# george-tyler-315-incline/ggml-neon-opt

Hardware: AMD Instinct MI355X
Metric: tg128 tok/s + Q4_K GEMV achieved-HBM-GB/s, TinyLlama-1.1B Q4_K_M @1 GPU (higher is better)
Workload: dtype q4_K/q6_K x q8_K (u4/u6*i8 dot4 -> i32, f32 combine); 1 GPU; tinyllama-1.1b Q4_K_M tg2221: full decode graph, token i at position i of a fresh f16 KV cache; parallelism=replicas x1, hipgraph=True

## Files before the change

ggml-neon-opt_amd/csrc/kq_api.hip:

```cpp
#include <algorithm>
#include <stdio.h>
#include <stdlib.h>
#include <string.h>

#include <atomic>
#include <mutex>
#include <string>
#include <vector>

#include <hip/hip_ext.h>

#include "kq_common.h"
#include "kq_internal.h"

namespace kq {

template <int NCOL, bool FUSEDQ, bool DEBUG, int TMASK>
__global__ void kq_gemv(const GemvArgs a);
__global__ void kq_quantize_q8K(const float *x, int64_t x_stride, uint8_t *y, int nb, int64_t nblocks);
template <int TMASK, bool FUSEDQ, int PRO>
__global__ void kq_rows(KQ_ROWS_PARAMS);
template <int TMASK, bool FUSEDQ, int PRO>
__global__ void kq_rows_dyn(KQ_ROWS_PARAMS);
template <bool AM>
__global__ void kq_quantize_q8L(const float *x, int64_t x_stride, uint8_t *y, int nb, int64_t nblocks);
template <int TYPE, int RT, int CW>
__global__ void kq_mmq(const MmqArgs a);
template <int RT, int CW>
__global__ void kq_mmq_mixed(const MmqArgs a);
__global__ void kq_stream_ceiling(const uint8_t *buf, int64_t per_wave, int waves_total, uint32_t *sink);
__global__ void kq_quantize_f16img(const float *x, int64_t x_stride, uint8_t *img, uint8_t *bs, int nb, int64_t nblocks);
template <int TYPE, int NW>
__global__ void kq_mmf(const MmfArgs a);
__global__ void kq_mmf_reduce(const float *slab, int n_split, int m_cols, int n_rows, int slab_rows, float *y,
                              int64_t y_col_stride, const float *res, int64_t res_col_stride);

namespace {

constexpr int kMaxDevices = 64;
std::mutex g_dev_mu;
std::atomic<int> g_dev_state[kMaxDevices];
int g_dev_cus[kMaxDevices] = {0};

int current_device() {
    int dev = 0;
    if (hipGetDevice(&dev) != hipSuccess || dev < 0 || dev >= kMaxDevices) return -1;
    return dev;
}

void probe_device(int dev) {
    int n = 0;
    if (hipGetDeviceCount(&n) != hipSuccess || n <= 0 || dev >= n) {
        g_dev_state[dev].store(-1);
        return;
    }
    hipDeviceProp_t prop;
    if (hipGetDeviceProperties(&prop, dev) != hipSuccess) {
        g_dev_state[dev].store(-1);
        return;
    }
    if (strncmp(prop.gcnArchName, "gfx950", 6) != 0) {
        fprintf(stderr, "ggml_mi355x: device %d is %s, this library is built for gfx950 only\n", dev,
                prop.gcnArchName);
        g_dev_state[dev].store(-1);
        return;
    }
    g_dev_cus[dev] = prop.multiProcessorCount > 0 ? prop.multiProcessorCount : 256;
    g_dev_state[dev].store(1, std::memory_order_release);
}

template <int NCOL, bool FUSEDQ, bool DEBUG>
gemv_fn pick_tm(int tmask) {
    switch (tmask) {
        case 1: return kq_gemv<NCOL, FUSEDQ, DEBUG, 1>;
        case 4: return kq_gemv<NCOL, FUSEDQ, DEBUG, 4>;
        default: return kq_gemv<NCOL, FUSEDQ, DEBUG, 7>;
    }
}

gemv_fn pick_gemv(int ncol, bool fusedq, bool debug, int tmask) {
    if (debug) return pick_tm<1, false, true>(tmask);
    if (fusedq) return pick_tm<1, true, false>(tmask);
    switch (ncol) {
        case 1: return pick_tm<1, false, false>(tmask);
        case 2: return pick_tm<2, false, false>(tmask);
        case 4: return pick_tm<4, false, false>(tmask);
        default: return pick_tm<8, false, false>(tmask);
    }
}

int type_bit(int type) { return type == Q4_K ? 1 : type == Q5_K ? 2 : type == Q6_K ? 4 : 0; }

constexpr size_t kMaxLds = 160 * 1024;
constexpr size_t kTargetLds = 80 * 1024;
constexpr int64_t kFusedQMaxNb = 32;
constexpr int64_t kRowsFusedMaxNb = ROWS_QPASS * 4 * ROWS_WAVES;
constexpr double kRowsSmallBytes = 5e6;
std::atomic<int> g_rows_waves{0};

struct KnobDef {
    const char *name;
    double def;
};
const KnobDef kKnobs[KNOB_COUNT] = {
    {"GEMV_DIAG", 0},  {"GEMV_RING", 0},     {"GEMV_PRE0", 1},       {"GEMV_PF", 0},
// ... 147 lines not shown
    a.R = BLOCKS_PER_STEP;
    a.m_total = (int)M;
    int64_t tasks = 0;
    for (int i = 0; i < n_desc; ++i) {
        a.type[i] = d[i].type;
        a.n_rows[i] = (int)d[i].n_rows;
        a.w[i] = (const uint8_t *)d[i].w;
        a.row_stride[i] = (int64_t)d[i].row_stride;
        a.y[i] = d[i].y;
        a.task_prefix[i] = (int)tasks;
        tasks += (d[i].n_rows + a.R - 1) / a.R;
    }
    if (tasks > 0x7fffffff) return MI355X_E_INVAL;
    for (int i = n_desc; i <= MI355X_MAX_FUSED; ++i) a.task_prefix[i] = (int)tasks;
    a.tasks_total = (int)tasks;
    pl.ncol = ncol;
    pl.fusedq = fusedq;
    pl.debug = debug;
    pl.tmask = tmask;
    pl.fn = pick_gemv(ncol, fusedq, debug, tmask);
    a.diag = (int)knob(KNOB_GEMV_DIAG);
    a.ring_override = (int)knob(KNOB_GEMV_RING);
    a.stamps = g_stamps;
    a.stamps_cap = g_stamps_cap;
    const int slot = tmask == 1 ? 8 * 16 * 9 : 8 * 16 * 14;
    const int dcands[3] = {tmask == 1 ? 8 : 6, tmask == 1 ? 6 : 5, 4};
    int D = 4;
    for (int i = 0; i < 3; ++i) {
        D = dcands[i];
        if ((size_t)lds_layout(ncol, (int)nb, 8 * ncol, fusedq, slot, D).total <= kTargetLds) break;
    }
    if (a.ring_override > 0) D = a.ring_override < 13 ? a.ring_override : 13;
    a.ring = D;
    const int64_t base_lds = lds_layout(ncol, (int)nb, 0, fusedq, slot, D).total;
    if ((size_t)base_lds > kMaxLds) return MI355X_E_UNSUPPORTED;
    int64_t wgs = (int64_t)num_cus() * resident_wgs((const void *)pl.fn, (size_t)base_lds + 1024);
    if (wgs > tasks) wgs = tasks > 0 ? tasks : 1;
    int64_t tpw = (tasks + wgs - 1) / wgs;
    while (tpw * 8 * ncol * 4 > 4096 && tpw > 1) {
        wgs *= 2;
        tpw = (tasks + wgs - 1) / wgs;
    }
    a.out_per_wg = (int)(tpw * 8 * ncol);
    const LdsLayout L = lds_layout(ncol, (int)nb, a.out_per_wg, fusedq, slot, D);
    if ((size_t)L.total > kMaxLds) return MI355X_E_UNSUPPORTED;
    pl.lds = (size_t)L.total;
    pl.grid = dim3((unsigned)wgs, (unsigned)((M + ncol - 1) / ncol), 1);
    return MI355X_OK;
}

void allow_lds(const void *fn, size_t lds) {
    if (lds <= 64 * 1024) return;
    static std::mutex mu;
    static std::vector<std::pair<int, const void *>> done;
    const int dev = current_device();
    std::lock_guard<std::mutex> lk(mu);
    for (auto &e : done)
        if (e.first == dev && e.second == fn) return;
    hipFuncSetAttribute(fn, hipFuncAttributeMaxDynamicSharedMemorySize, (int)kMaxLds);
    done.push_back({dev, fn});
}

int launch_gemv(const GemvPlan &pl, hipStream_t stream) {
    const GemvArgs &a = pl.a;
    if (a.tasks_total == 0 || a.m_total == 0) return MI355X_OK;
    allow_lds((const void *)pl.fn, pl.lds);
    hipEvent_t e0, e1;
    if (timing_slot(stream, e0, e1)) {
        hipExtLaunchKernelGGL(pl.fn, pl.grid, dim3(WG_THREADS), (uint32_t)pl.lds, stream, e0, e1, 0, a);
        timing_log(gemv_name(pl), gemv_bytes(a, pl.fusedq), e0, e1);
    } else {
        hipLaunchKernelGGL(pl.fn, pl.grid, dim3(WG_THREADS), pl.lds, stream, a);
    }
    const hipError_t e = hipGetLastError();
    return e == hipSuccess ? MI355X_OK : (int)e;
}

std::atomic<int> g_impl{MI355X_GEMV_AUTO};
bool rows_enabled() {
    return g_impl.load() != MI355X_GEMV_TASKS;
}


template <int TM, bool FQ, int PR>
rows_fn rows_inst(bool dyn) {
    if constexpr (TM == 7) {
        return kq_rows<TM, FQ, PR>;
    } else {
        return dyn ? kq_rows_dyn<TM, FQ, PR> : kq_rows<TM, FQ, PR>;
    }
}

template <int TM>
rows_fn rows_pick_pro(bool fusedq, int pro, bool dyn) {
    if (!fusedq) return rows_inst<TM, false, 0>(dyn);
    return pro == ROWS_PRO_NORM ? rows_inst<TM, true, 1>(dyn) : pro == ROWS_PRO_SWIGLU ? rows_inst<TM, true, 2>(dyn)
                                                                                       : rows_inst<TM, true, 0>(dyn);
}

rows_fn pick_rows(int tmask, bool fusedq, int pro, bool dyn = false) {
    switch (tmask) {
        case 1: return rows_pick_pro<1>(fusedq, pro, dyn);
        case 2: return rows_pick_pro<2>(fusedq, pro, dyn);
        case 4: return rows_pick_pro<4>(fusedq, pro, dyn);
        default: return rows_pick_pro<7>(fusedq, pro, false);
    }
}

int plan_rows(const mi355x_gemv_desc *d, int n_desc, int64_t K, bool fusedq, RowsPlan &pl, int waves_per_cu) {
    RowsArgs &a = pl.a;
    if (n_desc < 1 || n_desc > MI355X_MAX_FUSED) return MI355X_E_INVAL;
    if (K <= 0 || K % QK != 0) return MI355X_E_INVAL;
    const int64_t nb = K / QK;
    if (nb > 4096) return MI355X_E_UNSUPPORTED;
    if (fusedq && nb > kRowsFusedMaxNb) return MI355X_E_UNSUPPORTED;
    memset(&a, 0, sizeof(a));
    int tmask = 0;
    double bytes_total = 0;
    for (int i = 0; i < n_desc; ++i) {
        const int bb = block_bytes(d[i].type);
        if (!bb) return MI355X_E_UNSUPPORTED;
        if (d[i].n_rows < 0 || d[i].n_rows > 0x7fffffff) return MI355X_E_INVAL;
        if (d[i].n_rows > 0) {
            if (!d[i].w || !d[i].y) return MI355X_E_INVAL;
            if (((uintptr_t)d[i].w & 3u) != 0) return MI355X_E_INVAL;
            if (d[i].row_stride != (size_t)(nb * bb)) return MI355X_E_UNSUPPORTED;
            if (d[i].type != Q6_K && ((uintptr_t)d[i].w & 15u)) return MI355X_E_UNSUPPORTED;
        }
        bytes_total += (double)d[i].n_rows * bb;
        tmask |= type_bit(d[i].type);
    }
    if (tmask != 1 && tmask != 2 && tmask != 4) tmask = 7;
    pl.tmask = tmask;
    pl.fusedq = fusedq;
    pl.fn = pick_rows(tmask, fusedq, ROWS_PRO_NONE);
    a.n_desc = n_desc;
    a.nb = (int)nb;
    for (int i = 0; i < n_desc; ++i) {
        a.type[i] = d[i].type;
        a.w[i] = (const uint8_t *)d[i].w;
        a.y[i] = d[i].y;
        a.n_rows[i] = (int)d[i].n_rows;
    }
    {
        a.pf = (int)knob(KNOB_GEMV_PF);
        a.xmode = (int)knob(KNOB_GEMV_XMODE) & 7;
        a.diag = (int)knob(KNOB_GEMV_DIAG);
        const int pre = (int)knob(KNOB_GEMV_PRE0);
        a.pre0 = pre < 0 ? 0 : pre > 3 ? 3 : pre;
    }
    a.stamps = g_stamps;
    a.stamps_cap = g_stamps_cap;
    const double small_bytes = knob(KNOB_GEMV_SMALL_MB) * 1e6;
    if (waves_per_cu <= 0) {
        const int fixed = g_rows_waves.load();
        const int want = fixed > 0 ? fixed : bytes_total * nb < small_bytes ? ROWS_WAVES_SMALL : ROWS_WAVES;
        waves_per_cu = !fusedq || nb <= ROWS_QPASS * 4 * want ? want : ROWS_WAVES;
    }
    if (waves_per_cu > ROWS_WAVES) return MI355X_E_INVAL;
    pl.nwv = waves_per_cu;
    const int wpc_env = (int)knob(KNOB_GEMV_WPC);
    if (wpc_env > 0 && wpc_env < waves_per_cu) waves_per_cu = wpc_env;
    const int small_wg_env = (int)knob(KNOB_GEMV_SMALL_WG);
    int64_t n_wg = num_cus();
    if (small_wg_env > 0 && bytes_total * nb < small_bytes && small_wg_env < n_wg) n_wg = small_wg_env;
    const int64_t cap = n_wg * waves_per_cu;
    int64_t wv[MI355X_MAX_FUSED] = {0, 0, 0, 0};
    int64_t waves = 0;
    for (int i = 0; i < n_desc; ++i) {
        if (d[i].n_rows == 0) continue;
        const double share = (double)d[i].n_rows * block_bytes(d[i].type) / bytes_total;
        int64_t w = (int64_t)(share * (double)cap);
        const int64_t min_rows = (ROWS_SB + nb - 1) / nb;
        const int64_t wmax = (d[i].n_rows + min_rows - 1) / min_rows;
        if (w > wmax) w = wmax;
        if (w < 1) w = 1;
        wv[i] = w;
        waves += w;
    }
    while (waves > cap) {
        int big = 0;
        for (int i = 1; i < n_desc; ++i)
            if (wv[i] > wv[big]) big = i;
        --wv[big];
        --waves;
    }
    int64_t rpw = 0;
    waves = 0;
    for (int i = 0; i < n_desc; ++i) {
        a.wave_prefix[i] = (int)waves;
        if (wv[i] > 0) {
            a.rbase[i] = (int)(d[i].n_rows / wv[i]);
            a.rrem[i] = (int)(d[i].n_rows % wv[i]);
            const int64_t r = a.rbase[i] + (a.rrem[i] ? 1 : 0);
            rpw = r > rpw ? r : rpw;
        }
        waves += wv[i];
    }
    for (int i = n_desc; i <= MI355X_MAX_FUSED; ++i) a.wave_prefix[i] = (int)waves;
    a.waves_total = (int)waves;
    a.prio_bytes = 0;
    for (int i = 0; i < n_desc; ++i)
        if (wv[i] > 0) {
            const int64_t b = (int64_t)(a.rbase[i] + (a.rrem[i] ? 1 : 0)) * nb * block_bytes(d[i].type);
            a.prio_bytes = b > a.prio_bytes ? b : a.prio_bytes;
        }
    if (rpw > 0x7fffffff / 64) return MI355X_E_UNSUPPORTED;
    a.rpw = (int)(rpw > 0 ? rpw : 1);
    int g16 = ROWS_SB;
    while (nb % g16) g16 >>= 1;
    const int u = ROWS_SB / g16;
    int bR_full = (int)(ROWS_RECS / nb) / u * u;
    if (bR_full < u) bR_full = u;
    a.bR = a.rpw <= bR_full ? a.rpw : bR_full;
    const RowsLayout L = rows_layout((int)nb, tmask, a.bR, a.rpw, pl.nwv);
    if ((size_t)L.total > kMaxLds) return MI355X_E_UNSUPPORTED;
    pl.lds = (size_t)L.total;
    const int64_t grid = waves < n_wg ? waves : n_wg;
    pl.grid = dim3((unsigned)(grid > 0 ? grid : 1), 1, 1);
    pl.dyn = false;
    const double dyn_min = knob(KNOB_GEMV_DYN);
    const bool force = g_impl.load() == MI355X_GEMV_DYN;
    bool same_rows = true;
    for (int i = 1; i < n_desc; ++i) same_rows = same_rows && d[i].n_rows == d[0].n_rows;
    if (tmask != 7 && same_rows && (force || dyn_min > 0)) {
        int ush = 0;
        while ((int64_t)(1 << ush) * nb < ROWS_SB) ++ush;
        const double steps_per_wave = (double)n_desc * d[0].n_rows * nb / ROWS_SB / n_wg / pl.nwv;
        if ((int64_t)(1 << ush) * nb == ROWS_SB && steps_per_wave >= 16) ++ush;
        const int U = 1 << ush;
        const int Tu = (int)((U * nb + ROWS_SB - 1) / ROWS_SB);
        const int D = rows_depth(tmask == 1 ? Q4_K : tmask == 2 ? Q5_K : Q6_K);
        const int64_t flat = (int64_t)n_desc * ((d[0].n_rows + n_wg - 1) / n_wg);
        const int64_t rows = (int64_t)n_desc * d[0].n_rows;
        int bRd = (int)(ROWS_RECS / nb) / U * U;
        if (bRd < U) bRd = U;
        const double per_wave = (double)rows / (double)n_wg / U / pl.nwv;
        const bool auto_ok = per_wave >= dyn_min && steps_per_wave >= knob(KNOB_GEMV_DYN_STEPS);
        const RowsDynLayout DL = rows_dyn_layout((int)nb, tmask, bRd, (int)flat, pl.nwv);
        if ((force || auto_ok) && rows > 0 && (size_t)DL.total <= kMaxLds && flat < 0x7fffffff / 64) {
            pl.dyn = true;
            a.dyn_u = U;
            a.dyn_ush = ush;
            a.rbase[0] = (int)(d[0].n_rows / n_wg);
            a.rrem[0] = (int)(d[0].n_rows % n_wg);
            a.dyn_p = (D + Tu - 1) / Tu;
            const int p_knob = (int)knob(KNOB_GEMV_DYN_P);
            if (p_knob > 0) a.dyn_p = p_knob;
            a.bR = bRd;
            a.rpw = (int)flat;
            pl.lds = (size_t)DL.total;
            pl.grid = dim3((unsigned)n_wg, 1, 1);
            pl.fn = pick_rows(tmask, fusedq, ROWS_PRO_NONE, true);
        }
    }
    return MI355X_OK;
}

std::string rows_name(const RowsPlan &pl) {
    return std::string(pl.dyn ? "kq::kq_rows_dyn<" : "kq::kq_rows<") + std::to_string(pl.tmask) + ", " + (pl.fusedq ? "true" : "false") + ", " +
           std::to_string(pl.a.pro) + ">";
}

double rows_bytes(const RowsArgs &a, bool fusedq) {
    double w = 0, y = 0;
    for (int i = 0; i < a.n_desc; ++i) {
        const double rows = (double)a.n_rows[i];
        w += rows * a.nb * block_bytes(a.type[i]);
        y += rows * 4.0;
    }
    return w + y + (fusedq ? (double)a.nb * QK * 4.0 : (double)a.nb * Q8L_STRIDE);
}

int launch_rows(const RowsPlan &pl, hipStream_t stream) {
    const RowsArgs &a = pl.a;
    if (a.waves_total == 0) return MI355X_OK;
    allow_lds((const void *)pl.fn, pl.lds);
    const void *x = pl.fusedq ? (const void *)a.x : (const void *)a.xq;
    const int pass = 4 * pl.nwv;
    const int qiters = pl.fusedq ? (a.nb + pass - 1) / pass : 0;
    if (pl.nwv < 1 || pl.nwv > ROWS_WAVES || qiters > ROWS_QPASS || a.n_desc < 1 || a.n_desc > MI355X_MAX_FUSED)
        return MI355X_E_INVAL;
    const int cfg = rows_cfg(pl.nwv, qiters, a.n_desc, a.diag & 0x1ff);
    const int grid = (int)pl.grid.x;
    hipEvent_t e0, e1;
    if (timing_slot(stream, e0, e1)) {
        hipExtLaunchKernelGGL(pl.fn, pl.grid, dim3(pl.nwv * 64), (uint32_t)pl.lds, stream, e0, e1, 0, x, a.x2, a.w[0],
                              a.res[0], a.nb, a.waves_total, grid, cfg, a.rbase[0], a.rrem[0], a);
        timing_log(rows_name(pl), rows_bytes(a, pl.fusedq), e0, e1);
    } else {
        hipLaunchKernelGGL(pl.fn, pl.grid, dim3(pl.nwv * 64), pl.lds, stream, x, a.x2, a.w[0], a.res[0], a.nb,
                           a.waves_total, grid, cfg, a.rbase[0], a.rrem[0], a);
    }
    const hipError_t e = hipGetLastError();
    return e == hipSuccess ? MI355X_OK : (int)e;
}

int launch_quantize_q8L(const float *x, int64_t x_stride_floats, void *y, int64_t k, int64_t nrows,
                        hipStream_t stream, bool mmq) {
    const auto kern = mmq ? kq_quantize_q8L<true> : kq_quantize_q8L<false>;
    const int64_t nb = k / QK;
    const int64_t nblocks = nb * nrows;
    if (nblocks == 0) return MI355X_OK;
    const int64_t wgs = (nblocks + 15) / 16;
    hipEvent_t e0, e1;
    if (timing_slot(stream, e0, e1)) {
        hipExtLaunchKernelGGL(kern, dim3((unsigned)wgs), dim3(WG_THREADS), 0, stream, e0, e1, 0, x,
                              x_stride_floats, (uint8_t *)y, (int)nb, nblocks);
        timing_log("kq::kq_quantize_q8L", (double)nblocks * (QK * 4.0 + Q8L_STRIDE), e0, e1);
    } else {
        hipLaunchKernelGGL(kern, dim3((unsigned)wgs), dim3(WG_THREADS), 0, stream, x, x_stride_floats,
                           (uint8_t *)y, (int)nb, nblocks);
    }
    const hipError_t e = hipGetLastError();
    return e == hipSuccess ? MI355X_OK : (int)e;
}

constexpr int64_t kMmqMinCols = 16;

std::atomic<int> g_mmq_impl{MI355X_MMQ_AUTO};
int mmq_impl() { return g_mmq_impl.load(); }

struct MmqShape {
    int rt, cw;
};
MmqShape mmq_shape(int type, int64_t rows, int64_t M) {
    const int impl = mmq_impl();
    if (impl == MI355X_MMQ_TILE128) return {128, 1};
    if (impl == MI355X_MMQ_TILE128W) return {128, 2};
    if (impl == MI355X_MMQ_TILE64W) return {64, 2};
    if (impl == MI355X_MMQ_TILE64) return {64, 1};
    if (impl == MI355X_MMQ_TILE128X) return {128, type == Q6_K ? 2 : 4};
    if (impl == MI355X_MMQ_TILE192) return type == Q6_K ? MmqShape{128, 1} : MmqShape{192, 1};
    const int64_t rt128 = (rows + 127) / 128;
    const int64_t g128x128 = rt128 * ((M + 127) / 128), g128x64 = rt128 * ((M + 63) / 64);
    if (type != Q6_K && g128x128 >= 160 && g128x128 < 384 && g128x64 >= 512) return {128, 1};
    if (g128x128 >= 160) return {128, 2};
    if (type == Q6_K && ((rows + 63) / 64) * ((M + 127) / 128) >= 192) return {64, 2};
    if (type != Q6_K && rt128 * ((M + 63) / 64) >= 256) return {128, 1};
    return {64, 1};
}
const void *mmq_fn(int type, bool mixed, MmqShape sh) {
#define KQ_MMQ_PICK(RT, CW)                                                      \
    return mixed          ? (const void *)kq_mmq_mixed<RT, CW>                 \
         : type == Q5_K ? (const void *)kq_mmq<Q5_K, RT, CW>                   \
         : type == Q6_K ? (const void *)kq_mmq<Q6_K, RT, CW>                   \
                        : (const void *)kq_mmq<Q4_K, RT, CW>;
    if (sh.rt == 192 && !mixed && type != Q6_K)
        return type == Q5_K ? (const void *)kq_mmq<Q5_K, 192, 1> : (const void *)kq_mmq<Q4_K, 192, 1>;
    if (sh.rt == 128 && sh.cw == 4 && !mixed && type != Q6_K)
        return type == Q5_K ? (const void *)kq_mmq<Q5_K, 128, 4> : (const void *)kq_mmq<Q4_K, 128, 4>;
    if (sh.rt == 128 && sh.cw == 2) KQ_MMQ_PICK(128, 2)
    if (sh.rt == 64 && sh.cw == 2) KQ_MMQ_PICK(64, 2)
    if (sh.rt == 128) KQ_MMQ_PICK(128, 1)
    KQ_MMQ_PICK(64, 1)
#undef KQ_MMQ_PICK
}
size_t mmq_lds(int type, MmqShape sh) {
    return (size_t)mmq_nbuf(type, sh.rt, sh.cw) * (size_t)mmq_buf_bytes(type, sh.rt, sh.cw) + 16 + MMQ_PF_LDS;
}

int launch_mmq(int type, const void *w, int64_t K, int64_t N, size_t row_stride, const uint8_t *xq, int64_t M,
               float *y, int64_t y_col_stride, hipStream_t stream, const float *res, int64_t res_col_stride) {
// ... 254 lines not shown
        a.kv_k_cache = kv->k_cache;
        a.kv_v_cache = kv->v_cache;
        a.kv_n_ctx = kv->n_ctx;
        a.kv_hd = kv->hd;
    }
    a.w = a.mw[0];
    a.row_stride = a.mrow_stride[0];
    a.n_rows = a.mn_rows[0];
    a.y = a.my[0];
    a.y_col_stride = a.my_col_stride[0];
    const void *fn = mmq_fn(type, mixed, sh);
    size_t lds = mmq_lds(mixed ? Q6_K : type, sh);
    if (mixed) lds = std::max(lds, std::max(mmq_lds(Q4_K, sh), mmq_lds(Q5_K, sh)));
    const dim3 grid((unsigned)((M + mmq_cols(sh.cw) - 1) / mmq_cols(sh.cw)), (unsigned)tiles, 1);
    allow_lds(fn, lds);
    hipEvent_t e0, e1;
    void *args[] = {&a};
    hipError_t e;
    if (timing_slot(stream, e0, e1)) {
        e = hipExtLaunchKernel(fn, grid, dim3((unsigned)(64 * mmq_waves(rt, sh.cw))), args, lds, stream, e0, e1, 0);
        timing_log(mixed ? std::string("kq::kq_mmq_mixed") : std::string("kq::kq_mmq<") + std::to_string(type) + ">", wbytes + (double)M * a.nb * Q8L_STRIDE + ybytes,
                   e0, e1);
    } else {
        e = hipLaunchKernel(fn, grid, dim3((unsigned)(64 * mmq_waves(rt, sh.cw))), args, lds, stream);
    }
    if (e != hipSuccess) return (int)e;
    e = hipGetLastError();
    return e == hipSuccess ? MI355X_OK : (int)e;
}

bool mmq_applies(int type, const void *w, int64_t N, size_t row_stride, int64_t M) {
    if (!rows_enabled() || M < kMmqMinCols || N <= 0) return false;
    if (type != Q4_K && type != Q5_K && type != Q6_K) return false;
    if (N >= (1ll << 31) || M >= (1ll << 31)) return false;
    if (type == Q6_K) return true;
    return ((uintptr_t)w & 15u) == 0 && (row_stride & 15u) == 0;
}

int launch_quantize(const float *x, int64_t x_stride_floats, void *y, int64_t k, int64_t nrows,
                    hipStream_t stream) {
    const int64_t nb = k / QK;
    const int64_t nblocks = nb * nrows;
    if (nblocks == 0) return MI355X_OK;
    const int64_t wgs = (nblocks + WAVES_PER_WG - 1) / WAVES_PER_WG;
    hipEvent_t e0, e1;
    if (timing_slot(stream, e0, e1)) {
        hipExtLaunchKernelGGL(kq_quantize_q8K, dim3((unsigned)wgs), dim3(WG_THREADS), 0, stream, e0, e1, 0, x,
                              x_stride_floats, (uint8_t *)y, (int)nb, nblocks);
        timing_log("kq::kq_quantize_q8K", (double)nblocks * (QK * 4.0 + 292.0), e0, e1);
    } else {
        hipLaunchKernelGGL(kq_quantize_q8K, dim3((unsigned)wgs), dim3(WG_THREADS), 0, stream, x, x_stride_floats,
                           (uint8_t *)y, (int)nb, nblocks);
    }
    const hipError_t e = hipGetLastError();
    return e == hipSuccess ? MI355X_OK : (int)e;
}

size_t ext_x_bytes(int64_t k) { return ((size_t)k * 4 + 255) & ~(size_t)255; }

int gemv_m1(const mi355x_gemv_desc *d, int n, const float *x, int64_t k, void *ws, size_t ws_size,
            hipStream_t stream, const mi355x_gemv_ext *ext) {
    const bool has_ext = ext && (ext->prologue != MI355X_PRO_NONE || ext->epilogue != MI355X_EPI_NONE || [&] {
        for (int i = 0; i < n && i < MI355X_MAX_FUSED; ++i)
            if (ext->residual[i]) return true;
        return false;
    }());
    if (has_ext) {
        if (ext->prologue != MI355X_PRO_NONE && !ext->x2) return MI355X_E_INVAL;
        const bool epi = ext->epilogue == MI355X_EPI_SWIGLU;
        if (ext->epilogue != MI355X_EPI_NONE && !epi) return MI355X_E_INVAL;
        if (epi && (n != 2 || !ext->epi_y || d[0].n_rows != d[1].n_rows || ext->residual[0] || ext->residual[1]))
            return MI355X_E_INVAL;
        const bool x2_ok = ext->prologue == MI355X_PRO_NONE || ((uintptr_t)ext->x2 & 15u) == 0;
        if (rows_enabled() && k / QK <= kRowsFusedMaxNb && ((uintptr_t)x & 15u) == 0 && x2_ok) {
            RowsPlan rp;
            const int rc = plan_rows(d, n, k, true, rp);
            if (rc == MI355X_OK) {
                rp.a.x = x;
                rp.a.pro = ext->prologue == MI355X_PRO_RMS_NORM ? ROWS_PRO_NORM
                           : ext->prologue == MI355X_PRO_SWIGLU ? ROWS_PRO_SWIGLU
                                                                : ROWS_PRO_NONE;
                rp.a.x2 = ext->x2;
                rp.a.eps = ext->eps;
                rp.fn = pick_rows(rp.tmask, true, rp.a.pro, rp.dyn);
                for (int i = 0; i < n; ++i) {
                    rp.a.res[i] = ext->residual[i];
                    rp.a.n_rows[i] = (int)d[i].n_rows;
                }
                const int g = (int)rp.grid.x;
                const bool paired = epi && (rp.dyn || (rp.a.wave_prefix[2] == 2 * rp.a.wave_prefix[1] &&
                                                       rp.a.wave_prefix[1] % g == 0 && rp.a.rbase[0] == rp.a.rbase[1] &&
                                                       rp.a.rrem[0] == rp.a.rrem[1]));
                if (!epi || paired) {
                    if (paired) {
                        rp.a.epi = 1;
                        rp.a.epi_n = (int)d[0].n_rows;
                        rp.a.epi_wave_off = rp.a.wave_prefix[1] / g;
                        rp.a.epi_y = ext->epi_y;
                    }
                    if (!device_ok()) return MI355X_E_NODEVICE;
                    return launch_rows(rp, stream);
                }
            } else if (rc != MI355X_E_UNSUPPORTED) {
                return rc;
            }
        }
        const float *xs = x;
        uint8_t *w8 = (uint8_t *)ws;
        size_t wsz = ws_size;
        if (ext->prologue != MI355X_PRO_NONE) {
            if (!ws || ws_size < ext_x_bytes(k) || ((uintptr_t)ws & 15u)) return MI355X_E_WORKSPACE;
            if (!device_ok()) return MI355X_E_NODEVICE;
            float *xt = (float *)ws;
            const int rc = ext->prologue == MI355X_PRO_RMS_NORM ? launch_rms_norm(x, ext->x2, xt, k, 1, ext->eps, stream)
                                                                : launch_swiglu(x, ext->x2, xt, k, stream);
            if (rc) return rc;
            xs = xt;
            w8 += ext_x_bytes(k);
            wsz -= ext_x_bytes(k);
        }
        int rc = gemv_m1(d, n, xs, k, w8, wsz, stream, nullptr);
        if (rc) return rc;
        for (int i = 0; i < n; ++i)
            if (ext->residual[i] && d[i].n_rows > 0) {
                rc = launch_binary(0, d[i].y, ext->residual[i], d[i].y, d[i].n_rows, stream);
                if (rc) return rc;
            }
        if (epi && d[0].n_rows > 0) return launch_swiglu(d[0].y, d[1].y, ext->epi_y, d[0].n_rows, stream);
        return MI355X_OK;
    }
    const bool fusedq = k / QK <= kFusedQMaxNb && ((uintptr_t)x & 15u) == 0;
    const size_t need = (size_t)(k / QK) * 292;
    if (rows_enabled()) {
        RowsPlan rp;
        const int64_t fq_max = (int64_t)knob(KNOB_GEMV_FQMAX);
        const bool rows_fq = k / QK <= fq_max && k / QK <= kRowsFusedMaxNb && ((uintptr_t)x & 15u) == 0;
        int rc = plan_rows(d, n, k, rows_fq, rp);
        if (rc == MI355X_OK) {
            if (rows_fq) {
                rp.a.x = x;
                if (!device_ok()) return MI355X_E_NODEVICE;
                return launch_rows(rp, stream);
            }
            const size_t need_l = (size_t)(k / QK) * Q8L_STRIDE;
            if (!ws || ws_size < need_l || ((uintptr_t)ws & 15u)) return MI355X_E_WORKSPACE;
            if (!device_ok()) return MI355X_E_NODEVICE;
            rc = launch_quantize_q8L(x, k, ws, k, 1, stream);
            if (rc) return rc;
            rp.a.xq = (const uint8_t *)ws;
            return launch_rows(rp, stream);
        }
        if (rc != MI355X_E_UNSUPPORTED) return rc;
    }
    GemvPlan pl;
    int rc = plan_gemv(d, n, k, 1, 1, fusedq, false, pl);
    if (rc) return rc;
    if (fusedq) {
        pl.a.x = x;
        pl.a.x_col_stride = k;
        if (!device_ok()) return MI355X_E_NODEVICE;
        return launch_gemv(pl, stream);
    }
    if (!ws || ws_size < need || ((uintptr_t)ws & 3u)) return MI355X_E_WORKSPACE;
    if (!device_ok()) return MI355X_E_NODEVICE;
    rc = launch_quantize(x, k, ws, k, 1, stream);
    if (rc) return rc;
    pl.a.xq = (const uint8_t *)ws;
// ... 153 lines not shown
    if (ne11 == 0 || ne01 == 0) return MI355X_OK;
    if (!src1 || ((uintptr_t)src1 & 3u) || (nb11 & 3u) || !dst || ((uintptr_t)dst & 3u) || (nb1 & 3u))
        return MI355X_E_INVAL;
    if (ne11 > 1 && (nb11 < (size_t)ne00 * 4 || nb1 < (size_t)ne01 * 4)) return MI355X_E_INVAL;
    if (ne11 == 1) {
        mi355x_gemv_desc d = {src0_type, src0, ne01, nb01, dst};
        return gemv_m1(&d, 1, src1, ne00, workspace, workspace_size, (hipStream_t)stream);
    }
    size_t need = mi355x_mul_mat_workspace_size(src0_type, ne00, ne01, ne11);
    if (!workspace || workspace_size < need) return MI355X_E_WORKSPACE;
    if (mmf_applies(src0_type, src0, ne01, nb01, ne11, ne00) && ((uintptr_t)workspace & 15u) == 0) {
        if (!device_ok()) return MI355X_E_NODEVICE;
        int rc = launch_f16img(src1, (int64_t)(nb11 / 4), (uint8_t *)workspace, ne00, ne11, (hipStream_t)stream);
        if (rc) return rc;
        return launch_mmf_gemm(src0_type, src0, ne00, ne01, nb01, (uint8_t *)workspace, ne11, dst, (int64_t)(nb1 / 4),
                               (hipStream_t)stream);
    }
    if (mmq_applies(src0_type, src0, ne01, nb01, ne11) && ((uintptr_t)workspace & 15u) == 0) {
        if (!device_ok()) return MI355X_E_NODEVICE;
        int rc = launch_quantize_q8L(src1, (int64_t)(nb11 / 4), workspace, ne00, ne11, (hipStream_t)stream, true);
        if (rc) return rc;
        return launch_mmq(src0_type, src0, ne00, ne01, nb01, (const uint8_t *)workspace, ne11, dst,
                          (int64_t)(nb1 / 4), (hipStream_t)stream);
    }
    if (!device_ok()) return MI355X_E_NODEVICE;
    int rc = launch_quantize(src1, (int64_t)(nb11 / 4), workspace, ne00, ne11, (hipStream_t)stream);
    if (rc) return rc;
    const size_t q8_row = (size_t)(ne00 / QK) * 292;
    return mi355x_mul_mat_q8(src0_type, src0, ne00, ne01, nb01, workspace, ne11, q8_row, dst, nb1, stream);
}

int mi355x_gemv_fused(const mi355x_gemv_desc *descs, int n_desc, const float *x, int64_t k, void *workspace,
                      size_t workspace_size, void *stream) {
    if (!descs || !x || ((uintptr_t)x & 3u)) return MI355X_E_INVAL;
    if (k <= 0 || k % QK) return MI355X_E_INVAL;
    for (int i = 0; i < n_desc && i < MI355X_MAX_FUSED; ++i)
        if (descs[i].y && ((uintptr_t)descs[i].y & 3u)) return MI355X_E_INVAL;
    return gemv_m1(descs, n_desc, x, k, workspace, workspace_size, (hipStream_t)stream);
}

size_t mi355x_gemv_ext_workspace_size(int64_t k) {
    if (k <= 0 || k % QK) return 0;
    return ext_x_bytes(k) + mi355x_gemv_fused_workspace_size(k);
}

int mi355x_gemv_fused_ext(const mi355x_gemv_desc *descs, int n_desc, const float *x, int64_t k,
                          const mi355x_gemv_ext *ext, void *workspace, size_t workspace_size, void *stream) {
    if (!descs || !x || ((uintptr_t)x & 3u)) return MI355X_E_INVAL;
    if (k <= 0 || k % QK || n_desc < 1 || n_desc > MI355X_MAX_FUSED) return MI355X_E_INVAL;
    if (ext && (ext->prologue < MI355X_PRO_NONE || ext->prologue > MI355X_PRO_SWIGLU)) return MI355X_E_INVAL;
    if (ext && ext->prologue == MI355X_PRO_RMS_NORM && !(ext->eps >= 0.0f)) return MI355X_E_INVAL;
    if (ext && ext->epilogue == MI355X_EPI_SWIGLU && ((uintptr_t)ext->epi_y & 3u)) return MI355X_E_INVAL;
    for (int i = 0; i < n_desc; ++i) {
        if (descs[i].y && ((uintptr_t)descs[i].y & 3u)) return MI355X_E_INVAL;
        if (ext && ext->residual[i] && ((uintptr_t)ext->residual[i] & 3u)) return MI355X_E_INVAL;
    }
    return gemv_m1(descs, n_desc, x, k, workspace, workspace_size, (hipStream_t)stream, ext);
}

int mi355x_debug_stream(const void *buf, size_t bytes, void *sink, void *stream) {
    if (!buf || !sink || ((uintptr_t)buf & 15u)) return MI355X_E_INVAL;
    int dev = current_device();
    if (dev < 0 || !device_ok()) return MI355X_E_NODEVICE;
    const int cus = g_dev_cus[dev] > 0 ? g_dev_cus[dev] : 256;
    const int waves = cus * 12;
    const int64_t per_wave = (int64_t)(bytes / waves) / 2048 * 2048;
    if (per_wave <= 0) return MI355X_E_INVAL;
    const size_t lds = 4 * 4 * 2048;
    allow_lds((const void *)kq_stream_ceiling, lds);
    hipStream_t st = (hipStream_t)stream;
    hipEvent_t e0, e1;
    if (timing_slot(st, e0, e1)) {
        hipExtLaunchKernelGGL(kq_stream_ceiling, dim3((unsigned)(cus * 3)), dim3(256), (uint32_t)lds, st, e0, e1, 0,
                              (const uint8_t *)buf, per_wave, waves, (uint32_t *)sink);
        timing_log("kq::kq_stream_ceiling", (double)per_wave * waves, e0, e1);
    } else {
        hipLaunchKernelGGL(kq_stream_ceiling, dim3((unsigned)(cus * 3)), dim3(256), lds, st, (const uint8_t *)buf,
                           per_wave, waves, (uint32_t *)sink);
    }
    const hipError_t e = hipGetLastError();
    return e == hipSuccess ? MI355X_OK : (int)e;
}

int mi355x_debug_block_partials(int src0_type, const void *src0, int64_t ne00, int64_t ne01, size_t nb01,
                                const void *src1_q8, int32_t *out, void *stream) {
    if (!out || !src1_q8 || ((uintptr_t)src1_q8 & 3u)) return MI355X_E_INVAL;
    if (ne01 == 0) return MI355X_OK;
    const int64_t nb = ne00 / QK;
    float *dst = (float *)out;
    mi355x_gemv_desc d = {src0_type, src0, ne01, nb01, dst};
    GemvPlan pl;
    int rc = plan_gemv(&d, 1, ne00, 1, 1, false, true, pl);
    if (rc) return rc;
    pl.a.xq = (const uint8_t *)src1_q8;
    pl.a.xq_col_stride = (int64_t)(nb * 292);
    pl.a.dbg = out;
    if (!device_ok()) return MI355X_E_NODEVICE;
    return launch_gemv(pl, (hipStream_t)stream);
}

int mi355x_gemv_impl(int impl) {
    if (impl < MI355X_GEMV_AUTO || impl > MI355X_GEMV_DYN) return MI355X_E_INVAL;
    return g_impl.exchange(impl);
}

int mi355x_debug_knob(const char *name, double value, double *previous) {
    if (!name) return MI355X_E_INVAL;
    for (int k = 0; k < KNOB_COUNT; ++k) {
        if (strcmp(name, kKnobs[k].name) != 0) continue;
        if (previous) *previous = knob((Knob)k);
        if (value != value) {
            g_knob_set[k].store(false);
        } else {
            g_knob[k].store(value);
            g_knob_set[k].store(true);
        }
        g_knob_gen.fetch_add(1);
        return MI355X_OK;
    }
    return MI355X_E_INVAL;
}

int mi355x_mmq_impl(int impl) {
    if (impl < MI355X_MMQ_AUTO || impl > MI355X_MMQ_TILE192) return MI355X_E_INVAL;
    const int prev = mmq_impl();
    g_mmq_impl.store(impl);
    return prev;
}

int mi355x_prefill_precision(int precision) {
    if (precision < 0) return prefill_precision();
    if (precision > MI355X_PREFILL_F16_ALL) return MI355X_E_INVAL;
    const int prev = prefill_precision();
    g_prefill.store(precision);
    return prev;
}

int mi355x_gemv_waves(int waves) {
    if (waves < 0 || waves > ROWS_WAVES) return MI355X_E_INVAL;
    return g_rows_waves.exchange(waves);
}

}
namespace kq {
uint64_t *diag_stamps(int64_t *cap) {
    if (cap) *cap = g_stamps_cap;
    return g_stamps;
}
}
extern "C" {
int mi355x_diag_stamps(void *buf, size_t bytes) {
    g_stamps = (uint64_t *)buf;
    g_stamps_cap = buf ? (int64_t)(bytes / 8) : 0;
    return MI355X_OK;
}

int mi355x_timing_enable(int enable) {
    std::lock_guard<std::mutex> lk(g_tmu);
    g_timing = enable != 0;
    g_tlog.clear();
    g_tpool_used = 0;
    return MI355X_OK;
}

int mi355x_timing_read(mi355x_launch_timing *out, int max) {
    if (hipDeviceSynchronize() != hipSuccess) return MI355X_E_NODEVICE;
// ... 59 lines not shown
```

ggml-neon-opt_amd/csrc/kq_common.h:

```cpp
#pragma once

#include <hip/hip_runtime.h>
#include <stdint.h>

#include "ggml_mi355x.h"

namespace kq {

constexpr int QK = 256;
constexpr int WAVE = 64;
constexpr int WG_THREADS = 256;
constexpr int WAVES_PER_WG = WG_THREADS / WAVE;
constexpr int LANES_PER_BLOCK = 8;
constexpr int BLOCKS_PER_STEP = WAVE / LANES_PER_BLOCK;
constexpr int ACT_QS_STRIDE = 272;
constexpr int MAX_NCOL = 8;

constexpr int Q4_K = MI355X_TYPE_Q4_K;
constexpr int Q5_K = MI355X_TYPE_Q5_K;
constexpr int Q6_K = MI355X_TYPE_Q6_K;

__host__ __device__ constexpr int block_bytes(int type) {
    return type == Q4_K ? 144 : type == Q5_K ? 176 : type == Q6_K ? 210 : 0;
}

struct GemvArgs {
    int n_desc;
    int nb;
    int R;
    int m_total;
    int tasks_total;
    int out_per_wg;
    int diag;
    int ring;
    int ring_override;
    int task_prefix[MI355X_MAX_FUSED + 1];
    int type[MI355X_MAX_FUSED];
    int n_rows[MI355X_MAX_FUSED];
    const uint8_t *w[MI355X_MAX_FUSED];
    int64_t row_stride[MI355X_MAX_FUSED];
    float *y[MI355X_MAX_FUSED];
    int64_t y_col_stride[MI355X_MAX_FUSED];
    const float *x;
    int64_t x_col_stride;
    const uint8_t *xq;
    int64_t xq_col_stride;
    int32_t *dbg;
    uint64_t *stamps;
    int64_t stamps_cap;
};

struct LdsLayout {
    int ring, act, act_per_wave, act_col, recs, outs, spw, total;
};

__host__ __device__ inline LdsLayout lds_layout(int ncol, int nb, int out_per_wg, bool fusedq, int slot, int D) {
    LdsLayout L;
    L.spw = (nb + WAVES_PER_WG - 1) / WAVES_PER_WG;
    L.ring = 0;
    L.act = WAVES_PER_WG * D * slot;
    L.act_col = (L.spw * 292 + 16 + 15) & ~15;
    L.act_per_wave = fusedq ? L.spw * 1024 : ncol * L.act_col;
    L.recs = L.act + WAVES_PER_WG * L.act_per_wave;
    L.outs = L.recs + 2 * (WAVES_PER_WG - 1) * ncol * 8 * L.spw * 16;
    L.total = L.outs + out_per_wg * 4;
    return L;
}

#ifndef KQ_ROWS_WAVES
#define KQ_ROWS_WAVES 12
#endif
constexpr int ROWS_WAVES = KQ_ROWS_WAVES;
#ifndef KQ_ROWS_WAVES_SMALL
#define KQ_ROWS_WAVES_SMALL 6
#endif
constexpr int ROWS_WAVES_SMALL = KQ_ROWS_WAVES_SMALL;
constexpr int ROWS_QPASS = 3;
#ifndef KQ_ROWS_PF
#define KQ_ROWS_PF 2
#endif
constexpr int ROWS_PF = KQ_ROWS_PF;

#define KQ_ROWS_PARAMS                                                                                        \
    const void *x, const float *x2, const uint8_t *w0, const float *res0, int nb, int waves_total, int grid, \
        int cfg, int rbase0, int rrem0, const RowsArgs a
__host__ __device__ constexpr int rows_cfg(int nwv, int qiters, int n_desc, int diag) {
    return nwv | (qiters << 8) | (n_desc << 12) | (diag << 16);
}

struct RowsArgs {
    int bR;
    int rpw;
    int wave_prefix[MI355X_MAX_FUSED + 1];
    int epi;
    int rbase[MI355X_MAX_FUSED];
    int rrem[MI355X_MAX_FUSED];
    int type[MI355X_MAX_FUSED];
    const uint8_t *w[MI355X_MAX_FUSED];
    const float *res[MI355X_MAX_FUSED];
    float *y[MI355X_MAX_FUSED];
    float *epi_y;
    float eps;
    int epi_n, epi_wave_off;
    int dyn_u, dyn_p, dyn_ush;
    int n_rows[MI355X_MAX_FUSED];
    uint64_t *stamps;
    int64_t stamps_cap;
    int n_desc;
    int nb;
    int waves_total;
    const float *x;
    const uint8_t *xq;
    const float *x2;
    int pro;
    int diag;
    int pre0;
    int pf;
    int xmode;
    int64_t prio_bytes;
};
constexpr int ROWS_PRO_NONE = 0, ROWS_PRO_NORM = 1, ROWS_PRO_SWIGLU = 2;
constexpr int ROWS_X_ROT = 1, ROWS_X_BAR = 2, ROWS_X_PIPE = 4;

constexpr int ROWS_SB = 16;
#ifndef KQ_MMQ_PF
#define KQ_MMQ_PF 0
#endif
constexpr int MMQ_PF_LDS = KQ_MMQ_PF ? 1024 : 0;
constexpr int Q8L_STRIDE = 304;
#ifndef KQ_MMQ_NBUF
#define KQ_MMQ_NBUF 2
#endif
__host__ __device__ constexpr int mmq_cgroups(int cw) { return cw == 4 ? 1 : 2; }
__host__ __device__ constexpr int mmq_cols(int cw) { return 32 * cw * mmq_cgroups(cw); }
__host__ __device__ constexpr int mmq_waves(int rt, int cw) { return rt / 32 * mmq_cgroups(cw); }
#ifndef KQ_MMQ_Q6_STRIDE
#define KQ_MMQ_Q6_STRIDE 240
#endif
static_assert(KQ_MMQ_Q6_STRIDE % 16 == 0 && KQ_MMQ_Q6_STRIDE >= 224, "whole granules");
__host__ __device__ constexpr int mmq_buf_bytes(int type, int rt, int cw) {
    return mmq_cols(cw) * Q8L_STRIDE + rt * (type == Q6_K ? KQ_MMQ_Q6_STRIDE : block_bytes(type));
}
__host__ __device__ constexpr int mmq_nbuf(int type, int rt, int cw) {
    return KQ_MMQ_NBUF == 1 ? 1 : KQ_MMQ_NBUF >= 3 && ((rt == 128 && cw == 1) || (rt == 64 && cw == 2)) &&
                   3 * mmq_buf_bytes(type, rt, cw) + 16 + MMQ_PF_LDS <= 160 * 1024
               ? 3
               : 2;
}
constexpr int ROWS_RECS = 64;
__host__ __device__ constexpr int rows_gran(int type) { return block_bytes(type) + 1; }
__host__ __device__ constexpr int rows_slot(int type) { return 16 * rows_gran(type); }
__host__ __device__ constexpr int rows_ni(int type) { return (rows_gran(type) + 63) / 64; }
#ifndef KQ_ROWS_DQ4
#define KQ_ROWS_DQ4 3
#endif
#ifndef KQ_ROWS_DQ6
#define KQ_ROWS_DQ6 2
#endif
__host__ __device__ constexpr int rows_depth(int type) {
    return type == Q4_K ? KQ_ROWS_DQ4 : type == Q5_K ? 3 : KQ_ROWS_DQ6;
}
__host__ __device__ constexpr int rows_ring_bytes(int type) { return rows_depth(type) * rows_slot(type); }
__host__ __device__ constexpr int cmax(int a, int b) { return a > b ? a : b; }
__host__ __device__ constexpr int rows_ring(int tmask) {
    return 16 + cmax((tmask & 1) ? rows_ring_bytes(Q4_K) : 0,
                     cmax((tmask & 2) ? rows_ring_bytes(Q5_K) : 0, (tmask & 4) ? rows_ring_bytes(Q6_K) : 0));
}

struct RowsLayout {
    int act, ring, ring_stride, recs, recs_stride, outs, outs_stride, sums, total;
// ... 160 lines not shown
```

ggml-neon-opt_amd/csrc/kq_internal.h:

```cpp
#pragma once

#include <string>

#include "kq_common.h"

namespace kq {

int device_ok();
bool timing_slot(hipStream_t s, hipEvent_t &a, hipEvent_t &b);
void timing_log(const std::string &kernel, double bytes, hipEvent_t a, hipEvent_t b);
int num_cus();
int choose_ncol(int64_t M, int nb);
typedef void (*gemv_fn)(const GemvArgs);
struct GemvPlan {
    GemvArgs a;
    dim3 grid;
    size_t lds;
    gemv_fn fn;
    int ncol, tmask;
    bool fusedq, debug;
};
int plan_gemv(const mi355x_gemv_desc *d, int n_desc, int64_t K, int64_t M, int ncol, bool fusedq, bool debug,
              GemvPlan &pl);
int launch_gemv(const GemvPlan &pl, hipStream_t stream);
typedef void (*rows_fn)(KQ_ROWS_PARAMS);
struct RowsPlan {
    RowsArgs a;
    dim3 grid;
    size_t lds;
    rows_fn fn;
    int tmask;
    bool fusedq;
    int nwv;
    bool dyn = false;
};
int plan_rows(const mi355x_gemv_desc *d, int n_desc, int64_t K, bool fusedq, RowsPlan &pl,
              int waves_per_cu = 0);
int launch_rows(const RowsPlan &pl, hipStream_t stream);
bool rows_enabled();
int launch_quantize(const float *x, int64_t x_stride_floats, void *y, int64_t k, int64_t nrows,
                    hipStream_t stream);
int gemv_m1(const mi355x_gemv_desc *d, int n, const float *x, int64_t k, void *ws, size_t ws_size,
            hipStream_t stream, const mi355x_gemv_ext *ext = nullptr);
int launch_rms_norm(const float *x, const float *w, float *y, int64_t n, int64_t nrows, float eps, hipStream_t s);
int launch_binary(int op, const float *a, const float *b, float *y, int64_t n, hipStream_t s,
                  int64_t nb = 0);
int launch_attn_prompt(const AttnArgs &a, int n_tok, hipStream_t s);
int attn_cells_reserve(const AttnArgs &a, hipStream_t stream);
bool attn_prompt_q8_ok(const AttnArgs &a);
bool mmq_applies(int type, const void *w, int64_t N, size_t row_stride, int64_t M);
int launch_quantize_q8L(const float *x, int64_t x_stride_floats, void *y, int64_t k, int64_t nrows,
                        hipStream_t stream, bool mmq = false);
int launch_mmq(int type, const void *w, int64_t K, int64_t N, size_t row_stride, const uint8_t *xq, int64_t M,
               float *y, int64_t y_col_stride, hipStream_t stream, const float *res = nullptr,
               int64_t res_col_stride = 0);
bool mmq_tile64(int type, int64_t N, int64_t M);
bool mmf_on();
bool mmf_applies(int type, const void *w, int64_t N, size_t row_stride, int64_t M, int64_t K);
bool mmf_prefers(int type, int64_t N, int64_t K);
int launch_f16img(const float *x, int64_t x_stride_floats, uint8_t *ws, int64_t K, int64_t M, hipStream_t stream);
int launch_mmf_gemm(int type, const void *w, int64_t K, int64_t N, size_t row_stride, uint8_t *ws, int64_t M,
                    float *y, int64_t y_col_stride, hipStream_t stream, const float *res = nullptr,
                    int64_t res_col_stride = 0);
int launch_mmf_multi(int type, int n_mat, const void *const *w, const int64_t *N, const size_t *row_stride,
                     float *const *y, const int64_t *y_col_stride, int64_t K, uint8_t *ws, size_t ws_size, int64_t M,
                     hipStream_t stream, const float *res = nullptr, int64_t res_col_stride = 0);
struct MmqKv {
    int kind[4];
    const int32_t *pos;
    const float *rope;
    uint16_t *k_cache, *v_cache;
    int n_ctx, hd;
};
int launch_mmq_multi(const int *types, int n_mat, const void *const *w, const int64_t *N, const size_t *row_stride,
                     float *const *y, const int64_t *y_col_stride, int64_t K, const uint8_t *xq, int64_t M,
                     hipStream_t stream, const MmqKv *kv = nullptr);
int launch_rms_norm_q8L(const float *x, const float *w, void *yq, int64_t n, int64_t nrows, float eps, hipStream_t s);
int launch_swiglu_q8L(const float *g, const float *u, void *yq, int64_t n, int64_t nrows, hipStream_t s);
int launch_swiglu(const float *g, const float *u, float *y, int64_t n, hipStream_t s);
int attn_args_from(const mi355x_attn_desc *d, AttnArgs &a);
int launch_attn(const AttnArgs &a, hipStream_t s);
bool attn_group_ok(const AttnArgs &a, int nwaves);
size_t attn_group_bytes(const AttnArgs &a, int nwaves);
constexpr size_t kAttnOprojCounterBytes = 1024;
constexpr int kAttnOprojMaxCtx = 256;
size_t attn_oproj_buffer(int hd, int n_head, int n_head_kv, int n_ctx, int type, int64_t K, int64_t n_rows, int *nsb);
int launch_attn_oproj(const AttnArgs &a, int type, const void *w, int64_t n_rows, size_t row_stride, const float *res,
                      float *y, uint8_t *buf, size_t buf_size, hipStream_t stream);
int attn_batch_args_from(const mi355x_attn_batch_desc *d, int n_pos, AttnBatchArgs &b);
int attn_batch_form(const AttnBatchArgs &b);
int launch_attn_batch(const AttnBatchArgs &b, hipStream_t s);
int attn_impl();
size_t attn_lds16(int hd, int n_ctx);
int layer_plan(LayerArgs &a, int hd, int n_head);
int launch_layer(const LayerArgs &a, hipStream_t stream);
int64_t layer_table_stride(const LayerArgs &a);
void layer_table_fill(const LayerArgs &a, uint8_t *buf, int64_t stride);
uint64_t *diag_stamps(int64_t *cap);
void allow_lds(const void *fn, size_t lds);
enum Knob {
    KNOB_GEMV_DIAG,
    KNOB_GEMV_RING,
    KNOB_GEMV_PRE0,
    KNOB_GEMV_PF,
    KNOB_GEMV_XMODE,
    KNOB_GEMV_SMALL_MB,
    KNOB_GEMV_WPC,
    KNOB_GEMV_SMALL_WG,
    KNOB_GEMV_FQMAX,
    KNOB_MMF_WAVES,
    KNOB_MMF_ORDER,
    KNOB_ATTN_DIAG,
    KNOB_LOOPBACK_NOCOPY,
    KNOB_ATTN_OPROJ,
    KNOB_AO_NRB,
    KNOB_GEMV_DYN,
    KNOB_GEMV_DYN_P,
    KNOB_GEMV_DYN_STEPS,
    KNOB_COUNT
};
double knob(Knob k);
// ... 6 lines not shown
```

ggml-neon-opt_amd/csrc/kq_rows.hip:

```cpp
#include <hip/hip_ext.h>

#include "kq_internal.h"
#include "kq_ops_device.h"
#include "kq_rows_device.h"

#ifndef KQ_ROWS_DIAG
#define KQ_ROWS_DIAG 0
#endif
#if KQ_ROWS_DIAG
#define RDIAG(ld) ((ld).diag)
#define RSTAMPS(h) ((h).stamps)
#define RSTAMP() __builtin_amdgcn_s_memrealtime()
#else
#define RDIAG(ld) 0
#define RSTAMPS(h) ((uint64_t *)nullptr)
#define RSTAMP() ((uint64_t)0)
#endif

#ifndef KQ_ROWS_XMODE
#define KQ_ROWS_XMODE 0
#endif
#ifndef KQ_ROWS_PRE0
#define KQ_ROWS_PRE0 1
#endif
// ... 192 lines not shown
    __device__ __forceinline__ T *ptr() const {
        return (T *)(uintptr_t)((uint64_t)dw<I>() | ((uint64_t)dw<I + 1>() << 32));
    }
};
__device__ __forceinline__ RowsRun rows_fetch() {
    const auto *ka = __builtin_amdgcn_kernarg_segment_ptr();
    RowsRun r;
    asm volatile("s_load_dwordx16 %0, %4, %5\n\t"
                 "s_load_dwordx16 %1, %4, %6\n\t"
                 "s_load_dwordx16 %2, %4, %7\n\t" KQ_ROWS_RUN_TAIL " %3, %4, %8\n\t"
                 "s_waitcnt lgkmcnt(0)"
                 : "=&s"(r.a), "=&s"(r.b), "=&s"(r.c), "=&s"(r.d)
                 : "s"(ka), "i"(kRowsArgsOff), "i"(kRowsArgsOff + 64), "i"(kRowsArgsOff + 128), "i"(kRowsArgsOff + 192));
    return r;
}

template <class T>
__device__ __forceinline__ T sreg(T v) {
    asm volatile("" : "+s"(v));
    return v;
}

struct RowsHot {
    int m, r0, nrows;
    int type, bR, rpw;
    const uint8_t *w;
    const float *res;
    float *y;
    float eps;
    int epi, epi_n, epi_wave_off;
    float *epi_y;
    uint64_t *stamps;
    int64_t stamps_cap;
};

template <int TMASK>
__device__ __forceinline__ RowsHot rows_resolve(const RowsLead &ld, int gw) {
    const RowsRun r = rows_fetch();
    RowsHot h;
    h.bR = r.i32<RA_DW(bR)>(), h.rpw = r.i32<RA_DW(rpw)>();
    h.epi = r.i32<RA_DW(epi)>(), h.epi_n = r.i32<RA_DW(epi_n)>(), h.epi_wave_off = r.i32<RA_DW(epi_wave_off)>();
    h.eps = __uint_as_float(r.dw<RA_DW(eps)>());
    h.epi_y = r.ptr<float, RA_DW(epi_y)>();
#if KQ_ROWS_DIAG
    h.stamps = r.ptr<uint64_t, RA_DW(stamps)>();
    h.stamps_cap = (int64_t)(uintptr_t)r.ptr<uint8_t, RA_DW(stamps_cap)>();
#else
    h.stamps = nullptr, h.stamps_cap = 0;
#endif
    h.m = 0, h.w = ld.w0, h.res = ld.res0;
    h.type = TMASK == 7 ? sreg(r.i32<RA_DW(type)>()) : 0;
    h.y = sreg(r.ptr<float, RA_DW(y)>());
    int j = gw, base = ld.rbase0, rem = ld.rrem0;
    if (ld.n_desc > 1) {
        const int p1 = sreg(r.i32<RA_DW(wave_prefix) + 1>()), p2 = sreg(r.i32<RA_DW(wave_prefix) + 2>()),
                  p3 = sreg(r.i32<RA_DW(wave_prefix) + 3>());
        const int b1 = sreg(r.i32<RA_DW(rbase) + 1>()), b2 = sreg(r.i32<RA_DW(rbase) + 2>()), b3 = sreg(r.i32<RA_DW(rbase) + 3>());
        const int e1 = sreg(r.i32<RA_DW(rrem) + 1>()), e2 = sreg(r.i32<RA_DW(rrem) + 2>()), e3 = sreg(r.i32<RA_DW(rrem) + 3>());
        const uint8_t *w1 = sreg(r.ptr<const uint8_t, RA_DW(w) + 2>()), *w2 = sreg(r.ptr<const uint8_t, RA_DW(w) + 4>()),
                      *w3 = sreg(r.ptr<const uint8_t, RA_DW(w) + 6>());
        const float *s1 = sreg(r.ptr<const float, RA_DW(res) + 2>()), *s2 = sreg(r.ptr<const float, RA_DW(res) + 4>()),
                    *s3 = sreg(r.ptr<const float, RA_DW(res) + 6>());
        float *y1 = sreg(r.ptr<float, RA_DW(y) + 2>()), *y2 = sreg(r.ptr<float, RA_DW(y) + 4>()), *y3 = sreg(r.ptr<float, RA_DW(y) + 6>());
        int m = gw >= p1 ? 1 : 0;
        if (ld.n_desc > 2 && gw >= p2) m = 2;
        if (ld.n_desc > 3 && gw >= p3) m = 3;
        h.m = m;
        j = gw - (m == 0 ? 0 : m == 1 ? p1 : m == 2 ? p2 : p3);
        base = m == 0 ? base : m == 1 ? b1 : m == 2 ? b2 : b3;
        rem = m == 0 ? rem : m == 1 ? e1 : m == 2 ? e2 : e3;
        if (TMASK == 7) {
            const int t1 = sreg(r.i32<RA_DW(type) + 1>()), t2 = sreg(r.i32<RA_DW(type) + 2>()), t3 = sreg(r.i32<RA_DW(type) + 3>());
            h.type = m == 0 ? h.type : m == 1 ? t1 : m == 2 ? t2 : t3;
        }
        h.w = m == 0 ? h.w : m == 1 ? w1 : m == 2 ? w2 : w3;
        h.res = m == 0 ? h.res : m == 1 ? s1 : m == 2 ? s2 : s3;
        h.y = m == 0 ? h.y : m == 1 ? y1 : m == 2 ? y2 : y3;
    }
    h.r0 = j * base + (j < rem ? j : rem);
    h.nrows = gw < ld.waves_total ? base + (j < rem ? 1 : 0) : 0;
    return h;
}

template <int TYPE, bool FUSEDQ, int PRO, int TMASK, class Resolve>
__device__ __forceinline__ void rows_body(const RowsArgs &a, const RowsLead &ld, uint8_t *smem, int wave, int lane,
                                          uint64_t st0, Resolve resolve) {
    constexpr int BSZ = block_bytes(TYPE);
    constexpr int GRAN = rows_gran(TYPE);
    constexpr int NI = rows_ni(TYPE);
    constexpr int SLOT = rows_slot(TYPE);
    constexpr int D = rows_depth(TYPE);
    static_assert(D >= 2 && D <= 4, "vm_wait_k covers 3 steps in flight");
    const int nb = ld.nb;
    const int nwv = ld.nwv;
    const int q = lane >> 2, s = lane & 3;

    const int PASS = 4 * nwv;
    const int xm = !FUSEDQ ? 0 : KQ_ROWS_XMODE >= 0 ? KQ_ROWS_XMODE : a.xmode;
    u32x4 xv[ROWS_QPASS][4] = {};
    u32x4 x2v[ROWS_QPASS][4] = {};
    int qw = 0;
    const int rot = (xm & ROWS_X_ROT) ? (int)(blockIdx.x % (unsigned)nb) : 0;
    auto sbk = [&](int j) {
        int b = (j < nb ? j : nb - 1) + rot;
        return b >= nb ? b - nb : b;
    };
    if (FUSEDQ) {
        const float *const x = (const float *)ld.x;
#pragma unroll
        for (int i = 0; i < ROWS_QPASS; ++i) qw += (i < ld.qiters && PASS * i + 4 * wave < nb) ? 1 : 0;
#pragma unroll
        for (int i = 0; i < ROWS_QPASS; ++i) {
            if (i < qw) {
                const int b = sbk(PASS * i + 4 * wave + (lane >> 4));
                const float *xp = x + (int64_t)b * QK + 16 * (lane & 15);
#pragma unroll
                for (int k = 0; k < 4; ++k) xv[i][k] = gload16_asm(xp + 4 * k);
                if (PRO != ROWS_PRO_NONE) {
                    const float *x2p = ((RDIAG(ld) & 16) ? x : ld.x2) + (int64_t)b * QK + 16 * (lane & 15);
#pragma unroll
                    for (int k = 0; k < 4; ++k) x2v[i][k] = gload16_asm(x2p + 4 * k);
                }
            }
        }
    }
    const RowsHot h = resolve();
    const uint64_t sa = RSTAMP();
    const int bR = h.bR;
    const RowsLayout L = rows_layout(nb, TMASK, bR, h.rpw, nwv);
    uint8_t *const ring = smem + L.ring + wave * L.ring_stride;
    uint8_t *const ring_end = ring + D * SLOT;
    Rec *const recs = (Rec *)(smem + L.recs + wave * L.recs_stride);
    float *const outs = (float *)(smem + L.outs + wave * L.outs_stride);
    const uint8_t *const actq = smem + L.act;

    const int G = h.nrows * nb;
    const int T = (G + ROWS_SB - 1) / ROWS_SB;
    const uint8_t *src = h.w + (int64_t)h.r0 * nb * BSZ;
    const uint32_t mis = (uint32_t)((uintptr_t)src & 15u);
    const uint8_t *s16 = src - mis;
    const uint8_t *last16 =
        G > 0 ? (const uint8_t *)((uintptr_t)(src + (int64_t)G * BSZ - 1) & ~(uintptr_t)15) : s16;

    const bool pf_on = FUSEDQ && (KQ_ROWS_L2PF < 0 ? a.pf != 0 : KQ_ROWS_L2PF != 0) && T > D + 1;
    uint32_t pf_sink = 0;
    uint8_t *islot = ring;
    int it_ = 0;
    auto issue = [&]() {
        const uint8_t *base = s16 + (int64_t)it_ * (ROWS_SB * BSZ) + 16 * lane;
        if (it_ + 1 < T) {
#pragma unroll
            for (int i = 0; i < NI; ++i)
                if (i + 1 < NI || lane < GRAN - 64 * (NI - 1)) dma16_nt(base + 1024 * i, (LDS void *)(islot + 1024 * i));
        } else {
#pragma unroll
            for (int i = 0; i < NI; ++i) {
                const uint8_t *p = base + 1024 * i;
                if (i + 1 < NI || lane < GRAN - 64 * (NI - 1))
                    dma16_nt(p < last16 ? p : last16, (LDS void *)(islot + 1024 * i));
            }
        }
        islot = islot + SLOT == ring_end ? ring : islot + SLOT;
        ++it_;
    };

    const float *const res_p = h.res;
    uint32_t rv = 0;

    const int pre_req = KQ_ROWS_PRE0 < 0 ? a.pre0 : KQ_ROWS_PRE0;
    const int pre_cap = pre_req < D ? pre_req : D;
    const int pre0 = T >= pre_cap ? pre_cap : (T > 0 ? T : 0);
    uint64_t sx = 0, sq = 0, sf = 0;
    if (FUSEDQ) {
        const float *const x = (const float *)ld.x;
        constexpr int pro = PRO;
        constexpr int PL = PRO != ROWS_PRO_NONE ? 8 : 4;
        rv = gload4_asm(res_p && h.nrows > 0 ? res_p + h.r0 + (lane < h.nrows ? lane : 0) : x);
        if (xm & ROWS_X_BAR) asm volatile("s_barrier" ::: "memory");
        constexpr bool kConstPre = KQ_ROWS_PRE0 == 1 && KQ_ROWS_L2PF == 0;
        if (kConstPre && T == 0) {
            const uint8_t *xb = (const uint8_t *)x + 16 * lane;
#pragma unroll
            for (int i = 0; i < NI; ++i)
                if (KQ_ROWS_MASKED && i + 1 == NI) dma16_nt_lanes(xb, (LDS void *)(islot + 1024 * i), lane, GRAN - 64 * (NI - 1));
                else if (i + 1 < NI || lane < GRAN - 64 * (NI - 1)) dma16_nt(xb, (LDS void *)(islot + 1024 * i));
        }
        if (KQ_ROWS_MASKED && kConstPre && T > 0) {
            const uint8_t *base = s16 + 16 * lane;
            const uint8_t *lim = T > 1 ? base + 1024 * (NI - 1) : base + 1024 * (NI - 1) < last16 ? base + 1024 * (NI - 1) : last16;
#pragma unroll
            for (int i = 0; i + 1 < NI; ++i) {
                const uint8_t *p = base + 1024 * i;
                dma16_nt(T > 1 || p < last16 ? p : last16, (LDS void *)(islot + 1024 * i));
            }
            dma16_nt_lanes(lim, (LDS void *)(islot + 1024 * (NI - 1)), lane, GRAN - 64 * (NI - 1));
            islot = islot + SLOT == ring_end ? ring : islot + SLOT;
            ++it_;
        } else {
            for (int j = 0; j < pre0; ++j) issue();
        }
        if (pf_on) {
            const uint8_t *p = s16 + (int64_t)D * (ROWS_SB * BSZ) + 64 * lane;
#pragma unroll
            for (int i = 0; i < ROWS_PF; ++i) l2_touch(p + 4096 * i < last16 ? p + 4096 * i : last16, pf_sink);
        }
        const int tail = 1 + NI * pre0 + (pf_on ? ROWS_PF : 0);
        auto pin = [&]() {
            asm volatile("" : "+v"(xv[0][0]), "+v"(xv[0][1]), "+v"(xv[0][2]), "+v"(xv[0][3]), "+v"(xv[1][0]),
                         "+v"(xv[1][1]), "+v"(xv[1][2]), "+v"(xv[1][3]), "+v"(xv[2][0]), "+v"(xv[2][1]),
                         "+v"(xv[2][2]), "+v"(xv[2][3]));
            if (pro != ROWS_PRO_NONE) {
#pragma unroll
                for (int i = 0; i < ROWS_QPASS; ++i)
#pragma unroll
                    for (int k = 0; k < 4; ++k) asm volatile("" : "+v"(x2v[i][k]));
            }
        };
        if (pro != ROWS_PRO_NORM && (xm & ROWS_X_PIPE)) {
#pragma unroll
            for (int i = 0; i < ROWS_QPASS; ++i) {
                if (i < qw) {
                    vm_wait_dyn((qw - 1 - i) * PL + tail);
                    pin();
                    if (pro == ROWS_PRO_SWIGLU && !(RDIAG(ld) & 32)) {
#pragma unroll
                        for (int k = 0; k < 4; ++k) xv[i][k] = swiglu4(xv[i][k], x2v[i][k]);
                    }
                    const int j = PASS * i + 4 * wave + (lane >> 4);
                    if (j < nb && !(RDIAG(ld) & 64)) quant16_store(xv[i], lane & 15, smem + L.act + Q8L_STRIDE * sbk(j));
                }
            }
            if (RSTAMPS(h)) sx = sq = __builtin_amdgcn_s_memrealtime();
        } else {
            if (KQ_ROWS_LINT_BREAK) {
            } else if (kConstPre && KQ_ROWS_MASKED == 2) {
                vm_wait<NI + 1>();
            } else if (kConstPre) {
                vm_wait<NI>();
            } else {
                vm_wait_dyn(tail);
            }
            pin();
            if (RDIAG(ld) & 32) {
            } else if (pro == ROWS_PRO_SWIGLU) {
#pragma unroll
                for (int i = 0; i < ROWS_QPASS; ++i)
                    if (i < qw)
#pragma unroll
                        for (int k = 0; k < 4; ++k) xv[i][k] = swiglu4(xv[i][k], x2v[i][k]);
            } else if (pro == ROWS_PRO_NORM) {
                double *sums = (double *)(smem + L.sums);
#pragma unroll
                for (int i = 0; i < ROWS_QPASS; ++i) {
                    if (i < qw) {
                        const int j = PASS * i + 4 * wave + (lane >> 4);
                        double sq = 0.0;
                        if (j < nb) {
                            float v[16];
#pragma unroll
                            for (int k = 0; k < 4; ++k) {
                                v[4 * k] = __uint_as_float(xv[i][k].x), v[4 * k + 1] = __uint_as_float(xv[i][k].y);
                                v[4 * k + 2] = __uint_as_float(xv[i][k].z), v[4 * k + 3] = __uint_as_float(xv[i][k].w);
                            }
                            sq = sumsq16(v);
                        }
                        sq = row16_sum(sq);
                        if (j < nb && (lane & 15) == 0) sums[sbk(j)] = sq;
                    }
                }
                asm volatile("s_waitcnt lgkmcnt(0)\n\ts_barrier" ::: "memory");
                double tot = seq_sum_lanes(sums, nb, lane);
                if (rms_mean_ambiguous(div_by_count(tot, (int64_t)nb * QK), (int64_t)nb * QK))
                    tot = seq_sumsq_wave(x, (int64_t)nb * QK, lane);
                const float mean = (float)div_by_count(tot, (int64_t)nb * QK);
                const float scale = 1.0f / sqrtf(mean + h.eps);
#pragma unroll
                for (int i = 0; i < ROWS_QPASS; ++i)
                    if (i < qw)
#pragma unroll
                        for (int k = 0; k < 4; ++k) xv[i][k] = normmul4(xv[i][k], x2v[i][k], scale);
            }
            if (RSTAMPS(h)) sx = __builtin_amdgcn_s_memrealtime();
#pragma unroll 1
            for (int i = 0; i < qw; ++i) {
                u32x4 cur[4];
#pragma unroll
                for (int k = 0; k < 4; ++k) cur[k] = i == 0 ? xv[0][k] : i == 1 ? xv[1][k] : xv[2][k];
                const int j = PASS * i + 4 * wave + (lane >> 4);
                if (j < nb && !(RDIAG(ld) & 64)) quant16_store(cur, lane & 15, smem + L.act + Q8L_STRIDE * sbk(j));
            }
            if (RSTAMPS(h)) {
                asm volatile("s_waitcnt lgkmcnt(0)" ::: "memory");
                sq = __builtin_amdgcn_s_memrealtime();
            }
        }
    } else {
        const int ng = nb * (Q8L_STRIDE / 16);
        for (int j = wave; 64 * j < ng; j += nwv) {
            const int k = 64 * j + lane;
            if (k < ng) dma16((const uint8_t *)ld.x + 16 * k, (LDS void *)(smem + L.act + 1024 * j));
        }
        for (int j = 0; j < pre0; ++j) issue();
        vm_wait_k<NI>(pre0);
    }
    while (it_ < D && it_ < T) issue();
    asm volatile("s_waitcnt lgkmcnt(0)\n\ts_barrier" ::: "memory");
    const uint64_t st1 = RSTAMPS(h) ? __builtin_amdgcn_s_memrealtime() : 0;

    int io = q, rr = 0;
    while (io >= nb) {
        io -= nb;
        ++rr;
    }
    int bend = bR * nb < G ? bR * nb : G;
    int brow = 0;
    const uint8_t *cslot = ring;
    int prio = -1;
#pragma unroll 1
    for (int t = 0; t < T; ++t) {
        if (KQ_ROWS_PRIO && (t & 3) == 0) {
            const int64_t rem = (int64_t)(T - t) * (ROWS_SB * BSZ);
            int p = (int)(rem * 4 / (a.prio_bytes + 1));
            p = __builtin_amdgcn_readfirstlane(p > 3 ? 3 : p);
            if (p != prio) {
                prio = p;
                if (p == 3) __builtin_amdgcn_s_setprio(3);
                else if (p == 2) __builtin_amdgcn_s_setprio(2);
                else if (p == 1) __builtin_amdgcn_s_setprio(1);
                else __builtin_amdgcn_s_setprio(0);
            }
        }
        if (pf_on && t < pre0) {
            if (T - t >= D) vm_wait<NI * (D - 1) + ROWS_PF>();
            else vm_wait_kp<NI, ROWS_PF>(T - t - 1);
        } else if (T - t >= D) {
            vm_wait<NI * (D - 1)>();
        } else {
            vm_wait_k<NI>(T - t - 1);
        }
        if (!(RDIAG(ld) & 8) && ROWS_SB * t + q < G) {
            const uint8_t *blk = cslot + mis + q * BSZ;
            const uint8_t *ab = actq + io * Q8L_STRIDE;
            QuadOut r = TYPE == Q4_K ? quad_q4K(blk, ab, s) : TYPE == Q5_K ? quad_q5K(blk, ab, s) : quad_q6K(blk, ab, s);
            const int isum = quad_sum(r.isum);
            const int imin = quad_sum(r.imin);
            if (s == 0) {
                const float yd = *(const float *)ab;
                Rec rec;
                if (TYPE == Q6_K) {
                    rec.a = isum - 32 * imin;
                    rec.b = 0;
                    rec.c = h2f(r.dh) * yd;
                    rec.e = 0.f;
                } else {
                    rec.a = isum;
                    rec.b = imin;
                    rec.c = yd * h2f(r.dh & 0xffffu);
                    rec.e = yd * h2f(r.dh >> 16);
                }
                recs[io * bR + rr] = rec;
            }
        }
        cslot = cslot + SLOT == ring_end ? ring : cslot + SLOT;
        io += ROWS_SB;
        if (nb >= ROWS_SB) {
            if (io >= nb) {
                io -= nb;
                ++rr;
            }
        } else {
            while (io >= nb) {
                io -= nb;
                ++rr;
            }
        }
        if (it_ < T) issue();
        if (RSTAMPS(h) && t == 0) sf = __builtin_amdgcn_s_memrealtime();
        if (ROWS_SB * (t + 1) >= bend) {
            wave_lds_fence();
            const int nr = bR < h.nrows - brow ? bR : h.nrows - brow;
            if (lane < nr) {
                float v = 0.f;
                const Rec *rc = recs + lane;
#pragma unroll 4
                for (int i = 0; i < nb; ++i) v = chain_step(TYPE, rc[i * bR], v);
                outs[brow + lane] = v;
            }
            brow += bR;
            rr -= bR;
            bend = bend + bR * nb < G ? bend + bR * nb : G;
            wave_lds_fence();
        }
    }
    if (KQ_ROWS_PRIO) __builtin_amdgcn_s_setprio(0);
    const uint64_t st2 = RSTAMPS(h) ? __builtin_amdgcn_s_memrealtime() : 0;
    if (pf_on) {
        asm volatile("" ::"v"(pf_sink));
    }

    if (h.nrows > 0) {
        wave_lds_fence();
        float *y = h.y + h.r0;
        if (res_p) {
            asm volatile("s_waitcnt vmcnt(0)" ::: "memory");
            asm volatile("" : "+v"(rv));
            for (int k = 0; k < h.nrows; k += 64)
                if (k + lane < h.nrows)
                    store_y(y + k + lane, outs[k + lane] + (k == 0 ? __uint_as_float(rv) : res_p[h.r0 + k + lane]));
        } else {
            for (int k = 0; k < h.nrows; k += 64)
                if (k + lane < h.nrows) store_y(y + k + lane, outs[k + lane]);
        }
    }
    if (h.epi && !(RDIAG(ld) & 128)) {
        asm volatile("s_waitcnt lgkmcnt(0)\n\ts_barrier" ::: "memory");
        if (h.m == 1 && h.nrows > 0) {
            const float *gouts = (const float *)(smem + L.outs + (wave - h.epi_wave_off) * L.outs_stride);
            const int n4 = h.epi_n & ~3;
            for (int k = 0; k < h.nrows; k += 64)
                if (k + lane < h.nrows) {
                    const int r = h.r0 + k + lane;
                    const float gv = gouts[k + lane], uv = outs[k + lane];
                    store_y(h.epi_y + r, r < n4 ? v_silu(gv) * uv : (gv / (1.0f + expf(-gv))) * uv);
                }
        }
    }
    if (RSTAMPS(h)) {
        const int64_t o = ((int64_t)blockIdx.x * ROWS_WAVES + wave) * 8;
        if (lane == 0 && o + 7 < h.stamps_cap) {
            RSTAMPS(h)[o] = st0;
            RSTAMPS(h)[o + 1] = st1;
            RSTAMPS(h)[o + 2] = st2;
            RSTAMPS(h)[o + 3] = __builtin_amdgcn_s_memrealtime();
            RSTAMPS(h)[o + 4] = sx;
            RSTAMPS(h)[o + 5] = sq;
            RSTAMPS(h)[o + 6] = sf;
            RSTAMPS(h)[o + 7] = sa;
        }
    }
}

template <int TMASK, bool FUSEDQ, int PRO>
__global__ void __launch_bounds__(ROWS_WAVES * 64) kq_rows(KQ_ROWS_PARAMS) {
    extern __shared__ __attribute__((aligned(16))) uint8_t smem[];
    const RowsLead ld = rows_lead(x, x2, w0, res0, nb, waves_total, grid, cfg, rbase0, rrem0);
    if (RDIAG(ld) & 256) return;
    const uint64_t st0 = RSTAMP();
    const int lane = threadIdx.x & 63;
    const int wave = __builtin_amdgcn_readfirstlane(threadIdx.x >> 6);
    const int gw = wave * ld.grid + blockIdx.x;
    auto resolve = [&]() { return rows_resolve<TMASK>(ld, gw); };

    if (TMASK == 1) {
        rows_body<Q4_K, FUSEDQ, PRO, TMASK>(a, ld, smem, wave, lane, st0, resolve);
    } else if (TMASK == 2) {
        rows_body<Q5_K, FUSEDQ, PRO, TMASK>(a, ld, smem, wave, lane, st0, resolve);
    } else if (TMASK == 4) {
        rows_body<Q6_K, FUSEDQ, PRO, TMASK>(a, ld, smem, wave, lane, st0, resolve);
    } else {
        const RowsHot h = resolve();
        auto resolved = [&]() { return h; };
        if (h.type == Q6_K) rows_body<Q6_K, FUSEDQ, PRO, TMASK>(a, ld, smem, wave, lane, st0, resolved);
        else if (h.type == Q5_K) rows_body<Q5_K, FUSEDQ, PRO, TMASK>(a, ld, smem, wave, lane, st0, resolved);
        else rows_body<Q4_K, FUSEDQ, PRO, TMASK>(a, ld, smem, wave, lane, st0, resolved);
    }
}

#define KQ_ROWS_INST(TM, FQ, PR) template __global__ void kq_rows<TM, FQ, PR>(KQ_ROWS_PARAMS);
#define KQ_ROWS_INST_T(TM)        \
    KQ_ROWS_INST(TM, true, 0)     \
    KQ_ROWS_INST(TM, true, 1)     \
    KQ_ROWS_INST(TM, true, 2)     \
    KQ_ROWS_INST(TM, false, 0)
KQ_ROWS_INST_T(1)
KQ_ROWS_INST_T(2)
KQ_ROWS_INST_T(4)
KQ_ROWS_INST_T(7)

#ifndef KQ_ROWS_DYN_RR
#define KQ_ROWS_DYN_RR 0
#endif
namespace {
static_assert(MI355X_MAX_FUSED == 4, "four matrices at most");
struct DynUnit {
    const uint8_t *src;
    int rows, flat, G, T;
};
}

struct RowsDynHot {
    int bR, rpw, U, P, ush, N, epi, epi_n;
    const uint8_t *w1, *w2, *w3;
    const float *s1, *s2, *s3;
    float *y0, *y1, *y2, *y3, *epi_y;
    float eps;
    uint64_t *stamps;
    int64_t stamps_cap;
};
__device__ __forceinline__ RowsDynHot rows_dyn_resolve() {
    const RowsRun r = rows_fetch();
    RowsDynHot h;
    h.bR = r.i32<RA_DW(bR)>(), h.rpw = r.i32<RA_DW(rpw)>();
    h.U = r.i32<RA_DW(dyn_u)>(), h.P = r.i32<RA_DW(dyn_p)>(), h.ush = r.i32<RA_DW(dyn_ush)>(), h.N = r.i32<RA_DW(n_rows)>();
    h.epi = r.i32<RA_DW(epi)>(), h.epi_n = r.i32<RA_DW(epi_n)>();
    h.epi_y = r.ptr<float, RA_DW(epi_y)>();
    h.eps = __uint_as_float(r.dw<RA_DW(eps)>());
    h.w1 = sreg(r.ptr<const uint8_t, RA_DW(w) + 2>()), h.w2 = sreg(r.ptr<const uint8_t, RA_DW(w) + 4>());
    h.w3 = sreg(r.ptr<const uint8_t, RA_DW(w) + 6>());
    h.s1 = sreg(r.ptr<const float, RA_DW(res) + 2>()), h.s2 = sreg(r.ptr<const float, RA_DW(res) + 4>());
    h.s3 = sreg(r.ptr<const float, RA_DW(res) + 6>());
    h.y0 = sreg(r.ptr<float, RA_DW(y)>()), h.y1 = sreg(r.ptr<float, RA_DW(y) + 2>());
    h.y2 = sreg(r.ptr<float, RA_DW(y) + 4>()), h.y3 = sreg(r.ptr<float, RA_DW(y) + 6>());
#if KQ_ROWS_DIAG
    h.stamps = r.ptr<uint64_t, RA_DW(stamps)>();
    h.stamps_cap = (int64_t)(uintptr_t)r.ptr<uint8_t, RA_DW(stamps_cap)>();
#else
    h.stamps = nullptr, h.stamps_cap = 0;
#endif
    return h;
}

template <int TYPE, bool FUSEDQ, int PRO, int TMASK>
__device__ __forceinline__ void rows_dyn_body(const RowsArgs &a, const RowsLead &ld, uint8_t *smem, int wave, int lane,
                                              uint64_t st0) {
    uint64_t sx = 0, sq = 0, sf = 0;
    constexpr int BSZ = block_bytes(TYPE);
    constexpr int GRAN = rows_gran(TYPE);
    constexpr int NI = rows_ni(TYPE);
    constexpr int SLOT = rows_slot(TYPE);
    constexpr int D = rows_depth(TYPE);
    static_assert(D >= 2 && D <= 4, "vm_wait_k covers 3 steps in flight");
    const int nb = ld.nb;
    const int nwv = ld.nwv;
    const int b = (int)blockIdx.x;
    const int q = lane >> 2, s = lane & 3;

    const float *const x = (const float *)ld.x;
    const int PASS = 4 * nwv;
    u32x4 xv[ROWS_QPASS][4] = {};
    u32x4 x2v[ROWS_QPASS][4] = {};
    int qw = 0;
    if (FUSEDQ) {
#pragma unroll
        for (int i = 0; i < ROWS_QPASS; ++i) qw += (i < ld.qiters && PASS * i + 4 * wave < nb) ? 1 : 0;
#pragma unroll
        for (int i = 0; i < ROWS_QPASS; ++i) {
            if (i < qw) {
                const int j = PASS * i + 4 * wave + (lane >> 4);
                const int bb = j < nb ? j : nb - 1;
                const float *xp = x + (int64_t)bb * QK + 16 * (lane & 15);
#pragma unroll
                for (int k = 0; k < 4; ++k) xv[i][k] = gload16_asm(xp + 4 * k);
                if (PRO != ROWS_PRO_NONE) {
                    const float *x2p = ld.x2 + (int64_t)bb * QK + 16 * (lane & 15);
#pragma unroll
                    for (int k = 0; k < 4; ++k) x2v[i][k] = gload16_asm(x2p + 4 * k);
                }
            }
        }
    }
    const RowsDynHot h = rows_dyn_resolve();
    const uint8_t *const w0 = ld.w0, *const w1 = h.w1, *const w2 = h.w2, *const w3 = h.w3;
    const float *const s0 = ld.res0, *const s1 = h.s1, *const s2 = h.s2, *const s3 = h.s3;
    float *const y0 = h.y0, *const y1 = h.y1, *const y2 = h.y2, *const y3 = h.y3;
    const int U = h.U, P = h.P, bR = h.bR;
    const RowsDynLayout L = rows_dyn_layout(nb, TMASK, bR, h.rpw, nwv);
    uint8_t *const ring = smem + L.ring + wave * L.ring_stride;
    uint8_t *const ring_end = ring + D * SLOT;
    Rec *const recs = (Rec *)(smem + L.recs + wave * L.recs_stride);
    float *const outs = (float *)(smem + L.outs);
    uint32_t *const cnt = (uint32_t *)(smem + L.cnt);
    const uint8_t *const actq = smem + L.act;

    const int N = h.N;
    const int ush = h.ush;
    const int rbase = ld.rbase0, rrem = ld.rrem0;
    const int r0 = b * rbase + (b < rrem ? b : rrem);
    const int nr = rbase + (b < rrem ? 1 : 0);
    const int nu = (nr + U - 1) >> ush;
    const int units = ld.n_desc * nu, nflat = ld.n_desc * nr;
    const int64_t rowb = (int64_t)nb * BSZ;
    auto row_of = [&](int f) { return r0 + f; };
    auto unit_of = [&](int u) {
        DynUnit d;
        const int m = (u >= nu ? 1 : 0) + (u >= 2 * nu ? 1 : 0) + (u >= 3 * nu ? 1 : 0);
        const int lr = (u - m * nu) << ush;
        d.rows = nr - lr < U ? nr - lr : U;
        d.flat = m * nr + lr;
        const uint8_t *w = m == 0 ? w0 : m == 1 ? w1 : m == 2 ? w2 : w3;
        d.src = w + (int64_t)(r0 + lr) * rowb;
        d.G = d.rows * nb;
        d.T = (d.G + ROWS_SB - 1) / ROWS_SB;
        return d;
    };
    const int nstat = nwv * P < units ? nwv * P : units;

    uint32_t ul = 0, uh = 0, ug = 0, uf = 0;
    int ki = -1, is = 0, iT = 0, issued = 0;
    bool idone = false, iwait = false;
    const uint8_t *is16 = nullptr, *il16 = nullptr;
    uint8_t *islot = ring;
    auto take = [&](int u) {
        ++ki;
        const DynUnit d = unit_of(u);
        const bool mine = lane == (ki & 7);
        ul = mine ? (uint32_t)(uintptr_t)d.src : ul;
        uh = mine ? (uint32_t)((uintptr_t)d.src >> 32) : uh;
        ug = mine ? (uint32_t)(d.G | (d.rows << 16)) : ug;
        uf = mine ? (uint32_t)d.flat : uf;
        is16 = (const uint8_t *)((uintptr_t)d.src & ~(uintptr_t)15);
        il16 = (const uint8_t *)((uintptr_t)(d.src + (int64_t)d.G * BSZ - 1) & ~(uintptr_t)15);
        iT = d.T;
        is = 0;
    };
    auto next_unit = [&](bool claim_ok) {
        const int k = ki + 1;
        if (k < P) {
            const int u = wave * P + k;
            if (u < nstat) take(u);
            else idone = true;
            return;
        }
        if (!claim_ok) {
            iwait = true;
            return;
        }
        iwait = false;
#if KQ_ROWS_DYN_RR
        const int uu = nwv * P + (k - P) * nwv + wave;
#else
        uint32_t u = 0;
        if (lane == 0) u = __hip_atomic_fetch_add(cnt, 1u, __ATOMIC_RELAXED, __HIP_MEMORY_SCOPE_WORKGROUP);
        const int uu = __builtin_amdgcn_readfirstlane((int)u);
#endif
        if (uu < units) take(uu);
        else idone = true;
    };
    auto issue = [&](bool claim_ok) {
        const uint8_t *base = is16 + (int64_t)is * (ROWS_SB * BSZ) + 16 * lane;
        if (is + 1 < iT) {
#pragma unroll
            for (int i = 0; i < NI; ++i)
                if (i + 1 < NI || lane < GRAN - 64 * (NI - 1)) dma16_nt(base + 1024 * i, (LDS void *)(islot + 1024 * i));
        } else {
#pragma unroll
            for (int i = 0; i < NI; ++i) {
                const uint8_t *p = base + 1024 * i;
                if (i + 1 < NI || lane < GRAN - 64 * (NI - 1))
                    dma16_nt(p < il16 ? p : il16, (LDS void *)(islot + 1024 * i));
            }
        }
        islot = islot + SLOT == ring_end ? ring : islot + SLOT;
        ++is;
        ++issued;
        if (is == iT) next_unit(claim_ok);
    };
    next_unit(false);

    const int f0 = 64 * wave + lane;
    const int fm = (f0 >= nr ? 1 : 0) + (f0 >= 2 * nr ? 1 : 0) + (f0 >= 3 * nr ? 1 : 0);
    const float *fres = fm == 0 ? s0 : fm == 1 ? s1 : fm == 2 ? s2 : s3;
    const int frow = row_of(f0 - fm * nr);
    uint32_t rv = 0;

    if (FUSEDQ) {
        rv = gload4_asm(fres && f0 < nflat && frow < N ? fres + frow : x);
        if (ki < 0) {
            const uint8_t *xb = (const uint8_t *)x + 16 * lane;
#pragma unroll
            for (int i = 0; i < NI; ++i)
                if (i + 1 == NI) dma16_nt_lanes(xb, (LDS void *)(islot + 1024 * i), lane, GRAN - 64 * (NI - 1));
                else dma16_nt(xb, (LDS void *)(islot + 1024 * i));
        } else {
            const uint8_t *base = is16 + 16 * lane;
            const uint8_t *lim = iT > 1 ? base + 1024 * (NI - 1) : base + 1024 * (NI - 1) < il16 ? base + 1024 * (NI - 1) : il16;
#pragma unroll
            for (int i = 0; i + 1 < NI; ++i) {
                const uint8_t *p = base + 1024 * i;
                dma16_nt(iT > 1 || p < il16 ? p : il16, (LDS void *)(islot + 1024 * i));
            }
            dma16_nt_lanes(lim, (LDS void *)(islot + 1024 * (NI - 1)), lane, GRAN - 64 * (NI - 1));
            islot = islot + SLOT == ring_end ? ring : islot + SLOT;
            ++is;
            ++issued;
            if (is == iT) next_unit(false);
        }
        vm_wait<NI + 1>();
        if (RSTAMPS(h)) sx = __builtin_amdgcn_s_memrealtime();
        asm volatile("" : "+v"(xv[0][0]), "+v"(xv[0][1]), "+v"(xv[0][2]), "+v"(xv[0][3]), "+v"(xv[1][0]),
                     "+v"(xv[1][1]), "+v"(xv[1][2]), "+v"(xv[1][3]), "+v"(xv[2][0]), "+v"(xv[2][1]),
                     "+v"(xv[2][2]), "+v"(xv[2][3]));
        if (PRO != ROWS_PRO_NONE) {
#pragma unroll
            for (int i = 0; i < ROWS_QPASS; ++i)
#pragma unroll
                for (int k = 0; k < 4; ++k) asm volatile("" : "+v"(x2v[i][k]));
        }
        if (PRO == ROWS_PRO_SWIGLU) {
#pragma unroll
            for (int i = 0; i < ROWS_QPASS; ++i)
                if (i < qw)
#pragma unroll
                    for (int k = 0; k < 4; ++k) xv[i][k] = swiglu4(xv[i][k], x2v[i][k]);
        } else if (PRO == ROWS_PRO_NORM) {
            double *sums = (double *)(smem + L.sums);
#pragma unroll
            for (int i = 0; i < ROWS_QPASS; ++i) {
                if (i < qw) {
                    const int j = PASS * i + 4 * wave + (lane >> 4);
                    double sq = 0.0;
                    if (j < nb) {
                        float v[16];
#pragma unroll
                        for (int k = 0; k < 4; ++k) {
                            v[4 * k] = __uint_as_float(xv[i][k].x), v[4 * k + 1] = __uint_as_float(xv[i][k].y);
                            v[4 * k + 2] = __uint_as_float(xv[i][k].z), v[4 * k + 3] = __uint_as_float(xv[i][k].w);
                        }
                        sq = sumsq16(v);
                    }
                    sq = row16_sum(sq);
                    if (j < nb && (lane & 15) == 0) sums[j] = sq;
                }
            }
            asm volatile("s_waitcnt lgkmcnt(0)\n\ts_barrier" ::: "memory");
            double tot = seq_sum_lanes(sums, nb, lane);
            if (rms_mean_ambiguous(div_by_count(tot, (int64_t)nb * QK), (int64_t)nb * QK))
                tot = seq_sumsq_wave(x, (int64_t)nb * QK, lane);
            const float mean = (float)div_by_count(tot, (int64_t)nb * QK);
            const float scale = 1.0f / sqrtf(mean + h.eps);
#pragma unroll
            for (int i = 0; i < ROWS_QPASS; ++i)
                if (i < qw)
#pragma unroll
                    for (int k = 0; k < 4; ++k) xv[i][k] = normmul4(xv[i][k], x2v[i][k], scale);
        }
#pragma unroll 1
        for (int i = 0; i < qw; ++i) {
            u32x4 cur[4];
#pragma unroll
            for (int k = 0; k < 4; ++k) cur[k] = i == 0 ? xv[0][k] : i == 1 ? xv[1][k] : xv[2][k];
            const int j = PASS * i + 4 * wave + (lane >> 4);
            if (j < nb) quant16_store(cur, lane & 15, smem + L.act + Q8L_STRIDE * j);
        }
        if (RSTAMPS(h)) {
            asm volatile("s_waitcnt lgkmcnt(0)" ::: "memory");
            sq = __builtin_amdgcn_s_memrealtime();
        }
    } else {
        const int ng = nb * (Q8L_STRIDE / 16);
        for (int j = wave; 64 * j < ng; j += nwv) {
            const int k = 64 * j + lane;
            if (k < ng) dma16((const uint8_t *)ld.x + 16 * k, (LDS void *)(smem + L.act + 1024 * j));
        }
        rv = gload4_asm(fres && f0 < nflat && frow < N ? fres + frow : (const float *)ld.x);
        if (!idone && !iwait && ki >= 0) issue(false);
        vm_wait_k<NI>(issued);
    }
    while (!idone && !iwait && ki >= 0 && issued < D) issue(false);
    if (wave == 0 && lane == 0) *cnt = (uint32_t)(nwv * P);
    asm volatile("s_waitcnt lgkmcnt(0)\n\ts_barrier" ::: "memory");
    if (iwait) next_unit(true);
    while (!idone && ki >= 0 && issued < D) issue(true);
    const uint64_t st1 = RSTAMPS(h) ? __builtin_amdgcn_s_memrealtime() : 0;

    int kc = 0, cs = 0, cT = 0, cG = 0, cmis = 0, crows = 0, io = 0, rr = 0;
    int bro = 0;
    uint32_t bfl = 0;
    auto consume_unit = [&](int k) {
        const uint32_t gr = (uint32_t)__builtin_amdgcn_readlane((int)ug, k & 7);
        const int flat = __builtin_amdgcn_readlane((int)uf, k & 7);
        cG = (int)(gr & 0xffffu);
        crows = (int)(gr >> 16);
        cT = (cG + ROWS_SB - 1) / ROWS_SB;
        cmis = (int)((uint32_t)__builtin_amdgcn_readlane((int)ul, k & 7) & 15u);
        bfl = lane >= bro && lane < bro + crows ? (uint32_t)(flat + lane - bro) : bfl;
        cs = 0;
        io = q;
        rr = bro;
        while (io >= nb) {
            io -= nb;
            ++rr;
        }
    };
    auto replay = [&]() {
        wave_lds_fence();
        if (lane < bro) {
            float v = 0.f;
            const Rec *rc = recs + lane;
#pragma unroll 4
            for (int i = 0; i < nb; ++i) v = chain_step(TYPE, rc[i * bR], v);
            outs[bfl] = v;
        }
        wave_lds_fence();
        bro = 0;
    };
    int consumed = 0;
    if (issued > 0) consume_unit(0);
    const uint8_t *cslot = ring;
#pragma unroll 1
    while (consumed < issued) {
        vm_wait_k<NI>(issued - consumed - 1);
        if (ROWS_SB * cs + q < cG) {
            const uint8_t *blk = cslot + cmis + q * BSZ;
            const uint8_t *ab = actq + io * Q8L_STRIDE;
            QuadOut r = TYPE == Q4_K ? quad_q4K(blk, ab, s) : TYPE == Q5_K ? quad_q5K(blk, ab, s) : quad_q6K(blk, ab, s);
            const int isum = quad_sum(r.isum);
            const int imin = quad_sum(r.imin);
            if (s == 0) {
                const float yd = *(const float *)ab;
                Rec rec;
                if (TYPE == Q6_K) {
                    rec.a = isum - 32 * imin;
                    rec.b = 0;
                    rec.c = h2f(r.dh) * yd;
                    rec.e = 0.f;
                } else {
                    rec.a = isum;
                    rec.b = imin;
                    rec.c = yd * h2f(r.dh & 0xffffu);
                    rec.e = yd * h2f(r.dh >> 16);
                }
                recs[io * bR + rr] = rec;
            }
        }
        cslot = cslot + SLOT == ring_end ? ring : cslot + SLOT;
        ++consumed;
        ++cs;
        if (!idone) issue(true);
        if (RSTAMPS(h) && consumed == 1) sf = __builtin_amdgcn_s_memrealtime();
        if (cs == cT) {
            bro += crows;
            if (bro + U > bR || consumed == issued) replay();
            ++kc;
            if (consumed < issued) consume_unit(kc);
        } else {
            io += ROWS_SB;
            while (io >= nb) {
                io -= nb;
                ++rr;
            }
        }
    }

    const uint64_t st2 = RSTAMPS(h) ? __builtin_amdgcn_s_memrealtime() : 0;
    asm volatile("s_waitcnt vmcnt(0)" ::: "memory");
    asm volatile("" : "+v"(rv));
    asm volatile("s_waitcnt lgkmcnt(0)\n\ts_barrier" ::: "memory");
    for (int f = f0; f < nflat; f += 64 * nwv) {
        const int m = (f >= nr ? 1 : 0) + (f >= 2 * nr ? 1 : 0) + (f >= 3 * nr ? 1 : 0);
        const int row = f == f0 ? frow : row_of(f - m * nr);
        if (row >= N) continue;
        const float *res = m == 0 ? s0 : m == 1 ? s1 : m == 2 ? s2 : s3;
        float *y = m == 0 ? y0 : m == 1 ? y1 : m == 2 ? y2 : y3;
        float v = outs[f];
        if (res) v = v + (f == f0 ? __uint_as_float(rv) : res[row]);
        store_y(y + row, v);
    }
    if (h.epi) {
        const int n4 = h.epi_n & ~3;
        for (int f = f0; f < nr; f += 64 * nwv) {
            const int r = row_of(f);
            if (r >= N) continue;
            const float gv = outs[f], uv = outs[nr + f];
            store_y(h.epi_y + r, r < n4 ? v_silu(gv) * uv : (gv / (1.0f + expf(-gv))) * uv);
        }
    }
    if (RSTAMPS(h)) {
        const int64_t o = ((int64_t)blockIdx.x * ROWS_WAVES + wave) * 8;
        if (lane == 0 && o + 7 < h.stamps_cap) {
            RSTAMPS(h)[o] = st0;
            RSTAMPS(h)[o + 1] = st1;
            RSTAMPS(h)[o + 2] = st2;
            RSTAMPS(h)[o + 3] = __builtin_amdgcn_s_memrealtime();
            RSTAMPS(h)[o + 4] = sx;
            RSTAMPS(h)[o + 5] = sq;
            RSTAMPS(h)[o + 6] = sf;
            RSTAMPS(h)[o + 7] = (uint64_t)(ki + 1);
        }
    }
}
template <int TMASK, bool FUSEDQ, int PRO>
__global__ void __launch_bounds__(ROWS_WAVES * 64) kq_rows_dyn(KQ_ROWS_PARAMS) {
    extern __shared__ __attribute__((aligned(16))) uint8_t smem[];
    const RowsLead ld = rows_lead(x, x2, w0, res0, nb, waves_total, grid, cfg, rbase0, rrem0);
    const uint64_t st0 = RSTAMP();
    const int lane = threadIdx.x & 63;
    const int wave = __builtin_amdgcn_readfirstlane(threadIdx.x >> 6);
    constexpr int TYPE = TMASK == 1 ? Q4_K : TMASK == 2 ? Q5_K : Q6_K;
    rows_dyn_body<TYPE, FUSEDQ, PRO, TMASK>(a, ld, smem, wave, lane, st0);
}

#define KQ_ROWS_DYN_INST(TM, FQ, PR) template __global__ void kq_rows_dyn<TM, FQ, PR>(KQ_ROWS_PARAMS);
#define KQ_ROWS_DYN_INST_T(TM)        \
    KQ_ROWS_DYN_INST(TM, true, 0)     \
    KQ_ROWS_DYN_INST(TM, true, 1)     \
    KQ_ROWS_DYN_INST(TM, true, 2)     \
    KQ_ROWS_DYN_INST(TM, false, 0)
KQ_ROWS_DYN_INST_T(1)
KQ_ROWS_DYN_INST_T(2)
KQ_ROWS_DYN_INST_T(4)

}
```

ggml-neon-opt_amd/csrc/kq_rows_device.h:

```cpp
#pragma once

#include "kq_device.h"
#include "kq_ops_device.h"

namespace kq {

template <typename Op>
__device__ __forceinline__ int row16_reduce(int v, Op op) {
    v = op(v, __builtin_amdgcn_update_dpp(v, v, 0xB1, 0xF, 0xF, false));
    v = op(v, __builtin_amdgcn_update_dpp(v, v, 0x4E, 0xF, 0xF, false));
    v = op(v, __builtin_amdgcn_update_dpp(v, v, 0x141, 0xF, 0xF, false));
    v = op(v, __builtin_amdgcn_update_dpp(v, v, 0x140, 0xF, 0xF, false));
    return v;
}

__device__ __forceinline__ uint32_t qbyte(float iscale, float x) {
    int q = nearest_int_fused(iscale, x);
    q = q < 127 ? q : 127;
    return (uint32_t)q & 0xffu;
}

template <bool AM = false>
__device__ __forceinline__ void quant16_store(const u32x4 v[4], int l, uint8_t *qb) {
    float x[16];
#pragma unroll
    for (int k = 0; k < 4; ++k) {
        x[4 * k + 0] = __uint_as_float(v[k].x);
        x[4 * k + 1] = __uint_as_float(v[k].y);
        x[4 * k + 2] = __uint_as_float(v[k].z);
        x[4 * k + 3] = __uint_as_float(v[k].w);
    }
    float mp = 0.f, mn = 0.f;
#pragma unroll
    for (int k = 0; k < 16; ++k) {
        mp = fmaxf(mp, x[k]);
        mn = fmaxf(mn, -x[k]);
    }
    const int mpb = row16_reduce(__float_as_int(mp), [](int a, int c) { return a > c ? a : c; });
    const int mnb = row16_reduce(__float_as_int(mn), [](int a, int c) { return a > c ? a : c; });
    const float m = __int_as_float(mpb > mnb ? mpb : mnb);
    bool neg = mnb > mpb;
    if (mpb == mnb && mpb != 0) {
        uint32_t key = 0xffffffffu;
#pragma unroll
        for (int k = 15; k >= 0; --k)
            if (fabsf(x[k]) == m) key = 2u * (uint32_t)(16 * l + k) + (x[k] < 0.f ? 1u : 0u);
        key = (uint32_t)row16_reduce((int)key, [](int a, int c) { return (uint32_t)a < (uint32_t)c ? a : c; });
        neg = (key & 1u) != 0;
    }
    const float maxv = neg ? -m : m;
    const float iscale = -127.f / maxv;
    u32x4 q;
    q.x = qbyte(iscale, x[0]) | (qbyte(iscale, x[1]) << 8) | (qbyte(iscale, x[2]) << 16) | (qbyte(iscale, x[3]) << 24);
    q.y = qbyte(iscale, x[4]) | (qbyte(iscale, x[5]) << 8) | (qbyte(iscale, x[6]) << 16) | (qbyte(iscale, x[7]) << 24);
    q.z = qbyte(iscale, x[8]) | (qbyte(iscale, x[9]) << 8) | (qbyte(iscale, x[10]) << 16) |
          (qbyte(iscale, x[11]) << 24);
    q.w = qbyte(iscale, x[12]) | (qbyte(iscale, x[13]) << 8) | (qbyte(iscale, x[14]) << 16) |
          (qbyte(iscale, x[15]) << 24);
    int bsum = sdot4(q.x, 0x01010101u, 0);
    bsum = sdot4(q.y, 0x01010101u, bsum);
    bsum = sdot4(q.z, 0x01010101u, bsum);
    bsum = sdot4(q.w, 0x01010101u, bsum);
    float d = 1.f / iscale;
    if (m == 0.f) {
        q = u32x4{0u, 0u, 0u, 0u};
        bsum = 0;
        d = 0.f;
    }
    *(u32x4 *)(qb + 16 + 16 * l) = q;
    if (AM) {
        const int bs = bsum + __builtin_amdgcn_update_dpp(bsum, bsum, 0xB1, 0xF, 0xF, false);
        if (!(l & 1)) {
            *(_Float16 *)(qb + 272 + l) = (_Float16)(bs & 63);
            *(_Float16 *)(qb + 288 + l) = (_Float16)(bs >> 6);
        }
    } else {
        *(int16_t *)(qb + 272 + 2 * l) = (int16_t)bsum;
    }
    if (l == 0) *(float *)qb = d;
}

__device__ __forceinline__ uint32_t gload4_asm(const float *p) {
    uint32_t r;
    asm volatile("global_load_dword %0, %1, off" : "=v"(r) : "v"(p) : "memory");
    return r;
}

__device__ __forceinline__ u32x4 swiglu4(u32x4 g, u32x4 u) {
    u32x4 r;
    r.x = __float_as_uint(v_silu(__uint_as_float(g.x)) * __uint_as_float(u.x));
    r.y = __float_as_uint(v_silu(__uint_as_float(g.y)) * __uint_as_float(u.y));
    r.z = __float_as_uint(v_silu(__uint_as_float(g.z)) * __uint_as_float(u.z));
    r.w = __float_as_uint(v_silu(__uint_as_float(g.w)) * __uint_as_float(u.w));
    return r;
}

__device__ __forceinline__ u32x4 normmul4(u32x4 x, u32x4 w, float scale) {
    u32x4 r;
    r.x = __float_as_uint((__uint_as_float(x.x) * scale) * __uint_as_float(w.x));
    r.y = __float_as_uint((__uint_as_float(x.y) * scale) * __uint_as_float(w.y));
    r.z = __float_as_uint((__uint_as_float(x.z) * scale) * __uint_as_float(w.z));
    r.w = __float_as_uint((__uint_as_float(x.w) * scale) * __uint_as_float(w.w));
    return r;
}

__device__ __forceinline__ u32x4 gload16_asm(const float *p) {
    u32x4 r;
    asm volatile("global_load_dwordx4 %0, %1, off" : "=v"(r) : "v"(p) : "memory");
    return r;
}

__device__ __forceinline__ int dotacc(u32x4 q, u32x4 a, int acc) {
    acc = sdot4(q.x, a.x, acc);
    acc = sdot4(q.y, a.y, acc);
    acc = sdot4(q.z, a.z, acc);
    return sdot4(q.w, a.w, acc);
}

struct QuadOut {
    int isum, imin;
    uint32_t dh;
};

__device__ __forceinline__ QuadOut quad_q4K(const uint8_t *blk, const uint8_t *ab, int s) {
    const u32x4 hdr = *(const u32x4 *)blk;
    const u32x4 q0 = *(const u32x4 *)(blk + 16 + 32 * s);
    const u32x4 q1 = *(const u32x4 *)(blk + 32 + 32 * s);
    const uint8_t *aq = ab + 16 + 64 * s;
    const u32x4 a0 = *(const u32x4 *)(aq), a1 = *(const u32x4 *)(aq + 16);
    const u32x4 a2 = *(const u32x4 *)(aq + 32), a3 = *(const u32x4 *)(aq + 48);
    const ScMn s0 = scales_k4(hdr, 2 * s), s1 = scales_k4(hdr, 2 * s + 1);
    const int dlo = dotacc(q1 & 0x0f0f0f0fu, a1, dotacc(q0 & 0x0f0f0f0fu, a0, 0));
    const int dhi = dotacc((q1 >> 4) & 0x0f0f0f0fu, a3, dotacc((q0 >> 4) & 0x0f0f0f0fu, a2, 0));
    const uint2 bs = *(const uint2 *)(ab + 272 + 8 * s);
    QuadOut r;
    r.isum = __mul24(dlo, s0.sc_lo) + __mul24(dhi, s0.sc_hi);
    r.imin = ((int)(int16_t)(bs.x & 0xffffu) + (int)(int16_t)(bs.x >> 16)) * s0.mn +
             ((int)(int16_t)(bs.y & 0xffffu) + (int)(int16_t)(bs.y >> 16)) * s1.mn;
    r.dh = hdr.x;
    return r;
}

__device__ __forceinline__ QuadOut quad_q5K(const uint8_t *blk, const uint8_t *ab, int s) {
    const u32x4 hdr = *(const u32x4 *)blk;
    const u32x4 h0 = *(const u32x4 *)(blk + 16), h1 = *(const u32x4 *)(blk + 32);
    const u32x4 q0 = *(const u32x4 *)(blk + 48 + 32 * s);
    const u32x4 q1 = *(const u32x4 *)(blk + 64 + 32 * s);
    const uint8_t *aq = ab + 16 + 64 * s;
    const u32x4 a0 = *(const u32x4 *)(aq), a1 = *(const u32x4 *)(aq + 16);
    const u32x4 a2 = *(const u32x4 *)(aq + 32), a3 = *(const u32x4 *)(aq + 48);
    const ScMn s0 = scales_k4(hdr, 2 * s), s1 = scales_k4(hdr, 2 * s + 1);
    const uint32_t sl = (uint32_t)(2 * s), shh = (uint32_t)(2 * s + 1);
    const u32x4 lo0 = (q0 & 0x0f0f0f0fu) | (((h0 >> sl) & 0x01010101u) << 4);
    const u32x4 hi0 = ((q0 >> 4) & 0x0f0f0f0fu) | (((h0 >> shh) & 0x01010101u) << 4);
    const u32x4 lo1 = (q1 & 0x0f0f0f0fu) | (((h1 >> sl) & 0x01010101u) << 4);
    const u32x4 hi1 = ((q1 >> 4) & 0x0f0f0f0fu) | (((h1 >> shh) & 0x01010101u) << 4);
    const int dlo = dotacc(lo1, a1, dotacc(lo0, a0, 0));
    const int dhi = dotacc(hi1, a3, dotacc(hi0, a2, 0));
    const uint2 bs = *(const uint2 *)(ab + 272 + 8 * s);
    QuadOut r;
    r.isum = __mul24(dlo, s0.sc_lo) + __mul24(dhi, s0.sc_hi);
    r.imin = ((int)(int16_t)(bs.x & 0xffffu) + (int)(int16_t)(bs.x >> 16)) * s0.mn +
             ((int)(int16_t)(bs.y & 0xffffu) + (int)(int16_t)(bs.y >> 16)) * s1.mn;
    r.dh = hdr.x;
    return r;
}

__device__ __forceinline__ QuadOut quad_q6K(const uint8_t *blk, const uint8_t *ab, int s) {
    const uint32_t s4 = (uint32_t)((uintptr_t)blk & 3u);
    const uint8_t *b = blk - s4;
    const int n = s >> 1, part2 = s & 1;
    const u32x4 L0 = realign(*(const u32x4a *)(b + 32 * s), *(const uint32_t *)(b + 32 * s + 16), s4);
    const u32x4 L1 = realign(*(const u32x4a *)(b + 32 * s + 16), *(const uint32_t *)(b + 32 * s + 32), s4);
    const u32x4 H0 = realign(*(const u32x4a *)(b + 128 + 32 * n), *(const uint32_t *)(b + 144 + 32 * n), s4);
    const u32x4 H1 = realign(*(const u32x4a *)(b + 144 + 32 * n), *(const uint32_t *)(b + 160 + 32 * n), s4);
    const uint32_t w208 = *(const uint32_t *)(b + 208);
    const u32x4 SC = realign(*(const u32x4a *)(b + 192), w208, s4);
    const uint32_t shl = (uint32_t)part2 * 2u;
    const u32x4 ql0 = (L0 & 0x0f0f0f0fu) | (((H0 >> shl) & 0x03030303u) << 4);
    const u32x4 qh0 = ((L0 >> 4) & 0x0f0f0f0fu) | (((H0 >> (shl + 4u)) & 0x03030303u) << 4);
    const u32x4 ql1 = (L1 & 0x0f0f0f0fu) | (((H1 >> shl) & 0x03030303u) << 4);
    const u32x4 qh1 = ((L1 >> 4) & 0x0f0f0f0fu) | (((H1 >> (shl + 4u)) & 0x03030303u) << 4);
    const int elo = 128 * n + 32 * part2;
    const uint8_t *aq = ab + 16 + elo;
    const int sb = elo >> 4;
    const int d00 = dotacc(ql0, *(const u32x4 *)(aq), 0);
    const int d01 = dotacc(qh0, *(const u32x4 *)(aq + 64), 0);
    const int d10 = dotacc(ql1, *(const u32x4 *)(aq + 16), 0);
    const int d11 = dotacc(qh1, *(const u32x4 *)(aq + 80), 0);
    QuadOut r;
    r.isum = __mul24(d00, sbyte(SC, sb)) + __mul24(d01, sbyte(SC, sb + 4)) + __mul24(d10, sbyte(SC, sb + 1)) +
             __mul24(d11, sbyte(SC, sb + 5));
// ... 54 lines not shown
```

ggml-neon-opt_amd/ggml_mi355x/__init__.py:

```python
from __future__ import annotations

import ctypes
import os

HERE = os.path.dirname(os.path.abspath(__file__))
PKG_ROOT = os.path.dirname(HERE)
LIB_PATH = os.environ.get("MI355X_LIB") or os.path.join(PKG_ROOT, "lib", "libggml_mi355x.so")

TYPE_F32, TYPE_F16, TYPE_Q4_K, TYPE_Q5_K, TYPE_Q6_K, TYPE_Q8_K, TYPE_I32 = 0, 1, 12, 13, 14, 15, 26
TYPE_I64 = 27
QK_K = 256
BLOCK_BYTES = {TYPE_Q4_K: 144, TYPE_Q5_K: 176, TYPE_Q6_K: 210, TYPE_Q8_K: 292}
TYPE_NAMES = {TYPE_Q4_K: "q4_K", TYPE_Q5_K: "q5_K", TYPE_Q6_K: "q6_K", TYPE_Q8_K: "q8_K", TYPE_F32: "f32"}
MAX_FUSED = 4
OP_NONE, OP_MUL_MAT, OP_GET_ROWS, OP_RMS_NORM, OP_MUL, OP_ADD, OP_SWIGLU, OP_ROPE, OP_ATTN_DECODE, OP_ALL_GATHER, \
    OP_ALL_REDUCE = range(11)
OP_ATTN_BATCH = 11
MAX_SRC = 10
FLAG_OUTPUT = 1
E_OK, E_INVAL, E_UNSUPPORTED, E_WORKSPACE, E_NODEVICE, E_COMM, E_LAYER = 0, -1, -2, -3, -4, -6, -7
PRO_NONE, PRO_RMS_NORM, PRO_SWIGLU = 0, 1, 2
EPI_NONE, EPI_SWIGLU = 0, 1
ATTN_GROUP, ATTN_HEAD, ATTN_SPLIT = 0, 1, 2
ATTN_PATH_HEAD, ATTN_PATH_HEAD_BATCH, ATTN_PATH_SPLIT4, ATTN_PATH_SPLIT8, ATTN_PATH_CELLS, ATTN_PATH_GROUP, ATTN_PATH_KD1 = range(7)
MMQ_AUTO, MMQ_TILE64, MMQ_TILE128, MMQ_TILE128W, MMQ_TILE64W, MMQ_TILE128X, MMQ_TILE192 = 0, 1, 2, 3, 4, 5, 6
PREFILL_EXACT, PREFILL_F16, PREFILL_F16_ALL = 0, 1, 2

EXPORTED_SYMBOLS = (
    "mi355x_row_size", "mi355x_version", "mi355x_device_available",
    "mi355x_quantize_row_q8_K", "mi355x_vec_dot_q4_K_q8_K", "mi355x_vec_dot_q5_K_q8_K",
    "mi355x_vec_dot_q6_K_q8_K", "mi355x_quantize_q8_K", "mi355x_mul_mat_workspace_size",
    "mi355x_mul_mat", "mi355x_mul_mat_q8", "mi355x_gemv_fused", "mi355x_debug_block_partials", "mi355x_debug_stream",
    "mi355x_backend_init", "mi355x_backend_free", "mi355x_backend_name", "mi355x_backend_stream",
    "mi355x_backend_alloc", "mi355x_backend_free_buffer", "mi355x_backend_set_tensor",
    "mi355x_backend_get_tensor", "mi355x_backend_synchronize", "mi355x_backend_supports_op",
    "mi355x_backend_graph_compute", "mi355x_timing_enable", "mi355x_timing_read", "mi355x_diag_stamps",
    "mi355x_gemv_fused_workspace_size", "mi355x_gemv_impl",
    "mi355x_gguf_open", "mi355x_gguf_close", "mi355x_gguf_version", "mi355x_gguf_alignment",
    "mi355x_gguf_data_offset", "mi355x_gguf_n_tensors", "mi355x_gguf_find_tensor", "mi355x_gguf_get_tensor",
    "mi355x_gguf_tensor_data", "mi355x_gguf_upload", "mi355x_gguf_n_kv", "mi355x_gguf_find_key",
    "mi355x_gguf_key", "mi355x_gguf_kv_type", "mi355x_gguf_get_int", "mi355x_gguf_get_float",
    "mi355x_gguf_get_str", "mi355x_gguf_arr_n",
    "mi355x_gemv_ext_workspace_size", "mi355x_gemv_fused_ext", "mi355x_backend_set_fusion",
    "mi355x_get_rows", "mi355x_rms_norm", "mi355x_add", "mi355x_mul", "mi355x_swiglu",
    "mi355x_rope_table_size", "mi355x_rope_table", "mi355x_rope", "mi355x_attn_decode", "mi355x_attn_path",
    "mi355x_comm_id_size", "mi355x_comm_get_unique_id", "mi355x_backend_set_comm", "mi355x_backend_comm_world",
    "mi355x_backend_set_comm_loopback", "mi355x_lower_ggml_graph", "mi355x_attn_impl",
    "mi355x_mmq_impl",
    "mi355x_prefill_precision",
    "mi355x_gemv_waves",
    "mi355x_debug_knob",
    "mi355x_device_count", "mi355x_device_ordinal", "mi355x_device_memory", "mi355x_backend_memset", "mi355x_backend_set_attn_oproj",
    "mi355x_backend_set_layer_engine", "mi355x_backend_layer_error",
    "mi355x_attn_prompt",
    "mi355x_attn_prompt_impl",
    "mi355x_attn_batch", "mi355x_attn_batch_path",
)


class Mi355xError(RuntimeError):
    pass


class GemvDesc(ctypes.Structure):
    _fields_ = [("type", ctypes.c_int), ("w", ctypes.c_void_p), ("n_rows", ctypes.c_int64),
                ("row_stride", ctypes.c_size_t), ("y", ctypes.c_void_p)]


class LaunchTiming(ctypes.Structure):
    _fields_ = [("kernel", ctypes.c_char * 96), ("bytes", ctypes.c_double), ("ms", ctypes.c_float)]


class Tensor(ctypes.Structure):
    pass


Tensor._fields_ = [("type", ctypes.c_int), ("op", ctypes.c_int), ("ne", ctypes.c_int64 * 4),
                   ("nb", ctypes.c_size_t * 4), ("src", ctypes.POINTER(Tensor) * MAX_SRC), ("data", ctypes.c_void_p),
                   ("op_params", ctypes.c_int32 * 8), ("flags", ctypes.c_int32)]


class GTensor(ctypes.Structure):
    pass


GTensor._fields_ = [("type", ctypes.c_int), ("op", ctypes.c_int), ("ne", ctypes.c_int64 * 4),
                    ("nb", ctypes.c_size_t * 4), ("op_params", ctypes.c_int32 * 16), ("flags", ctypes.c_int32),
                    ("src", ctypes.POINTER(GTensor) * 10), ("view_src", ctypes.POINTER(GTensor)),
                    ("view_offs", ctypes.c_size_t), ("data", ctypes.c_void_p), ("name", ctypes.c_char * 64)]


class LowerOpts(ctypes.Structure):
    _fields_ = [("rope_table", ctypes.c_void_p), ("rope_n_pos", ctypes.c_int), ("rope_freq_base", ctypes.c_float),
                ("rope_freq_scale", ctypes.c_float), ("cells_eq_pos", ctypes.c_int),
                ("cells_from_graph", ctypes.c_int)]


(GOP_NONE, GOP_GET_ROWS, GOP_RMS_NORM, GOP_MUL, GOP_ADD, GOP_MUL_MAT, GOP_ROPE, GOP_SET_ROWS, GOP_SOFT_MAX, GOP_GLU,
 GOP_RESHAPE, GOP_VIEW, GOP_PERMUTE, GOP_TRANSPOSE, GOP_CONT, GOP_CPY) = range(16)
GLU_SWIGLU = 2


class AttnDesc(ctypes.Structure):
    _fields_ = [("q", ctypes.c_void_p), ("k", ctypes.c_void_p), ("v", ctypes.c_void_p), ("pos", ctypes.c_void_p),
                ("rope_table", ctypes.c_void_p), ("k_cache", ctypes.c_void_p), ("v_cache", ctypes.c_void_p),
                ("out", ctypes.c_void_p), ("n_ctx", ctypes.c_int), ("n_head", ctypes.c_int),
                ("n_head_kv", ctypes.c_int), ("head_dim", ctypes.c_int), ("scale", ctypes.c_float),
                ("rope_row", ctypes.c_int)]


class AttnBatchDesc(ctypes.Structure):
    _fields_ = [("a", AttnDesc), ("cells", ctypes.c_void_p), ("cells_type", ctypes.c_int), ("mask", ctypes.c_void_p),
                ("mask_type", ctypes.c_int), ("mask_row_bytes", ctypes.c_size_t), ("n_kv", ctypes.c_int),
                ("n_tokens", ctypes.c_int)]


class GemvExt(ctypes.Structure):
    _fields_ = [("prologue", ctypes.c_int), ("x2", ctypes.c_void_p), ("eps", ctypes.c_float),
                ("residual", ctypes.c_void_p * MAX_FUSED), ("epilogue", ctypes.c_int), ("epi_y", ctypes.c_void_p)]

_lib = None


def lib():
    global _lib
    if _lib is not None:
        return _lib
    if not os.path.exists(LIB_PATH):
        raise Mi355xError(f"{LIB_PATH} missing: run __graft_entry__.build() (make -C ggml-neon-opt_amd)")
    L = ctypes.CDLL(LIB_PATH)
    vp, sz, i64, i32 = ctypes.c_void_p, ctypes.c_size_t, ctypes.c_int64, ctypes.c_int
    L.mi355x_row_size.argtypes = [i32, i64]
    L.mi355x_row_size.restype = sz
    L.mi355x_version.restype = ctypes.c_char_p
    L.mi355x_device_available.restype = i32
    L.mi355x_device_count.restype = i32
    L.mi355x_device_ordinal.restype = i32
    L.mi355x_device_ordinal.argtypes = [i32]
    L.mi355x_device_memory.argtypes = [i32, ctypes.POINTER(ctypes.c_size_t), ctypes.POINTER(ctypes.c_size_t)]
    L.mi355x_device_memory.restype = i32
    L.mi355x_backend_memset.argtypes = [ctypes.c_void_p, ctypes.c_void_p, i32, ctypes.c_size_t]
    L.mi355x_backend_memset.restype = i32
    L.mi355x_backend_set_attn_oproj.argtypes = [ctypes.c_void_p, i32]
    L.mi355x_backend_set_attn_oproj.restype = i32
    L.mi355x_backend_set_layer_engine.argtypes = [ctypes.c_void_p, i32]
    L.mi355x_backend_set_layer_engine.restype = i32
    L.mi355x_backend_layer_error.argtypes = [ctypes.c_void_p]
    L.mi355x_backend_layer_error.restype = i32
    L.mi355x_quantize_row_q8_K.argtypes = [vp, vp, i64]
    for n in ("q4_K", "q5_K", "q6_K"):
        getattr(L, f"mi355x_vec_dot_{n}_q8_K").argtypes = [i32, vp, sz, vp, sz, vp, sz, i32]
    L.mi355x_quantize_q8_K.argtypes = [vp, sz, vp, i64, i64, vp]
    L.mi355x_quantize_q8_K.restype = i32
    L.mi355x_mul_mat_workspace_size.argtypes = [i32, i64, i64, i64]
    L.mi355x_mul_mat_workspace_size.restype = sz
    L.mi355x_mul_mat.argtypes = [i32, vp, i64, i64, sz, vp, i64, sz, vp, sz, vp, sz, vp]
    L.mi355x_mul_mat.restype = i32
    L.mi355x_mul_mat_q8.argtypes = [i32, vp, i64, i64, sz, vp, i64, sz, vp, sz, vp]
    L.mi355x_mul_mat_q8.restype = i32
    L.mi355x_gemv_fused.argtypes = [ctypes.POINTER(GemvDesc), i32, vp, i64, vp, sz, vp]
    L.mi355x_gemv_fused_workspace_size.argtypes = [i64]
    L.mi355x_gemv_fused_workspace_size.restype = sz
    L.mi355x_gemv_fused.restype = i32
    L.mi355x_debug_block_partials.argtypes = [i32, vp, i64, i64, sz, vp, vp, vp]
    L.mi355x_debug_block_partials.restype = i32
    L.mi355x_debug_stream.argtypes = [vp, sz, vp, vp]
    L.mi355x_debug_stream.restype = i32
    L.mi355x_backend_init.argtypes = [i32]
    L.mi355x_backend_init.restype = vp
    L.mi355x_backend_free.argtypes = [vp]
    L.mi355x_backend_name.argtypes = [vp]
    L.mi355x_backend_name.restype = ctypes.c_char_p
    L.mi355x_backend_stream.argtypes = [vp]
    L.mi355x_backend_stream.restype = vp
    L.mi355x_backend_alloc.argtypes = [vp, sz]
    L.mi355x_backend_alloc.restype = vp
    L.mi355x_backend_free_buffer.argtypes = [vp, vp]
    L.mi355x_backend_set_tensor.argtypes = [vp, vp, vp, sz]
    L.mi355x_backend_set_tensor.restype = i32
    L.mi355x_backend_get_tensor.argtypes = [vp, vp, vp, sz]
    L.mi355x_backend_get_tensor.restype = i32
    L.mi355x_backend_synchronize.argtypes = [vp]
    L.mi355x_backend_synchronize.restype = i32
    L.mi355x_backend_supports_op.argtypes = [ctypes.POINTER(Tensor)]
    L.mi355x_backend_supports_op.restype = i32
    L.mi355x_backend_graph_compute.argtypes = [vp, ctypes.POINTER(ctypes.POINTER(Tensor)), i32, i32]
    L.mi355x_backend_graph_compute.restype = i32
    L.mi355x_timing_enable.argtypes = [i32]
    L.mi355x_timing_enable.restype = i32
    L.mi355x_timing_read.argtypes = [ctypes.POINTER(LaunchTiming), i32]
    L.mi355x_timing_read.restype = i32
    L.mi355x_gemv_impl.argtypes = [i32]
    L.mi355x_gemv_impl.restype = i32
    L.mi355x_diag_stamps.argtypes = [vp, sz]
    L.mi355x_diag_stamps.restype = i32
    f32 = ctypes.c_float
    L.mi355x_gemv_ext_workspace_size.argtypes = [i64]
    L.mi355x_gemv_ext_workspace_size.restype = sz
    L.mi355x_gemv_fused_ext.argtypes = [ctypes.POINTER(GemvDesc), i32, vp, i64, ctypes.POINTER(GemvExt), vp, sz, vp]
    L.mi355x_gemv_fused_ext.restype = i32
    L.mi355x_backend_set_fusion.argtypes = [vp, i32]
    L.mi355x_backend_set_fusion.restype = i32
    L.mi355x_get_rows.argtypes = [i32, vp, i64, sz, i64, vp, i64, vp, vp]
    L.mi355x_rms_norm.argtypes = [vp, vp, vp, i64, i64, f32, vp]
    L.mi355x_add.argtypes = [vp, vp, vp, i64, vp]
    L.mi355x_mul.argtypes = [vp, vp, vp, i64, vp]
    L.mi355x_swiglu.argtypes = [vp, vp, vp, i64, vp]
    L.mi355x_rope_table_size.argtypes = [i32, i32]
    L.mi355x_rope_table_size.restype = sz
    L.mi355x_rope_table.argtypes = [vp, i32, i32, f32, f32, vp]
    L.mi355x_rope.argtypes = [vp, vp, i32, i32, i32, vp, vp, i32, vp]
    L.mi355x_attn_decode.argtypes = [ctypes.POINTER(AttnDesc), vp]
    L.mi355x_attn_path.argtypes = [ctypes.POINTER(AttnDesc)]
    L.mi355x_attn_path.restype = i32
    L.mi355x_attn_prompt.argtypes = [ctypes.POINTER(AttnDesc), i32, vp]
    L.mi355x_attn_batch.argtypes = [ctypes.POINTER(AttnBatchDesc), vp]
    L.mi355x_attn_batch.restype = i32
    L.mi355x_attn_batch_path.argtypes = [ctypes.POINTER(AttnBatchDesc)]
    L.mi355x_attn_batch_path.restype = i32
    L.mi355x_attn_prompt_impl.argtypes = [i32]
    L.mi355x_attn_prompt_impl.restype = i32
    L.mi355x_attn_impl.argtypes = [i32]
    L.mi355x_attn_impl.restype = i32
    L.mi355x_mmq_impl.argtypes = [i32]
    L.mi355x_mmq_impl.restype = i32
    L.mi355x_prefill_precision.argtypes = [i32]
    L.mi355x_prefill_precision.restype = i32
    L.mi355x_gemv_waves.argtypes = [i32]
    L.mi355x_gemv_waves.restype = i32
    L.mi355x_debug_knob.argtypes = [ctypes.c_char_p, ctypes.c_double, ctypes.POINTER(ctypes.c_double)]
    L.mi355x_debug_knob.restype = i32
    for n in ("mi355x_get_rows", "mi355x_rms_norm", "mi355x_add", "mi355x_mul", "mi355x_swiglu",
              "mi355x_rope_table", "mi355x_rope", "mi355x_attn_decode", "mi355x_attn_prompt"):
        getattr(L, n).restype = i32
    L.mi355x_lower_ggml_graph.argtypes = [ctypes.POINTER(ctypes.POINTER(GTensor)), i32, ctypes.POINTER(LowerOpts),
                                          ctypes.POINTER(Tensor), i32, ctypes.POINTER(ctypes.POINTER(Tensor)), i32,
                                          ctypes.POINTER(i32)]
    L.mi355x_lower_ggml_graph.restype = i32
    L.mi355x_comm_id_size.argtypes = []
    L.mi355x_comm_id_size.restype = sz
    L.mi355x_comm_get_unique_id.argtypes = [vp]
    L.mi355x_comm_get_unique_id.restype = i32
    L.mi355x_backend_set_comm.argtypes = [vp, i32, i32, vp]
    L.mi355x_backend_set_comm.restype = i32
    L.mi355x_backend_comm_world.argtypes = [vp]
    L.mi355x_backend_comm_world.restype = i32
    L.mi355x_backend_set_comm_loopback.argtypes = [vp, i32, i32]
    L.mi355x_backend_set_comm_loopback.restype = i32
    from . import gguf as _gguf
    _gguf.bind(L)
# ... 68 lines not shown
        x = x[None]
    assert x.dtype == torch.float32 and x.is_cuda and x.stride(1) == 1
    M, K = x.shape
    if out is None:
        out = torch.empty((M, K // QK_K * 292), dtype=torch.uint8, device=x.device)
    _check(lib().mi355x_quantize_q8_K(x.data_ptr(), x.stride(0) * 4, out.data_ptr(), K, M, _stream(stream)),
           "mi355x_quantize_q8_K")
    return out


def mul_mat(type_, w, K, x, out=None, workspace=None, stream=None):
    torch = _torch()
    _require_device()
    if x.dim() == 1:
        x = x[None]
    M = x.shape[0]
    N = w.shape[0]
    if out is None:
        out = torch.empty((M, N), dtype=torch.float32, device=x.device)
    ws = int(lib().mi355x_mul_mat_workspace_size(type_, K, N, M))
    if M == 1 and x.data_ptr() % 16:
        ws = max(ws, K // QK_K * 304)
    if ws and (workspace is None or workspace.numel() < ws):
        workspace = _workspace(ws, x.device, stream)
    _check(lib().mi355x_mul_mat(type_, w.data_ptr(), K, N, w.stride(0), x.data_ptr(), M, x.stride(0) * 4,
                                out.data_ptr(), out.stride(0) * 4,
                                workspace.data_ptr() if ws else None, ws, _stream(stream)), "mi355x_mul_mat")
    return out


def mul_mat_q8(type_, w, K, q8, out=None, stream=None):
    torch = _torch()
    _require_device()
    if q8.dim() == 1:
        q8 = q8[None]
    M = q8.shape[0]
    N = w.shape[0]
    if out is None:
        out = torch.empty((M, N), dtype=torch.float32, device=q8.device)
    _check(lib().mi355x_mul_mat_q8(type_, w.data_ptr(), K, N, w.stride(0), q8.data_ptr(), M, q8.stride(0),
                                   out.data_ptr(), out.stride(0) * 4, _stream(stream)), "mi355x_mul_mat_q8")
    return out


_ws_cache = {}


def _workspace(nbytes, device, stream=None):
    torch = _torch()
    key = (str(device), _stream(stream).value or 0)
    buf = _ws_cache.get(key)
    if buf is None or buf.numel() < nbytes:
        buf = torch.empty(max(nbytes, 1), dtype=torch.uint8, device=device)
        _ws_cache[key] = buf
    return buf


def gemv_fused(mats, x, stream=None, workspace=None):
    _require_device()
    n = len(mats)
    descs = (GemvDesc * n)()
    for i, (t, w, y) in enumerate(mats):
        descs[i] = GemvDesc(t, w.data_ptr(), w.shape[0], w.stride(0), y.data_ptr())
    K = x.shape[-1]
    need = int(lib().mi355x_gemv_fused_workspace_size(K))
    if need and (workspace is None or workspace.numel() < need):
        workspace = _workspace(need, x.device, stream)
    _check(lib().mi355x_gemv_fused(descs, n, x.data_ptr(), K, workspace.data_ptr() if need else None, need,
                                   _stream(stream)), "mi355x_gemv_fused")


def mmq_impl(impl):
    return int(lib().mi355x_mmq_impl(impl))


def prefill_precision(p=-1):
    return int(lib().mi355x_prefill_precision(p))


def gemv_waves(waves):
    return int(lib().mi355x_gemv_waves(waves))


DEBUG_KNOBS = ("GEMV_DIAG", "GEMV_RING", "GEMV_PRE0", "GEMV_PF", "GEMV_XMODE", "GEMV_SMALL_MB", "GEMV_WPC",
               "GEMV_SMALL_WG", "GEMV_FQMAX", "MMF_WAVES", "MMF_ORDER", "ATTN_DIAG", "LOOPBACK_NOCOPY",
               "ATTN_OPROJ", "AO_NRB", "GEMV_DYN", "GEMV_DYN_P", "GEMV_DYN_STEPS")


def debug_knob(name, value=float("nan")):
    prev = ctypes.c_double(0.0)
    rc = lib().mi355x_debug_knob(name.encode(), float(value), ctypes.byref(prev))
    if rc != 0:
        raise Mi355xError(f"debug_knob: unknown knob {name!r}")
    return prev.value


def attn_prompt_impl(impl):
    return int(lib().mi355x_attn_prompt_impl(impl))


def attn_impl(impl):
    return int(lib().mi355x_attn_impl(impl))


def gemv_fused_ext(mats, x, prologue=PRO_NONE, x2=None, eps=0.0, residual=None, epi_y=None, stream=None):
    _require_device()
    n = len(mats)
    descs = (GemvDesc * n)()
    for i, (t, w, y) in enumerate(mats):
        descs[i] = GemvDesc(t, w.data_ptr(), w.shape[0], w.stride(0), y.data_ptr())
    ext = GemvExt()
    ext.prologue = prologue
    ext.x2 = x2.data_ptr() if x2 is not None else None
    ext.eps = eps
    for i in range(MAX_FUSED):
        r = residual[i] if residual is not None and i < len(residual) else None
        ext.residual[i] = r.data_ptr() if r is not None else None
    ext.epilogue = EPI_SWIGLU if epi_y is not None else EPI_NONE
    ext.epi_y = epi_y.data_ptr() if epi_y is not None else None
    K = x.shape[-1]
    need = int(lib().mi355x_gemv_ext_workspace_size(K))
    ws = _workspace(need, x.device, stream)
    _check(lib().mi355x_gemv_fused_ext(descs, n, x.data_ptr(), K, ctypes.byref(ext), ws.data_ptr(), need,
                                       _stream(stream)), "mi355x_gemv_fused_ext")


def get_rows(type_, table, K, ids, out=None, stream=None):
    torch = _torch()
    _require_device()
    n = ids.numel()
    if out is None:
        out = torch.empty((n, K), dtype=torch.float32, device=ids.device)
    _check(lib().mi355x_get_rows(type_, table.data_ptr(), K, table.stride(0) * table.element_size(), table.shape[0],
                                 ids.data_ptr(), n, out.data_ptr(), _stream(stream)), "mi355x_get_rows")
    return out


def rms_norm(x, eps, w=None, out=None, stream=None):
    torch = _torch()
    _require_device()
    x2 = x if x.dim() == 2 else x[None]
    if out is None:
        out = torch.empty_like(x)
    _check(lib().mi355x_rms_norm(x.data_ptr(), w.data_ptr() if w is not None else None, out.data_ptr(),
                                 x2.shape[1], x2.shape[0], eps, _stream(stream)), "mi355x_rms_norm")
    return out


def add(a, b, out=None, stream=None):
    out = _torch().empty_like(a) if out is None else out
    _check(lib().mi355x_add(a.data_ptr(), b.data_ptr(), out.data_ptr(), a.numel(), _stream(stream)), "mi355x_add")
    return out


def mul(a, b, out=None, stream=None):
    out = _torch().empty_like(a) if out is None else out
    _check(lib().mi355x_mul(a.data_ptr(), b.data_ptr(), out.data_ptr(), a.numel(), _stream(stream)), "mi355x_mul")
    return out


def swiglu(g, u, out=None, stream=None):
    out = _torch().empty_like(g) if out is None else out
    _check(lib().mi355x_swiglu(g.data_ptr(), u.data_ptr(), out.data_ptr(), g.numel(), _stream(stream)),
           "mi355x_swiglu")
    return out

# ... 234 lines not shown
```

include/ggml_mi355x.h:

```cpp
#ifndef GGML_MI355X_H
#define GGML_MI355X_H

#include <stddef.h>
#include <stdint.h>

#ifdef __cplusplus
extern "C" {
#endif

#define MI355X_QK_K 256
#define MI355X_K_SCALE_SIZE 12

typedef uint16_t mi355x_half;

typedef struct {
    mi355x_half d;
    mi355x_half dmin;
    uint8_t scales[MI355X_K_SCALE_SIZE];
    uint8_t qs[MI355X_QK_K / 2];
} mi355x_block_q4_K;

typedef struct {
    mi355x_half d;
    mi355x_half dmin;
// ... 15 lines not shown
    int16_t bsums[MI355X_QK_K / 16];
} mi355x_block_q8_K;

enum mi355x_type {
    MI355X_TYPE_F32  = 0,
    MI355X_TYPE_F16  = 1,
    MI355X_TYPE_Q4_K = 12,
    MI355X_TYPE_Q5_K = 13,
    MI355X_TYPE_Q6_K = 14,
    MI355X_TYPE_Q8_K = 15,
    MI355X_TYPE_I32  = 26,
    MI355X_TYPE_I64  = 27,
};

enum mi355x_status {
    MI355X_OK           = 0,
    MI355X_E_INVAL      = -1,
    MI355X_E_UNSUPPORTED = -2,
    MI355X_E_WORKSPACE  = -3,
    MI355X_E_NODEVICE   = -4,
    MI355X_E_COMM       = -6,
    MI355X_E_LAYER      = -7,
};

size_t mi355x_row_size(int type, int64_t k);

const char *mi355x_version(void);
int mi355x_device_available(void);

void mi355x_quantize_row_q8_K(const float *x, void *y, int64_t k);

void mi355x_vec_dot_q4_K_q8_K(int n, float *s, size_t bs, const void *vx, size_t bx,
                              const void *vy, size_t by, int nrc);
void mi355x_vec_dot_q5_K_q8_K(int n, float *s, size_t bs, const void *vx, size_t bx,
                              const void *vy, size_t by, int nrc);
void mi355x_vec_dot_q6_K_q8_K(int n, float *s, size_t bs, const void *vx, size_t bx,
                              const void *vy, size_t by, int nrc);

int mi355x_quantize_q8_K(const float *x, size_t x_stride, void *y, int64_t k, int64_t nrows,
                         void *stream);

size_t mi355x_mul_mat_workspace_size(int src0_type, int64_t ne00, int64_t ne01, int64_t ne11);
int mi355x_mul_mat(int src0_type, const void *src0, int64_t ne00, int64_t ne01, size_t nb01,
                   const float *src1, int64_t ne11, size_t nb11,
                   float *dst, size_t nb1,
                   void *workspace, size_t workspace_size, void *stream);

int mi355x_mul_mat_q8(int src0_type, const void *src0, int64_t ne00, int64_t ne01, size_t nb01,
                      const void *src1_q8, int64_t ne11, size_t nb11,
                      float *dst, size_t nb1, void *stream);

#define MI355X_MAX_FUSED 4
typedef struct {
    int type;
    const void *w;
    int64_t n_rows;
    size_t row_stride;
    float *y;
} mi355x_gemv_desc;
size_t mi355x_gemv_fused_workspace_size(int64_t k);
int mi355x_gemv_fused(const mi355x_gemv_desc *descs, int n_desc, const float *x, int64_t k,
                      void *workspace, size_t workspace_size, void *stream);

#define MI355X_PRO_NONE 0
#define MI355X_PRO_RMS_NORM 1
#define MI355X_PRO_SWIGLU 2
#define MI355X_EPI_NONE 0
#define MI355X_EPI_SWIGLU 1
typedef struct {
    int prologue;
    const float *x2;
    float eps;
    const float *residual[MI355X_MAX_FUSED];
    int epilogue;
    float *epi_y;
} mi355x_gemv_ext;
size_t mi355x_gemv_ext_workspace_size(int64_t k);
int mi355x_gemv_fused_ext(const mi355x_gemv_desc *descs, int n_desc, const float *x, int64_t k,
                          const mi355x_gemv_ext *ext, void *workspace, size_t workspace_size, void *stream);

int mi355x_debug_stream(const void *buf, size_t bytes, void *sink, void *stream);
int mi355x_debug_block_partials(int src0_type, const void *src0, int64_t ne00, int64_t ne01,
                                size_t nb01, const void *src1_q8, int32_t *out, void *stream);

typedef struct {
    char kernel[96];
    double bytes;
    float ms;
} mi355x_launch_timing;
int mi355x_timing_enable(int enable);
int mi355x_timing_read(mi355x_launch_timing *out, int max);
int mi355x_diag_stamps(void *buf, size_t bytes);
#define MI355X_GEMV_AUTO 0
#define MI355X_GEMV_TASKS 1
#define MI355X_GEMV_ROWS 2
#define MI355X_GEMV_DYN 3
int mi355x_gemv_impl(int impl);
#define MI355X_MMQ_AUTO 0
#define MI355X_MMQ_TILE64 1
#define MI355X_MMQ_TILE128 2
#define MI355X_MMQ_TILE128W 3
#define MI355X_MMQ_TILE64W 4
#define MI355X_MMQ_TILE128X 5
#define MI355X_MMQ_TILE192 6
int mi355x_mmq_impl(int impl);
#define MI355X_PREFILL_EXACT 0
#define MI355X_PREFILL_F16 1
#define MI355X_PREFILL_F16_ALL 2
int mi355x_prefill_precision(int precision);
int mi355x_gemv_waves(int waves);
int mi355x_debug_knob(const char *name, double value, double *previous);


int mi355x_get_rows(int type, const void *table, int64_t ne0, size_t row_stride, int64_t n_rows,
                    const int32_t *ids, int64_t n_ids, float *dst, void *stream);
int mi355x_rms_norm(const float *x, const float *w, float *y, int64_t n, int64_t nrows, float eps, void *stream);
int mi355x_add(const float *a, const float *b, float *y, int64_t n, void *stream);
int mi355x_mul(const float *a, const float *b, float *y, int64_t n, void *stream);
int mi355x_swiglu(const float *gate, const float *up, float *y, int64_t n, void *stream);
size_t mi355x_rope_table_size(int n_pos, int n_dims);
int mi355x_rope_table(float *table, int n_pos, int n_dims, float freq_base, float freq_scale, void *stream);
int mi355x_rope(const float *x, float *y, int head_dim, int n_dims, int n_heads, const int32_t *pos,
                const float *table, int n_pos, void *stream);
typedef struct {
    const float *q, *k, *v;
    const int32_t *pos;
    const float *rope_table;
    uint16_t *k_cache;
    uint16_t *v_cache;
    float *out;
    int n_ctx, n_head, n_head_kv, head_dim;
    float scale;
    int rope_row;
} mi355x_attn_desc;
int mi355x_attn_decode(const mi355x_attn_desc *a, void *stream);
#define MI355X_ATTN_PATH_HEAD 0
#define MI355X_ATTN_PATH_HEAD_BATCH 1
#define MI355X_ATTN_PATH_SPLIT4 2
#define MI355X_ATTN_PATH_SPLIT8 3
#define MI355X_ATTN_PATH_CELLS 4
#define MI355X_ATTN_PATH_GROUP 5
#define MI355X_ATTN_PATH_KD1 6
int mi355x_attn_path(const mi355x_attn_desc *a);
int mi355x_attn_prompt(const mi355x_attn_desc *a, int n_tokens, void *stream);
#define MI355X_ATTN_GROUP 0
#define MI355X_ATTN_HEAD 1
#define MI355X_ATTN_SPLIT 2
int mi355x_attn_impl(int impl);
int mi355x_attn_prompt_impl(int impl);
typedef struct {
    mi355x_attn_desc a;
    const void *cells; int cells_type;
    const void *mask;  int mask_type; size_t mask_row_bytes;
    int n_kv, n_tokens;
} mi355x_attn_batch_desc;
int mi355x_attn_batch(const mi355x_attn_batch_desc *d, void *stream);
int mi355x_attn_batch_path(const mi355x_attn_batch_desc *d);

enum mi355x_op {
    MI355X_OP_NONE = 0, MI355X_OP_MUL_MAT = 1, MI355X_OP_GET_ROWS = 2, MI355X_OP_RMS_NORM = 3,
    MI355X_OP_MUL = 4, MI355X_OP_ADD = 5, MI355X_OP_SWIGLU = 6, MI355X_OP_ROPE = 7,
    MI355X_OP_ATTN_DECODE = 8, MI355X_OP_ALL_GATHER = 9, MI355X_OP_ALL_REDUCE = 10,
    MI355X_OP_ATTN_BATCH = 11,
};
#define MI355X_MAX_SRC 10
#define MI355X_TENSOR_FLAG_OUTPUT 1
// ... 118 lines not shown
```

Measured before the change: 1379 tok/s.

## Add wide-lane fused activation prologue for rows GEMV when few row steps

Adds a templated prologue form (LSH) in the fused-quantize rows GEMV kernels that spreads each 256-element superblock over 32 or 64 lanes, so the activation load, norm/swiglu and q8 quantization finish in a single pass instead of several 16-lane passes. The wide form is picked only when the per-wave row step count is small and the K dimension fits in the waves, which is the small-matrix decode case. New cross-lane reductions use permlane16/32 swaps. It also adds a debug entry point and a plan query for testing. The cost is three times as many kernel instantiations and extra cross-lane reduction work per superblock.

New measurement: 1438 tok/s, median of 6. 1.04x the previous value.

```diff
diff --git a/ggml-neon-opt_amd/csrc/kq_api.hip b/ggml-neon-opt_amd/csrc/kq_api.hip
--- a/ggml-neon-opt_amd/csrc/kq_api.hip
+++ b/ggml-neon-opt_amd/csrc/kq_api.hip
@@ -18,9 +18,9 @@
 template <int NCOL, bool FUSEDQ, bool DEBUG, int TMASK>
 __global__ void kq_gemv(const GemvArgs a);
 __global__ void kq_quantize_q8K(const float *x, int64_t x_stride, uint8_t *y, int nb, int64_t nblocks);
-template <int TMASK, bool FUSEDQ, int PRO>
+template <int TMASK, bool FUSEDQ, int PRO, int LSH>
 __global__ void kq_rows(KQ_ROWS_PARAMS);
-template <int TMASK, bool FUSEDQ, int PRO>
+template <int TMASK, bool FUSEDQ, int PRO, int LSH>
 __global__ void kq_rows_dyn(KQ_ROWS_PARAMS);
 template <bool AM>
 __global__ void kq_quantize_q8L(const float *x, int64_t x_stride, uint8_t *y, int nb, int64_t nblocks);
@@ -334,28 +334,33 @@
 }
 
 
-template <int TM, bool FQ, int PR>
+template <int TM, bool FQ, int PR, int LS>
 rows_fn rows_inst(bool dyn) {
     if constexpr (TM == 7) {
-        return kq_rows<TM, FQ, PR>;
+        return kq_rows<TM, FQ, PR, LS>;
     } else {
-        return dyn ? kq_rows_dyn<TM, FQ, PR> : kq_rows<TM, FQ, PR>;
-    }
+        return dyn ? kq_rows_dyn<TM, FQ, PR, LS> : kq_rows<TM, FQ, PR, LS>;
+    }
+}
+
+template <int TM, int PR>
+rows_fn rows_pick_form(int lsh, bool dyn) {
+    return lsh == 2 ? rows_inst<TM, true, PR, 2>(dyn) : lsh == 1 ? rows_inst<TM, true, PR, 1>(dyn) : rows_inst<TM, true, PR, 0>(dyn);
 }
 
 template <int TM>
-rows_fn rows_pick_pro(bool fusedq, int pro, bool dyn) {
-    if (!fusedq) return rows_inst<TM, false, 0>(dyn);
-    return pro == ROWS_PRO_NORM ? rows_inst<TM, true, 1>(dyn) : pro == ROWS_PRO_SWIGLU ? rows_inst<TM, true, 2>(dyn)
-                                                                                       : rows_inst<TM, true, 0>(dyn);
-}
-
-rows_fn pick_rows(int tmask, bool fusedq, int pro, bool dyn = false) {
+rows_fn rows_pick_pro(bool fusedq, int pro, bool dyn, int lsh) {
+    if (!fusedq) return rows_inst<TM, false, 0, 0>(dyn);
+    return pro == ROWS_PRO_NORM ? rows_pick_form<TM, 1>(lsh, dyn) : pro == ROWS_PRO_SWIGLU ? rows_pick_form<TM, 2>(lsh, dyn)
+                                                                                         : rows_pick_form<TM, 0>(lsh, dyn);
+}
+
+rows_fn pick_rows(int tmask, bool fusedq, int pro, bool dyn, int lsh) {
     switch (tmask) {
-        case 1: return rows_pick_pro<1>(fusedq, pro, dyn);
-        case 2: return rows_pick_pro<2>(fusedq, pro, dyn);
-        case 4: return rows_pick_pro<4>(fusedq, pro, dyn);
-        default: return rows_pick_pro<7>(fusedq, pro, false);
+        case 1: return rows_pick_pro<1>(fusedq, pro, dyn, lsh);
+        case 2: return rows_pick_pro<2>(fusedq, pro, dyn, lsh);
+        case 4: return rows_pick_pro<4>(fusedq, pro, dyn, lsh);
+        default: return rows_pick_pro<7>(fusedq, pro, false, lsh);
     }
 }
 
@@ -385,7 +390,6 @@
     if (tmask != 1 && tmask != 2 && tmask != 4) tmask = 7;
     pl.tmask = tmask;
     pl.fusedq = fusedq;
-    pl.fn = pick_rows(tmask, fusedq, ROWS_PRO_NONE);
     a.n_desc = n_desc;
     a.nb = (int)nb;
     for (int i = 0; i < n_desc; ++i) {
@@ -459,6 +463,8 @@
         }
     if (rpw > 0x7fffffff / 64) return MI355X_E_UNSUPPORTED;
     a.rpw = (int)(rpw > 0 ? rpw : 1);
+    pl.lsh = fusedq ? rows_pro_form((int)nb, pl.nwv, (rpw * nb + ROWS_SB - 1) / ROWS_SB).lsh : 0;
+    pl.fn = pick_rows(tmask, fusedq, ROWS_PRO_NONE, false, pl.lsh);
     int g16 = ROWS_SB;
     while (nb % g16) g16 >>= 1;
     const int u = ROWS_SB / g16;
@@ -503,7 +509,7 @@
             a.rpw = (int)flat;
             pl.lds = (size_t)DL.total;
             pl.grid = dim3((unsigned)n_wg, 1, 1);
-            pl.fn = pick_rows(tmask, fusedq, ROWS_PRO_NONE, true);
+            pl.fn = pick_rows(tmask, fusedq, ROWS_PRO_NONE, true, pl.lsh);
         }
     }
     return MI355X_OK;
@@ -529,8 +535,8 @@
     if (a.waves_total == 0) return MI355X_OK;
     allow_lds((const void *)pl.fn, pl.lds);
     const void *x = pl.fusedq ? (const void *)a.x : (const void *)a.xq;
-    const int pass = 4 * pl.nwv;
-    const int qiters = pl.fusedq ? (a.nb + pass - 1) / pass : 0;
+    const int qiters = !pl.fusedq ? 0 : pl.lsh ? 1 : (a.nb + 4 * pl.nwv - 1) / (4 * pl.nwv);
+    if (pl.lsh < 0 || pl.lsh > 2 || (pl.lsh && (!pl.fusedq || a.nb * (16 << pl.lsh) > 64 * pl.nwv))) return MI355X_E_INVAL;
     if (pl.nwv < 1 || pl.nwv > ROWS_WAVES || qiters > ROWS_QPASS || a.n_desc < 1 || a.n_desc > MI355X_MAX_FUSED)
         return MI355X_E_INVAL;
     const int cfg = rows_cfg(pl.nwv, qiters, a.n_desc, a.diag & 0x1ff);
@@ -951,7 +957,7 @@
                                                                 : ROWS_PRO_NONE;
                 rp.a.x2 = ext->x2;
                 rp.a.eps = ext->eps;
-                rp.fn = pick_rows(rp.tmask, true, rp.a.pro, rp.dyn);
+                rp.fn = pick_rows(rp.tmask, true, rp.a.pro, rp.dyn, rp.lsh);
                 for (int i = 0; i < n; ++i) {
                     rp.a.res[i] = ext->residual[i];
                     rp.a.n_rows[i] = (int)d[i].n_rows;
@@ -1271,6 +1277,32 @@
     return e == hipSuccess ? MI355X_OK : (int)e;
 }
 
+int mi355x_rows_prologue_plan(int64_t k, int waves, int64_t steps, int *lanes, int *passes) {
+    if (k <= 0 || k % QK || waves < 1 || waves > ROWS_WAVES || steps < 0) return MI355X_E_INVAL;
+    const int64_t nb = k / QK;
+    if (nb > kRowsFusedMaxNb) return MI355X_E_UNSUPPORTED;
+    const RowsProForm f = rows_pro_form((int)nb, waves, steps);
+    if (f.passes > ROWS_QPASS) return MI355X_E_UNSUPPORTED;
+    if (lanes) *lanes = 16 << f.lsh;
+    if (passes) *passes = f.passes;
+    return MI355X_OK;
+}
+
+int mi355x_debug_rows_prologue(int prologue, const float *x, const float *x2, float eps, int64_t k, int waves, void *out,
+                               size_t out_bytes, void *stream) {
+    if (!x || !out || ((uintptr_t)x & 15u) || ((uintptr_t)out & 15u)) return MI355X_E_INVAL;
+    if (prologue < MI355X_PRO_NONE || prologue > MI355X_PRO_SWIGLU) return MI355X_E_INVAL;
+    if (prologue != MI355X_PRO_NONE && (!x2 || ((uintptr_t)x2 & 15u))) return MI355X_E_INVAL;
+    if (prologue == MI355X_PRO_RMS_NORM && !(eps >= 0.0f)) return MI355X_E_INVAL;
+    const int rc = mi355x_rows_prologue_plan(k, waves, 0, nullptr, nullptr);
+    if (rc) return rc;
+    const int64_t nb = k / QK;
+    if (out_bytes < (size_t)nb * Q8L_STRIDE) return MI355X_E_INVAL;
+    if (!device_ok()) return MI355X_E_NODEVICE;
+    const int pro = prologue == MI355X_PRO_RMS_NORM ? ROWS_PRO_NORM : prologue == MI355X_PRO_SWIGLU ? ROWS_PRO_SWIGLU : ROWS_PRO_NONE;
+    return launch_rows_prologue_dbg(pro, x, x2, eps, (int)nb, waves, (uint8_t *)out, (hipStream_t)stream);
+}
+
 int mi355x_debug_block_partials(int src0_type, const void *src0, int64_t ne00, int64_t ne01, size_t nb01,
                                 const void *src1_q8, int32_t *out, void *stream) {
     if (!out || !src1_q8 || ((uintptr_t)src1_q8 & 3u)) return MI355X_E_INVAL;
diff --git a/ggml-neon-opt_amd/csrc/kq_common.h b/ggml-neon-opt_amd/csrc/kq_common.h
--- a/ggml-neon-opt_amd/csrc/kq_common.h
+++ b/ggml-neon-opt_amd/csrc/kq_common.h
@@ -86,6 +86,19 @@
         int cfg, int rbase0, int rrem0, const RowsArgs a
 __host__ __device__ constexpr int rows_cfg(int nwv, int qiters, int n_desc, int diag) {
     return nwv | (qiters << 8) | (n_desc << 12) | (diag << 16);
+}
+constexpr int ROWS_PRO_WIDE_STEPS = 2;
+struct RowsProForm {
+    int lsh, passes;
+};
+#ifndef KQ_ROWS_PRO_WIDE
+#define KQ_ROWS_PRO_WIDE 1
+#endif
+__host__ __device__ constexpr RowsProForm rows_pro_form(int nb, int nwv, int64_t steps = 0) {
+    const bool wide = KQ_ROWS_PRO_WIDE && steps <= ROWS_PRO_WIDE_STEPS;
+    return wide && nb * 64 <= 64 * nwv   ? RowsProForm{2, 1}
+           : wide && nb * 32 <= 64 * nwv ? RowsProForm{1, 1}
+                                         : RowsProForm{0, (nb + 4 * nwv - 1) / (4 * nwv)};
 }
 
 struct RowsArgs {
diff --git a/ggml-neon-opt_amd/csrc/kq_internal.h b/ggml-neon-opt_amd/csrc/kq_internal.h
--- a/ggml-neon-opt_amd/csrc/kq_internal.h
+++ b/ggml-neon-opt_amd/csrc/kq_internal.h
@@ -32,11 +32,14 @@
     int tmask;
     bool fusedq;
     int nwv;
+    int lsh = 0;
     bool dyn = false;
 };
 int plan_rows(const mi355x_gemv_desc *d, int n_desc, int64_t K, bool fusedq, RowsPlan &pl,
               int waves_per_cu = 0);
 int launch_rows(const RowsPlan &pl, hipStream_t stream);
+int launch_rows_prologue_dbg(int pro, const float *x, const float *x2, float eps, int nb, int waves, uint8_t *out,
+                             hipStream_t s);
 bool rows_enabled();
 int launch_quantize(const float *x, int64_t x_stride_floats, void *y, int64_t k, int64_t nrows,
                     hipStream_t stream);
diff --git a/ggml-neon-opt_amd/csrc/kq_rows.hip b/ggml-neon-opt_amd/csrc/kq_rows.hip
--- a/ggml-neon-opt_amd/csrc/kq_rows.hip
+++ b/ggml-neon-opt_amd/csrc/kq_rows.hip
@@ -298,7 +298,201 @@
     return h;
 }
 
-template <int TYPE, bool FUSEDQ, int PRO, int TMASK, class Resolve>
+template <int LSH>
+struct RowsPrologue {
+    static constexpr int NP = LSH ? 1 : ROWS_QPASS;
+    static constexpr int NL = 4 >> LSH;
+    static constexpr int LP = 16 << LSH;
+    static constexpr int SPW = 4 >> LSH;
+    u32x4 xv[NP][NL];
+    u32x4 x2v[NP][NL];
+    int qw = 0;
+    int nb, pass, rot, wave, lane;
+
+    __device__ __forceinline__ int slot(int i) const { return pass * i + SPW * wave + (lane >> (4 + LSH)); }
+    __device__ __forceinline__ int sl() const { return lane & (LP - 1); }
+    __device__ __forceinline__ int sbk(int j) const {
+        const int b = (j < nb ? j : nb - 1) + rot;
+        return b >= nb ? b - nb : b;
+    }
+
+    template <int PRO, bool ASM = true>
+    __device__ __forceinline__ void load(const RowsLead &ld, int wave_, int lane_, int rot_, int diag) {
+        nb = ld.nb, pass = SPW * ld.nwv, rot = rot_, wave = wave_, lane = lane_;
+        const float *const x = (const float *)ld.x;
+        const float *const x2 = (diag & 16) ? x : ld.x2;
+#pragma unroll
+        for (int i = 0; i < NP; ++i) qw += (i < ld.qiters && pass * i + SPW * wave < nb) ? 1 : 0;
+#pragma unroll
+        for (int i = 0; i < NP; ++i)
+#pragma unroll
+            for (int k = 0; k < NL; ++k) {
+                asm volatile("" : "=v"(xv[i][k]));
+                if (PRO != ROWS_PRO_NONE) asm volatile("" : "=v"(x2v[i][k]));
+            }
+#pragma unroll
+        for (int i = 0; i < NP; ++i) {
+            if (i < qw) {
+                const int64_t e = (int64_t)sbk(slot(i)) * QK + (16 >> LSH) * sl();
+#pragma unroll
+                for (int k = 0; k < NL; ++k) {
+                    if (ASM) gload16_into(xv[i][k], x + e + 4 * k);
+                    else xv[i][k] = *(const u32x4 *)(x + e + 4 * k);
+                }
+                if (PRO != ROWS_PRO_NONE) {
+#pragma unroll
+                    for (int k = 0; k < NL; ++k) {
+                        if (ASM) gload16_into(x2v[i][k], x2 + e + 4 * k);
+                        else x2v[i][k] = *(const u32x4 *)(x2 + e + 4 * k);
+                    }
+                }
+            }
+        }
+    }
+
+    template <int PRO>
+    __device__ __forceinline__ void pin() {
+        if constexpr (LSH == 0) {
+            asm volatile("" : "+v"(xv[0][0]), "+v"(xv[0][1]), "+v"(xv[0][2]), "+v"(xv[0][3]), "+v"(xv[1][0]),
+                         "+v"(xv[1][1]), "+v"(xv[1][2]), "+v"(xv[1][3]), "+v"(xv[2][0]), "+v"(xv[2][1]),
+                         "+v"(xv[2][2]), "+v"(xv[2][3]));
+        } else {
+#pragma unroll
+            for (int k = 0; k < NL; ++k) asm volatile("" : "+v"(xv[0][k]));
+        }
+        if (PRO != ROWS_PRO_NONE) {
+#pragma unroll
+            for (int i = 0; i < NP; ++i)
+#pragma unroll
+                for (int k = 0; k < NL; ++k) asm volatile("" : "+v"(x2v[i][k]));
+        }
+    }
+
+    __device__ __forceinline__ void swiglu_pass(int i) {
+#pragma unroll
+        for (int k = 0; k < NL; ++k) xv[i][k] = swiglu4(xv[i][k], x2v[i][k]);
+    }
+
+    __device__ __forceinline__ void values(int i, float v[4 * NL]) const {
+#pragma unroll
+        for (int k = 0; k < NL; ++k) {
+            v[4 * k] = __uint_as_float(xv[i][k].x), v[4 * k + 1] = __uint_as_float(xv[i][k].y);
+            v[4 * k + 2] = __uint_as_float(xv[i][k].z), v[4 * k + 3] = __uint_as_float(xv[i][k].w);
+        }
+    }
+
+    __device__ __forceinline__ void norm(double *sums, const float *x, float eps) {
+#pragma unroll
+        for (int i = 0; i < NP; ++i) {
+            if (i < qw) {
+                const int j = slot(i);
+                double sq = 0.0;
+                if (j < nb) {
+                    float v[4 * NL];
+#pragma unroll
+                    for (int k = 0; k < NL; ++k) {
+                        v[4 * k] = __uint_as_float(xv[i][k].x), v[4 * k + 1] = __uint_as_float(xv[i][k].y);
+                        v[4 * k + 2] = __uint_as_float(xv[i][k].z), v[4 * k + 3] = __uint_as_float(xv[i][k].w);
+                    }
+                    if constexpr (LSH == 0) {
+                        sq = sumsq16(v);
+                    } else {
+#pragma unroll
+                        for (int k = 0; k < 4 * NL; ++k) sq += (double)(v[k] * v[k]);
+                    }
+                }
+                if constexpr (LSH == 0) sq = row16_sum(sq);
+                else sq = sblk_sum<LP>(sq);
+                if (j < nb && sl() == 0) sums[sbk(j)] = sq;
+            }
+        }
+        asm volatile("s_waitcnt lgkmcnt(0)\n\ts_barrier" ::: "memory");
+        double tot = seq_sum_lanes(sums, nb, lane);
+        if (rms_mean_ambiguous(div_by_count(tot, (int64_t)nb * QK), (int64_t)nb * QK))
+            tot = seq_sumsq_wave(x, (int64_t)nb * QK, lane);
+        const float mean = (float)div_by_count(tot, (int64_t)nb * QK);
+        const float scale = 1.0f / sqrtf(mean + eps);
+#pragma unroll
+        for (int i = 0; i < NP; ++i)
+            if (i < qw)
+#pragma unroll
+                for (int k = 0; k < NL; ++k) xv[i][k] = normmul4(xv[i][k], x2v[i][k], scale);
+    }
+
+    __device__ __forceinline__ void quantize_pass(int i, uint8_t *act) {
+        const int j = slot(i);
+        uint8_t *const qb = act + Q8L_STRIDE * sbk(j);
+        if constexpr (LSH == 0) {
+            u32x4 cur[4];
+#pragma unroll
+            for (int k = 0; k < 4; ++k) {
+                const u32x4 p0 = xv[0][k], p1 = xv[1][k], p2 = xv[2][k];
+                cur[k] = i == 0 ? p0 : i == 1 ? p1 : p2;
+            }
+            if (j < nb) quant16_store(cur, lane & 15, qb);
+        } else {
+            float v[4 * NL];
+            values(0, v);
+            quant_wide_store<LP>(v, sl(), qb, j < nb);
+        }
+    }
+
+    template <int PRO>
+    __device__ __forceinline__ void finish(uint8_t *act, double *sums, const float *x, float eps, int diag, bool stamp,
+                                           uint64_t &sx) {
+        pin<PRO>();
+        if (diag & 32) {
+        } else if (PRO == ROWS_PRO_SWIGLU) {
+#pragma unroll
+            for (int i = 0; i < NP; ++i)
+                if (i < qw) swiglu_pass(i);
+        } else if (PRO == ROWS_PRO_NORM) {
+            norm(sums, x, eps);
+        }
+        if (stamp) sx = __builtin_amdgcn_s_memrealtime();
+        if (!(diag & 64)) {
+#pragma unroll 1
+            for (int i = 0; i < qw; ++i) quantize_pass(i, act);
+        }
+    }
+};
+
+template <int PRO, int LSH>
+__global__ void __launch_bounds__(ROWS_WAVES * 64) kq_rows_prologue_dbg(const float *x, const float *x2, int nb, int cfg,
+                                                                        float eps, uint8_t *out) {
+    extern __shared__ __attribute__((aligned(16))) uint8_t smem[];
+    const RowsLead ld = rows_lead(x, x2, nullptr, nullptr, nb, 0, 1, cfg, 0, 0);
+    const int lane = threadIdx.x & 63;
+    const int wave = __builtin_amdgcn_readfirstlane(threadIdx.x >> 6);
+    RowsPrologue<LSH> pg;
+    pg.template load<PRO, false>(ld, wave, lane, 0, 0);
+    uint64_t sx = 0;
+    pg.template finish<PRO>(smem, (double *)(smem + nb * Q8L_STRIDE), x, eps, 0, false, sx);
+    asm volatile("s_waitcnt lgkmcnt(0)\n\ts_barrier" ::: "memory");
+    const int ng = nb * (Q8L_STRIDE / 16);
+    for (int k = threadIdx.x; k < ng; k += ld.nwv * 64) ((u32x4 *)out)[k] = ((const u32x4 *)smem)[k];
+}
+
+template <int PRO>
+static auto rows_prologue_dbg_fn(int lsh) {
+    return lsh == 2 ? kq_rows_prologue_dbg<PRO, 2> : lsh == 1 ? kq_rows_prologue_dbg<PRO, 1> : kq_rows_prologue_dbg<PRO, 0>;
+}
+
+int launch_rows_prologue_dbg(int pro, const float *x, const float *x2, float eps, int nb, int waves, uint8_t *out,
+                             hipStream_t s) {
+    const RowsProForm f = rows_pro_form(nb, waves);
+    const int cfg = rows_cfg(waves, f.passes, 1, 0);
+    const size_t lds = (size_t)nb * Q8L_STRIDE + (size_t)nb * 8;
+    const auto fn = pro == ROWS_PRO_NORM ? rows_prologue_dbg_fn<ROWS_PRO_NORM>(f.lsh)
+                    : pro == ROWS_PRO_SWIGLU ? rows_prologue_dbg_fn<ROWS_PRO_SWIGLU>(f.lsh)
+                                             : rows_prologue_dbg_fn<ROWS_PRO_NONE>(f.lsh);
+    allow_lds((const void *)fn, lds);
+    hipLaunchKernelGGL(fn, dim3(1), dim3(waves * 64), lds, s, x, x2, nb, cfg, eps, out);
+    const hipError_t e = hipGetLastError();
+    return e == hipSuccess ? MI355X_OK : (int)e;
+}
+
+template <int TYPE, bool FUSEDQ, int PRO, int TMASK, int LSH, class Resolve>
 __device__ __forceinline__ void rows_body(const RowsArgs &a, const RowsLead &ld, uint8_t *smem, int wave, int lane,
                                           uint64_t st0, Resolve resolve) {
     constexpr int BSZ = block_bytes(TYPE);
@@ -311,35 +505,9 @@
     const int nwv = ld.nwv;
     const int q = lane >> 2, s = lane & 3;
 
-    const int PASS = 4 * nwv;
     const int xm = !FUSEDQ ? 0 : KQ_ROWS_XMODE >= 0 ? KQ_ROWS_XMODE : a.xmode;
-    u32x4 xv[ROWS_QPASS][4] = {};
-    u32x4 x2v[ROWS_QPASS][4] = {};
-    int qw = 0;
-    const int rot = (xm & ROWS_X_ROT) ? (int)(blockIdx.x % (unsigned)nb) : 0;
-    auto sbk = [&](int j) {
-        int b = (j < nb ? j : nb - 1) + rot;
-        return b >= nb ? b - nb : b;
-    };
-    if (FUSEDQ) {
-        const float *const x = (const float *)ld.x;
-#pragma unroll
-        for (int i = 0; i < ROWS_QPASS; ++i) qw += (i < ld.qiters && PASS * i + 4 * wave < nb) ? 1 : 0;
-#pragma unroll
-        for (int i = 0; i < ROWS_QPASS; ++i) {
-            if (i < qw) {
-                const int b = sbk(PASS * i + 4 * wave + (lane >> 4));
-                const float *xp = x + (int64_t)b * QK + 16 * (lane & 15);
-#pragma unroll
-                for (int k = 0; k < 4; ++k) xv[i][k] = gload16_asm(xp + 4 * k);
-                if (PRO != ROWS_PRO_NONE) {
-                    const float *x2p = ((RDIAG(ld) & 16) ? x : ld.x2) + (int64_t)b * QK + 16 * (lane & 15);
-#pragma unroll
-                    for (int k = 0; k < 4; ++k) x2v[i][k] = gload16_asm(x2p + 4 * k);
-                }
-            }
-        }
-    }
+    RowsPrologue<LSH> pg;
+    if (FUSEDQ) pg.template load<PRO>(ld, wave, lane, (xm & ROWS_X_ROT) ? (int)(blockIdx.x % (unsigned)nb) : 0, RDIAG(ld));
     const RowsHot h = resolve();
     const uint64_t sa = RSTAMP();
     const int bR = h.bR;
@@ -390,7 +558,7 @@
     if (FUSEDQ) {
         const float *const x = (const float *)ld.x;
         constexpr int pro = PRO;
-        constexpr int PL = PRO != ROWS_PRO_NONE ? 8 : 4;
+        constexpr int PL = (PRO != ROWS_PRO_NONE ? 2 : 1) * RowsPrologue<LSH>::NL;
         rv = gload4_asm(res_p && h.nrows > 0 ? res_p + h.r0 + (lane < h.nrows ? lane : 0) : x);
         if (xm & ROWS_X_BAR) asm volatile("s_barrier" ::: "memory");
         constexpr bool kConstPre = KQ_ROWS_PRE0 == 1 && KQ_ROWS_L2PF == 0;
@@ -421,29 +589,14 @@
             for (int i = 0; i < ROWS_PF; ++i) l2_touch(p + 4096 * i < last16 ? p + 4096 * i : last16, pf_sink);
         }
         const int tail = 1 + NI * pre0 + (pf_on ? ROWS_PF : 0);
-        auto pin = [&]() {
-            asm volatile("" : "+v"(xv[0][0]), "+v"(xv[0][1]), "+v"(xv[0][2]), "+v"(xv[0][3]), "+v"(xv[1][0]),
-                         "+v"(xv[1][1]), "+v"(xv[1][2]), "+v"(xv[1][3]), "+v"(xv[2][0]), "+v"(xv[2][1]),
-                         "+v"(xv[2][2]), "+v"(xv[2][3]));
-            if (pro != ROWS_PRO_NONE) {
-#pragma unroll
-                for (int i = 0; i < ROWS_QPASS; ++i)
-#pragma unroll
-                    for (int k = 0; k < 4; ++k) asm volatile("" : "+v"(x2v[i][k]));
-            }
-        };
         if (pro != ROWS_PRO_NORM && (xm & ROWS_X_PIPE)) {
 #pragma unroll
-            for (int i = 0; i < ROWS_QPASS; ++i) {
-                if (i < qw) {
-                    vm_wait_dyn((qw - 1 - i) * PL + tail);
-                    pin();
-                    if (pro == ROWS_PRO_SWIGLU && !(RDIAG(ld) & 32)) {
-#pragma unroll
-                        for (int k = 0; k < 4; ++k) xv[i][k] = swiglu4(xv[i][k], x2v[i][k]);
-                    }
-                    const int j = PASS * i + 4 * wave + (lane >> 4);
-                    if (j < nb && !(RDIAG(ld) & 64)) quant16_store(xv[i], lane & 15, smem + L.act + Q8L_STRIDE * sbk(j));
+            for (int i = 0; i < RowsPrologue<LSH>::NP; ++i) {
+                if (i < pg.qw) {
+                    vm_wait_dyn((pg.qw - 1 - i) * PL + tail);
+                    pg.template pin<PRO>();
+                    if (pro == ROWS_PRO_SWIGLU && !(RDIAG(ld) & 32)) pg.swiglu_pass(i);
+                    if (!(RDIAG(ld) & 64)) pg.quantize_pass(i, smem + L.act);
                 }
             }
             if (RSTAMPS(h)) sx = sq = __builtin_amdgcn_s_memrealtime();
@@ -456,55 +609,7 @@
             } else {
                 vm_wait_dyn(tail);
             }
-            pin();
-            if (RDIAG(ld) & 32) {
-            } else if (pro == ROWS_PRO_SWIGLU) {
-#pragma unroll
-                for (int i = 0; i < ROWS_QPASS; ++i)
-                    if (i < qw)
-#pragma unroll
-                        for (int k = 0; k < 4; ++k) xv[i][k] = swiglu4(xv[i][k], x2v[i][k]);
-            } else if (pro == ROWS_PRO_NORM) {
-                double *sums = (double *)(smem + L.sums);
-#pragma unroll
-                for (int i = 0; i < ROWS_QPASS; ++i) {
-                    if (i < qw) {
-                        const int j = PASS * i + 4 * wave + (lane >> 4);
-                        double sq = 0.0;
-                        if (j < nb) {
-                            float v[16];
-#pragma unroll
-                            for (int k = 0; k < 4; ++k) {
-                                v[4 * k] = __uint_as_float(xv[i][k].x), v[4 * k + 1] = __uint_as_float(xv[i][k].y);
-                                v[4 * k + 2] = __uint_as_float(xv[i][k].z), v[4 * k + 3] = __uint_as_float(xv[i][k].w);
-                            }
-                            sq = sumsq16(v);
-                        }
-                        sq = row16_sum(sq);
-                        if (j < nb && (lane & 15) == 0) sums[sbk(j)] = sq;
-                    }
-                }
-                asm volatile("s_waitcnt lgkmcnt(0)\n\ts_barrier" ::: "memory");
-                double tot = seq_sum_lanes(sums, nb, lane);
-                if (rms_mean_ambiguous(div_by_count(tot, (int64_t)nb * QK), (int64_t)nb * QK))
-                    tot = seq_sumsq_wave(x, (int64_t)nb * QK, lane);
-                const float mean = (float)div_by_count(tot, (int64_t)nb * QK);
-                const float scale = 1.0f / sqrtf(mean + h.eps);
-#pragma unroll
-                for (int i = 0; i < ROWS_QPASS; ++i)
-                    if (i < qw)
-#pragma unroll
-                        for (int k = 0; k < 4; ++k) xv[i][k] = normmul4(xv[i][k], x2v[i][k], scale);
-            }
-            if (RSTAMPS(h)) sx = __builtin_amdgcn_s_memrealtime();
-#pragma unroll 1
-            for (int i = 0; i < qw; ++i) {
-                u32x4 cur[4];
-#pragma unroll
-                for (int k = 0; k < 4; ++k) cur[k] = i == 0 ? xv[0][k] : i == 1 ? xv[1][k] : xv[2][k];
-                const int j = PASS * i + 4 * wave + (lane >> 4);
-                if (j < nb && !(RDIAG(ld) & 64)) quant16_store(cur, lane & 15, smem + L.act + Q8L_STRIDE * sbk(j));
-            }
+            pg.template finish<PRO>(smem + L.act, (double *)(smem + L.sums), x, h.eps, RDIAG(ld), RSTAMPS(h) != nullptr, sx);
             if (RSTAMPS(h)) {
                 asm volatile("s_waitcnt lgkmcnt(0)" ::: "memory");
                 sq = __builtin_amdgcn_s_memrealtime();
@@ -656,7 +761,7 @@
     }
 }
 
-template <int TMASK, bool FUSEDQ, int PRO>
+template <int TMASK, bool FUSEDQ, int PRO, int LSH>
 __global__ void __launch_bounds__(ROWS_WAVES * 64) kq_rows(KQ_ROWS_PARAMS) {
     extern __shared__ __attribute__((aligned(16))) uint8_t smem[];
     const RowsLead ld = rows_lead(x, x2, w0, res0, nb, waves_total, grid, cfg, rbase0, rrem0);
@@ -668,26 +773,23 @@
     auto resolve = [&]() { return rows_resolve<TMASK>(ld, gw); };
 
     if (TMASK == 1) {
-        rows_body<Q4_K, FUSEDQ, PRO, TMASK>(a, ld, smem, wave, lane, st0, resolve);
+        rows_body<Q4_K, FUSEDQ, PRO, TMASK, LSH>(a, ld, smem, wave, lane, st0, resolve);
     } else if (TMASK == 2) {
-        rows_body<Q5_K, FUSEDQ, PRO, TMASK>(a, ld, smem, wave, lane, st0, resolve);
+        rows_body<Q5_K, FUSEDQ, PRO, TMASK, LSH>(a, ld, smem, wave, lane, st0, resolve);
     } else if (TMASK == 4) {
-        rows_body<Q6_K, FUSEDQ, PRO, TMASK>(a, ld, smem, wave, lane, st0, resolve);
+        rows_body<Q6_K, FUSEDQ, PRO, TMASK, LSH>(a, ld, smem, wave, lane, st0, resolve);
     } else {
         const RowsHot h = resolve();
         auto resolved = [&]() { return h; };
-        if (h.type == Q6_K) rows_body<Q6_K, FUSEDQ, PRO, TMASK>(a, ld, smem, wave, lane, st0, resolved);
-        else if (h.type == Q5_K) rows_body<Q5_K, FUSEDQ, PRO, TMASK>(a, ld, smem, wave, lane, st0, resolved);
-        else rows_body<Q4_K, FUSEDQ, PRO, TMASK>(a, ld, smem, wave, lane, st0, resolved);
-    }
-}
-
-#define KQ_ROWS_INST(TM, FQ, PR) template __global__ void kq_rows<TM, FQ, PR>(KQ_ROWS_PARAMS);
-#define KQ_ROWS_INST_T(TM)        \
-    KQ_ROWS_INST(TM, true, 0)     \
-    KQ_ROWS_INST(TM, true, 1)     \
-    KQ_ROWS_INST(TM, true, 2)     \
-    KQ_ROWS_INST(TM, false, 0)
+        if (h.type == Q6_K) rows_body<Q6_K, FUSEDQ, PRO, TMASK, LSH>(a, ld, smem, wave, lane, st0, resolved);
+        else if (h.type == Q5_K) rows_body<Q5_K, FUSEDQ, PRO, TMASK, LSH>(a, ld, smem, wave, lane, st0, resolved);
+        else rows_body<Q4_K, FUSEDQ, PRO, TMASK, LSH>(a, ld, smem, wave, lane, st0, resolved);
+    }
+}
+
+#define KQ_ROWS_INST(TM, FQ, PR, LS) template __global__ void kq_rows<TM, FQ, PR, LS>(KQ_ROWS_PARAMS);
+#define KQ_ROWS_INST_P(TM, PR) KQ_ROWS_INST(TM, true, PR, 0) KQ_ROWS_INST(TM, true, PR, 1) KQ_ROWS_INST(TM, true, PR, 2)
+#define KQ_ROWS_INST_T(TM) KQ_ROWS_INST_P(TM, 0) KQ_ROWS_INST_P(TM, 1) KQ_ROWS_INST_P(TM, 2) KQ_ROWS_INST(TM, false, 0, 0)
 KQ_ROWS_INST_T(1)
 KQ_ROWS_INST_T(2)
 KQ_ROWS_INST_T(4)
@@ -736,7 +838,7 @@
     return h;
 }
 
-template <int TYPE, bool FUSEDQ, int PRO, int TMASK>
+template <int TYPE, bool FUSEDQ, int PRO, int TMASK, int LSH>
 __device__ __forceinline__ void rows_dyn_body(const RowsArgs &a, const RowsLead &ld, uint8_t *smem, int wave, int lane,
                                               uint64_t st0) {
     uint64_t sx = 0, sq = 0, sf = 0;
@@ -752,29 +854,8 @@
     const int q = lane >> 2, s = lane & 3;
 
     const float *const x = (const float *)ld.x;
-    const int PASS = 4 * nwv;
-    u32x4 xv[ROWS_QPASS][4] = {};
-    u32x4 x2v[ROWS_QPASS][4] = {};
-    int qw = 0;
-    if (FUSEDQ) {
-#pragma unroll
-        for (int i = 0; i < ROWS_QPASS; ++i) qw += (i < ld.qiters && PASS * i + 4 * wave < nb) ? 1 : 0;
-#pragma unroll
-        for (int i = 0; i < ROWS_QPASS; ++i) {
-            if (i < qw) {
-                const int j = PASS * i + 4 * wave + (lane >> 4);
-                const int bb = j < nb ? j : nb - 1;
-                const float *xp = x + (int64_t)bb * QK + 16 * (lane & 15);
-#pragma unroll
-                for (int k = 0; k < 4; ++k) xv[i][k] = gload16_asm(xp + 4 * k);
-                if (PRO != ROWS_PRO_NONE) {
-                    const float *x2p = ld.x2 + (int64_t)bb * QK + 16 * (lane & 15);
-#pragma unroll
-                    for (int k = 0; k < 4; ++k) x2v[i][k] = gload16_asm(x2p + 4 * k);
-                }
-            }
-        }
-    }
+    RowsPrologue<LSH> pg;
+    if (FUSEDQ) pg.template load<PRO>(ld, wave, lane, 0, 0);
     const RowsDynHot h = rows_dyn_resolve();
     const uint8_t *const w0 = ld.w0, *const w1 = h.w1, *const w2 = h.w2, *const w3 = h.w3;
     const float *const s0 = ld.res0, *const s1 = h.s1, *const s2 = h.s2, *const s3 = h.s3;
@@ -903,61 +984,8 @@
         }
         vm_wait<NI + 1>();
         if (RSTAMPS(h)) sx = __builtin_amdgcn_s_memrealtime();
-        asm volatile("" : "+v"(xv[0][0]), "+v"(xv[0][1]), "+v"(xv[0][2]), "+v"(xv[0][3]), "+v"(xv[1][0]),
-                     "+v"(xv[1][1]), "+v"(xv[1][2]), "+v"(xv[1][3]), "+v"(xv[2][0]), "+v"(xv[2][1]),
-                     "+v"(xv[2][2]), "+v"(xv[2][3]));
-        if (PRO != ROWS_PRO_NONE) {
-#pragma unroll
-            for (int i = 0; i < ROWS_QPASS; ++i)
-#pragma unroll
-                for (int k = 0; k < 4; ++k) asm volatile("" : "+v"(x2v[i][k]));
-        }
-        if (PRO == ROWS_PRO_SWIGLU) {
-#pragma unroll
-            for (int i = 0; i < ROWS_QPASS; ++i)
-                if (i < qw)
-#pragma unroll
-                    for (int k = 0; k < 4; ++k) xv[i][k] = swiglu4(xv[i][k], x2v[i][k]);
-        } else if (PRO == ROWS_PRO_NORM) {
-            double *sums = (double *)(smem + L.sums);
-#pragma unroll
-            for (int i = 0; i < ROWS_QPASS; ++i) {
-                if (i < qw) {
-                    const int j = PASS * i + 4 * wave + (lane >> 4);
-                    double sq = 0.0;
-                    if (j < nb) {
-                        float v[16];
-#pragma unroll
-                        for (int k = 0; k < 4; ++k) {
-                            v[4 * k] = __uint_as_float(xv[i][k].x), v[4 * k + 1] = __uint_as_float(xv[i][k].y);
-                            v[4 * k + 2] = __uint_as_float(xv[i][k].z), v[4 * k + 3] = __uint_as_float(xv[i][k].w);
-                        }
-                        sq = sumsq16(v);
-                    }
-                    sq = row16_sum(sq);
-                    if (j < nb && (lane & 15) == 0) sums[j] = sq;
-                }
-            }
-            asm volatile("s_waitcnt lgkmcnt(0)\n\ts_barrier" ::: "memory");
-            double tot = seq_sum_lanes(sums, nb, lane);
-            if (rms_mean_ambiguous(div_by_count(tot, (int64_t)nb * QK), (int64_t)nb * QK))
-                tot = seq_sumsq_wave(x, (int64_t)nb * QK, lane);
-            const float mean = (float)div_by_count(tot, (int64_t)nb * QK);
-            const float scale = 1.0f / sqrtf(mean + h.eps);
-#pragma unroll
-            for (int i = 0; i < ROWS_QPASS; ++i)
-                if (i < qw)
-#pragma unroll
-                    for (int k = 0; k < 4; ++k) xv[i][k] = normmul4(xv[i][k], x2v[i][k], scale);
-        }
-#pragma unroll 1
-        for (int i = 0; i < qw; ++i) {
-            u32x4 cur[4];
-#pragma unroll
-            for (int k = 0; k < 4; ++k) cur[k] = i == 0 ? xv[0][k] : i == 1 ? xv[1][k] : xv[2][k];
-            const int j = PASS * i + 4 * wave + (lane >> 4);
-            if (j < nb) quant16_store(cur, lane & 15, smem + L.act + Q8L_STRIDE * j);
-        }
+        uint64_t sxt = 0;
+        pg.template finish<PRO>(smem + L.act, (double *)(smem + L.sums), x, h.eps, 0, false, sxt);
         if (RSTAMPS(h)) {
             asm volatile("s_waitcnt lgkmcnt(0)" ::: "memory");
             sq = __builtin_amdgcn_s_memrealtime();
@@ -1095,7 +1123,7 @@
         }
     }
 }
-template <int TMASK, bool FUSEDQ, int PRO>
+template <int TMASK, bool FUSEDQ, int PRO, int LSH>
 __global__ void __launch_bounds__(ROWS_WAVES * 64) kq_rows_dyn(KQ_ROWS_PARAMS) {
     extern __shared__ __attribute__((aligned(16))) uint8_t smem[];
     const RowsLead ld = rows_lead(x, x2, w0, res0, nb, waves_total, grid, cfg, rbase0, rrem0);
@@ -1103,15 +1131,14 @@
     const int lane = threadIdx.x & 63;
     const int wave = __builtin_amdgcn_readfirstlane(threadIdx.x >> 6);
     constexpr int TYPE = TMASK == 1 ? Q4_K : TMASK == 2 ? Q5_K : Q6_K;
-    rows_dyn_body<TYPE, FUSEDQ, PRO, TMASK>(a, ld, smem, wave, lane, st0);
-}
-
-#define KQ_ROWS_DYN_INST(TM, FQ, PR) template __global__ void kq_rows_dyn<TM, FQ, PR>(KQ_ROWS_PARAMS);
-#define KQ_ROWS_DYN_INST_T(TM)        \
-    KQ_ROWS_DYN_INST(TM, true, 0)     \
-    KQ_ROWS_DYN_INST(TM, true, 1)     \
-    KQ_ROWS_DYN_INST(TM, true, 2)     \
-    KQ_ROWS_DYN_INST(TM, false, 0)
+    rows_dyn_body<TYPE, FUSEDQ, PRO, TMASK, LSH>(a, ld, smem, wave, lane, st0);
+}
+
+#define KQ_ROWS_DYN_INST(TM, FQ, PR, LS) template __global__ void kq_rows_dyn<TM, FQ, PR, LS>(KQ_ROWS_PARAMS);
+#define KQ_ROWS_DYN_INST_P(TM, PR) \
+    KQ_ROWS_DYN_INST(TM, true, PR, 0) KQ_ROWS_DYN_INST(TM, true, PR, 1) KQ_ROWS_DYN_INST(TM, true, PR, 2)
+#define KQ_ROWS_DYN_INST_T(TM) \
+    KQ_ROWS_DYN_INST_P(TM, 0) KQ_ROWS_DYN_INST_P(TM, 1) KQ_ROWS_DYN_INST_P(TM, 2) KQ_ROWS_DYN_INST(TM, false, 0, 0)
 KQ_ROWS_DYN_INST_T(1)
 KQ_ROWS_DYN_INST_T(2)
 KQ_ROWS_DYN_INST_T(4)
diff --git a/ggml-neon-opt_amd/csrc/kq_rows_device.h b/ggml-neon-opt_amd/csrc/kq_rows_device.h
--- a/ggml-neon-opt_amd/csrc/kq_rows_device.h
+++ b/ggml-neon-opt_amd/csrc/kq_rows_device.h
@@ -80,6 +80,90 @@
     if (l == 0) *(float *)qb = d;
 }
 
+__device__ __forceinline__ void swap_rows16(uint32_t v, uint32_t &a, uint32_t &b) {
+    const auto r = __builtin_amdgcn_permlane16_swap(v, v, false, false);
+    a = r[0], b = r[1];
+}
+__device__ __forceinline__ void swap_rows32(uint32_t v, uint32_t &a, uint32_t &b) {
+    const auto r = __builtin_amdgcn_permlane32_swap(v, v, false, false);
+    a = r[0], b = r[1];
+}
+template <int LP, typename Op>
+__device__ __forceinline__ int sblk_reduce(int v, Op op) {
+    static_assert(LP == 32 || LP == 64, "lanes per superblock");
+    v = row16_reduce(v, op);
+    uint32_t a, b;
+    swap_rows16((uint32_t)v, a, b);
+    v = op((int)a, (int)b);
+    if (LP == 64) {
+        swap_rows32((uint32_t)v, a, b);
+        v = op((int)a, (int)b);
+    }
+    return v;
+}
+template <int LP>
+__device__ __forceinline__ double sblk_sum(double v) {
+    static_assert(LP == 32 || LP == 64, "lanes per superblock");
+    v = row16_sum(v);
+#pragma unroll
+    for (int step = 0; step < (LP == 64 ? 2 : 1); ++step) {
+        const uint64_t u = __builtin_bit_cast(uint64_t, v);
+        uint32_t la, lb, ha, hb;
+        if (step == 0) swap_rows16((uint32_t)u, la, lb), swap_rows16((uint32_t)(u >> 32), ha, hb);
+        else swap_rows32((uint32_t)u, la, lb), swap_rows32((uint32_t)(u >> 32), ha, hb);
+        v = __builtin_bit_cast(double, ((uint64_t)ha << 32) | la) + __builtin_bit_cast(double, ((uint64_t)hb << 32) | lb);
+    }
+    return v;
+}
+
+template <int LP>
+__device__ __forceinline__ void quant_wide_store(const float *x, int l, uint8_t *qb, bool st) {
+    constexpr int VP = 256 / LP;
+    float mp = 0.f, mn = 0.f;
+#pragma unroll
+    for (int k = 0; k < VP; ++k) {
+        mp = fmaxf(mp, x[k]);
+        mn = fmaxf(mn, -x[k]);
+    }
+    const int mpb = sblk_reduce<LP>(__float_as_int(mp), [](int a, int c) { return a > c ? a : c; });
+    const int mnb = sblk_reduce<LP>(__float_as_int(mn), [](int a, int c) { return a > c ? a : c; });
+    const float m = __int_as_float(mpb > mnb ? mpb : mnb);
+    bool neg = mnb > mpb;
+    if (__any(mpb == mnb && mpb != 0)) {
+        uint32_t key = 0xffffffffu;
+#pragma unroll
+        for (int k = VP - 1; k >= 0; --k)
+            if (fabsf(x[k]) == m) key = 2u * (uint32_t)(VP * l + k) + (x[k] < 0.f ? 1u : 0u);
+        key = (uint32_t)sblk_reduce<LP>((int)key, [](int a, int c) { return (uint32_t)a < (uint32_t)c ? a : c; });
+        if (mpb == mnb && mpb != 0) neg = (key & 1u) != 0;
+    }
+    const float maxv = neg ? -m : m;
+    const float iscale = -127.f / maxv;
+    uint32_t q[VP / 4];
+    int bsum = 0;
+#pragma unroll
+    for (int k = 0; k < VP / 4; ++k) {
+        q[k] = qbyte(iscale, x[4 * k]) | (qbyte(iscale, x[4 * k + 1]) << 8) | (qbyte(iscale, x[4 * k + 2]) << 16) |
+               (qbyte(iscale, x[4 * k + 3]) << 24);
+        bsum = sdot4(q[k], 0x01010101u, bsum);
+    }
+    float d = 1.f / iscale;
+    if (m == 0.f) {
+#pragma unroll
+        for (int k = 0; k < VP / 4; ++k) q[k] = 0u;
+        bsum = 0;
+        d = 0.f;
+    }
+    bsum += __builtin_amdgcn_update_dpp(bsum, bsum, 0xB1, 0xF, 0xF, false);
+    if (VP == 4) bsum += __builtin_amdgcn_update_dpp(bsum, bsum, 0x4E, 0xF, 0xF, false);
+    if (st) {
+        if (VP == 8) *(uint2 *)(qb + 16 + 8 * l) = make_uint2(q[0], q[VP / 4 - 1]);
+        else *(uint32_t *)(qb + 16 + 4 * l) = q[0];
+        if (!(l & (16 / VP - 1))) *(int16_t *)(qb + 272 + 2 * (l / (16 / VP))) = (int16_t)bsum;
+        if (l == 0) *(float *)qb = d;
+    }
+}
+
 __device__ __forceinline__ uint32_t gload4_asm(const float *p) {
     uint32_t r;
     asm volatile("global_load_dword %0, %1, off" : "=v"(r) : "v"(p) : "memory");
@@ -108,6 +192,10 @@
     u32x4 r;
     asm volatile("global_load_dwordx4 %0, %1, off" : "=v"(r) : "v"(p) : "memory");
     return r;
+}
+
+__device__ __forceinline__ void gload16_into(u32x4 &r, const float *p) {
+    asm volatile("global_load_dwordx4 %0, %1, off" : "+v"(r) : "v"(p) : "memory");
 }
 
 __device__ __forceinline__ int dotacc(u32x4 q, u32x4 a, int acc) {
diff --git a/ggml-neon-opt_amd/ggml_mi355x/__init__.py b/ggml-neon-opt_amd/ggml_mi355x/__init__.py
--- a/ggml-neon-opt_amd/ggml_mi355x/__init__.py
+++ b/ggml-neon-opt_amd/ggml_mi355x/__init__.py
@@ -55,6 +55,7 @@
     "mi355x_attn_prompt",
     "mi355x_attn_prompt_impl",
     "mi355x_attn_batch", "mi355x_attn_batch_path",
+    "mi355x_rows_prologue_plan", "mi355x_debug_rows_prologue",
 )
 
 
@@ -166,6 +167,10 @@
     L.mi355x_debug_block_partials.restype = i32
     L.mi355x_debug_stream.argtypes = [vp, sz, vp, vp]
     L.mi355x_debug_stream.restype = i32
+    L.mi355x_rows_prologue_plan.argtypes = [i64, i32, i64, ctypes.POINTER(i32), ctypes.POINTER(i32)]
+    L.mi355x_rows_prologue_plan.restype = i32
+    L.mi355x_debug_rows_prologue.argtypes = [i32, vp, vp, ctypes.c_float, i64, i32, vp, sz, vp]
+    L.mi355x_debug_rows_prologue.restype = i32
     L.mi355x_backend_init.argtypes = [i32]
     L.mi355x_backend_init.restype = vp
     L.mi355x_backend_free.argtypes = [vp]
@@ -400,6 +405,23 @@
     return int(lib().mi355x_gemv_waves(waves))
 
 
+def rows_prologue_plan(k, waves, steps=0):
+    lanes, passes = ctypes.c_int(0), ctypes.c_int(0)
+    rc = int(lib().mi355x_rows_prologue_plan(k, waves, steps, ctypes.byref(lanes), ctypes.byref(passes)))
+    return (lanes.value, passes.value) if rc == 0 else rc
+
+
+def debug_rows_prologue(x, waves, prologue=PRO_NONE, x2=None, eps=0.0, stream=None):
+    _require_device()
+    torch = _torch()
+    K = x.shape[-1]
+    out = torch.empty((K // QK_K, 304), dtype=torch.uint8, device=x.device)
+    _check(lib().mi355x_debug_rows_prologue(prologue, x.data_ptr(), x2.data_ptr() if x2 is not None else None, eps, K,
+                                            waves, out.data_ptr(), out.numel(), _stream(stream)),
+           "mi355x_debug_rows_prologue")
+    return out
+
+
 DEBUG_KNOBS = ("GEMV_DIAG", "GEMV_RING", "GEMV_PRE0", "GEMV_PF", "GEMV_XMODE", "GEMV_SMALL_MB", "GEMV_WPC",
                "GEMV_SMALL_WG", "GEMV_FQMAX", "MMF_WAVES", "MMF_ORDER", "ATTN_DIAG", "LOOPBACK_NOCOPY",
                "ATTN_OPROJ", "AO_NRB", "GEMV_DYN", "GEMV_DYN_P", "GEMV_DYN_STEPS")
diff --git a/include/ggml_mi355x.h b/include/ggml_mi355x.h
--- a/include/ggml_mi355x.h
+++ b/include/ggml_mi355x.h
@@ -121,6 +121,9 @@
 int mi355x_debug_stream(const void *buf, size_t bytes, void *sink, void *stream);
 int mi355x_debug_block_partials(int src0_type, const void *src0, int64_t ne00, int64_t ne01,
                                 size_t nb01, const void *src1_q8, int32_t *out, void *stream);
+int mi355x_rows_prologue_plan(int64_t k, int waves, int64_t steps, int *lanes, int *passes);
+int mi355x_debug_rows_prologue(int prologue, const float *x, const float *x2, float eps, int64_t k, int waves,
+                               void *out, size_t out_bytes, void *stream);
 
 typedef struct {
     char kernel[96];
```
